# JoeyT1994/TensorNetworkQuantumSimulator.jl

Measured on AMD Instinct MI355X. Metric: two-site gates/sec at fixed chi (LxL TFIM Trotter layer), higher is better.
Workload: dtype c64 (ComplexF32; Gram/eigen steps in f64; the chi = 32 plane products as exact bf16 x 3 splits with f32 accumulation, TNQS_NO_BF16X3=1 for f32 matrix instructions)

## Files before the change

### include/tnqs_debug.h

```cpp
#ifndef TNQS_DEBUG_H
#define TNQS_DEBUG_H
#include <stdint.h>
#include "tnqs.h"
#ifdef __cplusplus
extern "C" {
#endif
int tnqs_dbg_jacobi(int dtype, int m, int n, void* A_inout, void* V_out, int* sweeps_out);
int tnqs_dbg_theta_svd_pre(int m, int n, int nq, void* A_inout, const void* Q, void* V_out, int* sweeps_out, int copies, int reps, double* ms_out, double* phase_us_out ,
                           int cap );
int tnqs_dbg_time_jacobi_f32(int m, int n, const void* A, int copies, int reps, double* ms_out, int* sweeps_out);
int tnqs_dbg_chol(int n, const void* G, void* L_out, void* W_out, int* fail_out, double tau);
int tnqs_dbg_fiber_gemm(int dtype, int D, int PA, int K, int PB, int Do, int No, const void* in, const void* X, void* out,
                        double* norm2_out, int use_mfma);
int tnqs_dbg_gram(int dtype, int D, int PA, int K, int PB, const void* X, const void* Y, void* out, int acc64, int use_mfma);
int tnqs_dbg_gram_fused(int PA, int K, int PB, const void* X, const void* Y, const void* M, void* out);
int tnqs_dbg_gauge_gram(int z, const int* chi, int bleg, const void* X, const void* M, void* out);
int tnqs_dbg_pair(int C0, int NMID, int NHI, const void* in, const void* Mx, const void* My, void* out);
int tnqs_dbg_pair_legs(int d, int z, const int* chi, int lx, int ly, const void* in, const void* Mx, const void* My, void* out);
int tnqs_dbg_pair_gram(int d, int z, const int* chi, int lx, int ly, const void* X, const void* Y, const void* M, void* out);
int tnqs_dbg_pair_gram2(int d, int z, const int* chi, int lx, int ly, const void* X, const void* Y, const void* Mx, const void* My, void* out_y, void* out_x);
int tnqs_dbg_bench_plane(int which, int nsites, int lx, int ly, int reps, double* ms);
#define TNQS_DBG_ROUTE_X3 1
#define TNQS_DBG_ROUTE_F32 2
#define TNQS_DBG_ROUTE_F64 3
#define TNQS_DBG_ROUTE_F64_SHARED 4
#define TNQS_DBG_ROUTE_HALF_LINES 5
#define TNQS_DBG_ROUTE_WHOLE_LINES 6
#define TNQS_DBG_ROUTE_SMALL_SCALAR 7
#define TNQS_DBG_ROUTE_SMALL_MFMA16 8
int tnqs_dbg_rowgemm(int D, int K, int nitems, const int* PA, const int* PB, const int* No, const void* in, const void* X, void* out, double* norm2_out,
                     int tpw, int* route_out);
int tnqs_dbg_gram_mfma(int nitems, const int* shape, const void* X, const void* Y, void* out, int nchunks, int* route_out);
int tnqs_dbg_pair16(int d, int nitems, const int* z, const int* chi, const int* lx, const int* ly, const void* in, const void* M, void* out, int spw, int* route_out);
int tnqs_dbg_pair_gram2x16(int d, int nitems, const int* z, const int* chi, const int* lx, const int* ly, const int* both, const void* X, const void* Y, const void* M,
                           void* out_y, void* out_x, int spw);
int tnqs_dbg_svd_tall(int nitems, const int* m, const int* n, void* A, int* chol_fail, int* polished, int* sweeps);
int tnqs_dbg_small_site(int nitems, const int* d, const int* z, const int* chi, const int* jo, const void* psi, const void* M, const int* present, int form,
                        const void* old_msg, const int* has_old, int normalize, void* out, void* new_msg, double* diff_out, int* route_out);
int tnqs_dbg_msg_finalize(int dtype, int nitems, const int* chi, const int* nchunks, const void* partials, const void* old_msg, const int* has_old, int normalize,
                          void* new_msg, double* diff_out);
int tnqs_dbg_default_sequence(tnqs_handle h, int* src, int* dst, int cap, int* n_out);
int tnqs_dbg_default_sequence_graph(int nv, int ne, const int32_t* esrc, const int32_t* edst, int* src, int* dst, int* level, int cap, int* n_out);
int tnqs_dbg_gate_schedule(int nv, int ne, const int32_t* esrc, const int32_t* edst, int ngates, const int32_t* nverts, const int32_t* verts, int update_cache,
                           int* step_of_gate, int* step_is_bp, int cap, int* nsteps_out);
int tnqs_dbg_fiber_plan(int use, int dtype, int use_mfma, int use_chi64, int nitems, const int* shape, int* launches_out, int cap, int* nlaunches_out, int* items_out);
int tnqs_dbg_loop_cgemm(int dtype, int opB, int nitems, const int* m, const int* n, const int* k, const void* A, const void* B, void* C, int guard);
int tnqs_dbg_loop_antiproject(int dtype, int nitems, const int* nr, const int* nc, void* T_inout, const void* f, const void* b);
int tnqs_dbg_loop_trace(int dtype, int nitems, const int* p, const int* q, const void* X, const void* Y, double* out_re_im);
int tnqs_dbg_msg_rescale(int dtype, int nitems, const int* chi, const void* me, const void* mer, const int* present, void* me_out, void* mer_out, int guard);
int tnqs_dbg_edge_scalar(int dtype, int nitems, const int* chi, const void* me, const void* mer, const int* present, double* out_re_im);
int tnqs_dbg_env_prepare(int dtype, int nitems, const int* n, const void* msg, const int* present, void* H_out, void* V_out, int guard);
int tnqs_dbg_env_finish(int dtype, int nitems, const int* n, const void* A, const void* V, const double* cutoff, void* msqrt_out, void* proj_out, int* flags_out, int guard);
int tnqs_dbg_symg_build(int dtype, int nitems, const int* n, const void* AX, const void* VX, const void* AY, const void* VY, double reg, void* rx, void* ry, void* irx, void* iry,
                        void* Ce, void* Ce0, int* flag_out, int guard);
int tnqs_dbg_symg_finish(int dtype, int nitems, const int* n, const void* USigma, const void* Vsvd, const void* irx, const void* iry, void* Xs, void* Xd, double* S, int guard);
int tnqs_dbg_diag(int dtype, int nitems, const int* chi, const double* S, void* out, int guard);
int tnqs_dbg_cscale(int dtype, int nitems, const int* len, const void* src, const double* re, const double* im, void* dst, int guard);
int tnqs_dbg_pending_scale(tnqs_handle h, int v, double* factor);
#ifdef __cplusplus
}
#endif
#endif
```

### tensornetworkquantumsimulator.jl_amd/csrc/api.cpp

```cpp
#include <cmath>
#include <cstring>
#include <string>
#include "engine.hpp"

using namespace tnqs;

struct tnqs_state_s { State* s; };

static thread_local std::string g_err;

template <class F> static int guard(F&& f) {
    try { f(); return TNQS_OK; }
    catch (const Err& e) { g_err = e.what(); return e.code; }
    catch (const std::bad_alloc&) { g_err = "out of host memory"; return TNQS_ERR_HIP; }
    catch (const std::exception& e) { g_err = e.what(); return TNQS_ERR_INVALID; }
    catch (...) { g_err = "unknown error"; return TNQS_ERR_INVALID; }
}
static State* S(tnqs_handle h) { if (!h || !h->s) throw Err(TNQS_ERR_INVALID, "null handle"); return h->s; }

extern "C" {

int tnqs_version(void) { return 102; }
const char* tnqs_last_error(void) { return g_err.c_str(); }
int tnqs_device_count(int* count) {
// ... 80 lines not shown
            double ore = op[2 * (sp + d * si)], oim = op[2 * (sp + d * si) + 1];
            double rre = r[2 * (si + d * sp)], rim = r[2 * (si + d * sp) + 1];
            nre += ore * rre - oim * rim; nim += ore * rim + oim * rre;
        }
        for (int si = 0; si < d; ++si) { tre += r[2 * (si + d * si)]; tim += r[2 * (si + d * si) + 1]; }
        double den = tre * tre + tim * tim;
        out[0] = (nre * tre + nim * tim) / den; out[1] = (nim * tre - nre * tim) / den;
    });
}
int tnqs_expect_region(tnqs_handle h, int nr, const int32_t* rv, const int32_t* parent, const double* ops, double* out4) {
    return guard([&] { expect_region(S(h), nr, rv, parent, ops, out4); });
}
int tnqs_vertex_scalars(tnqs_handle h, double* out) { return guard([&] { if (!out) throw Err(TNQS_ERR_INVALID, "vertex_scalars: null"); vertex_scalars(S(h), out); }); }
int tnqs_edge_scalars(tnqs_handle h, double* out) { return guard([&] { if (!out) throw Err(TNQS_ERR_INVALID, "edge_scalars: null"); edge_scalars(S(h), out); }); }
int tnqs_rescale(tnqs_handle h) { return guard([&] { rescale(S(h)); }); }
int tnqs_rescale_messages(tnqs_handle h, int n_edges, const int32_t* eu, const int32_t* ev) {
    return guard([&] { if (n_edges < 0) throw Err(TNQS_ERR_INVALID, "rescale_messages: negative count"); rescale_messages(S(h), n_edges, eu, ev); });
}
int tnqs_rescale_vertices(tnqs_handle h, int n_vertices, const int32_t* verts) {
    return guard([&] { if (n_vertices < 0) throw Err(TNQS_ERR_INVALID, "rescale_vertices: negative count"); rescale_vertices(S(h), n_vertices, verts); });
}
int tnqs_symmetric_gauge(tnqs_handle h, double regularization) { return guard([&] { symmetric_gauge(S(h), regularization); }); }
int tnqs_project_site(tnqs_handle h, int v, int config) { return guard([&] { project_site(S(h), v, config); }); }
int tnqs_site_dim(tnqs_handle h, int v, int* d) { return guard([&] { if (!d) throw Err(TNQS_ERR_INVALID, "site_dim: null output"); site_dim(S(h), v, d); }); }
int tnqs_site_probabilities(tnqs_handle h, int v, double* out_p) { return guard([&] { if (!out_p) throw Err(TNQS_ERR_INVALID, "site_probabilities: null output"); site_probabilities(S(h), v, out_p); }); }
int tnqs_sample_bp(tnqs_handle h, int nsamples, const tnqs_bp_opts* bp_opts, uint64_t seed, const double* uniforms, int32_t* out_config, double* out_prob, tnqs_apply_stats* stats) {
    return guard([&] { sample_bp(S(h), nsamples, bp_opts, seed, uniforms, out_config, out_prob, stats); });
}
int tnqs_loop_weights(tnqs_handle h, int ncycles, const int32_t* cycle_len, const int32_t* cycle_verts, double* out_re_im) {
    return guard([&] { loop_weights(S(h), ncycles, cycle_len, cycle_verts, out_re_im); });
}
int tnqs_expect_all(tnqs_handle h, const double* ops, double* out) {
    return guard([&] { if (!ops || !out) throw Err(TNQS_ERR_INVALID, "expect_all: null"); expect_all(S(h), ops, out); });
}

int tnqs_set_sharding(tnqs_handle h, int rank, int nranks, const int32_t* owner, tnqs_allgather_fn fn, void* ctx,
                      void* exch_dev, int64_t exch_bytes) {
    return guard([&] {
        State* s = S(h);
        if (nranks < 1 || rank < 0 || rank >= nranks) throw Err(TNQS_ERR_INVALID, "set_sharding: bad rank");
        if (nranks > 1) {
            if (!owner || !fn || !exch_dev || exch_bytes <= 0) throw Err(TNQS_ERR_INVALID, "set_sharding: owner, callback and exchange buffer are required for nranks > 1");
            for (int v = 0; v < s->g->nv; ++v) if (owner[v] < 0 || owner[v] >= nranks) throw Err(TNQS_ERR_INVALID, "set_sharding: owner out of range");
            s->owner.assign(owner, owner + s->g->nv);
        } else s->owner.clear();
        materialize_pending_all(s);
        s->comm.reset();
        s->rank = rank; s->nranks = nranks; s->ag_fn = fn; s->ag_ctx = ctx; s->exch = exch_dev; s->exch_bytes = (size_t)exch_bytes;
        if (nranks > 1) for (int v = 0; v < s->g->nv; ++v) if (!s->owns(v)) { s->site[v] = nullptr; s->sscale[v] = nullptr; }
    });
}

int tnqs_rccl_unique_id(void* out128) { return guard([&] { if (!out128) throw Err(TNQS_ERR_INVALID, "rccl_unique_id: null output"); rccl_unique_id(out128); }); }
int tnqs_set_sharding_rccl(tnqs_handle h, int rank, int nranks, const int32_t* owner, const void* unique_id128, int64_t exch_bytes) {
    return guard([&] { set_sharding_rccl(S(h), rank, nranks, owner, unique_id128, exch_bytes); });
}
int tnqs_sharding_stats(tnqs_handle h, int64_t* n_exchanges, int64_t* bytes_exchanged) {
    return guard([&] { State* s = S(h); if (n_exchanges) *n_exchanges = s->comm ? s->comm->n_exchanges : 0; if (bytes_exchanged) *bytes_exchanged = s->comm ? s->comm->bytes_exchanged : 0; });
}
int tnqs_rccl_selftest(int device, int64_t bytes) { return guard([&] { rccl_selftest(device, bytes); }); }
int tnqs_rccl_preflight(void) { return guard([&] { rccl_preflight(); }); }

int tnqs_profile_enable(tnqs_handle h, int on) { return guard([&] { S(h)->prof->on = on != 0; }); }
int tnqs_profile_get(tnqs_handle h, int cls, int64_t* launches, double* ms, double* bytes, double* flops) {
    return guard([&] {
        State* s = S(h);
        if (cls < 0 || cls >= TNQS_PROF_NCLASSES) throw Err(TNQS_ERR_INVALID, "profile_get: bad class");
        prof_collect(s);
        const ProfClass& pc = s->prof->cls[cls];
        if (launches) *launches = pc.launches;
        if (ms) *ms = pc.ms;
        if (bytes) *bytes = pc.bytes;
        if (flops) *flops = pc.flops;
    });
}
int tnqs_profile_reset(tnqs_handle h) {
    return guard([&] { State* s = S(h); prof_collect(s); for (auto& p : s->prof->cls) p = ProfClass{}; });
}

}

#include "../../include/tnqs_debug.h"
#include "kernels.hpp"
namespace tnqs { void dbg_default_sequence(const Graph& g, std::vector<int>& src, std::vector<int>& dst);
                 std::shared_ptr<Graph> dbg_make_graph(int nv, int ne, const int32_t* es, const int32_t* ed);
                 void dbg_default_sequence_graph(const Graph& g, std::vector<int>& src, std::vector<int>& dst, std::vector<int>& level);
                 void dbg_pair(int C0, int NMID, int NHI, const void* in, const void* Mx, const void* My, void* out);
                 void dbg_gram_fused(int PA, int K, int PB, const void* X, const void* Y, const void* M, void* out);
                 void dbg_gauge_gram(int z, const int* chi, int bleg, const void* X, const void* M, void* out);
                 void dbg_jacobi(int dtype, int m, int n, void* A, void* V, int* sweeps);
                 void dbg_chol(int n, const void* G, void* L, void* W, int* fail, double tau);
                 void dbg_theta_svd_pre(int m, int n, int nq, void* A, const void* Q, void* V, int* sweeps, int copies, int reps, double* ms, double* phase_us, int cap);
                 void dbg_time_jacobi_f32(int m, int n, const void* A, int copies, int reps, double* ms, int* sweeps);
                 void dbg_pair_legs(int d, int z, const int* chi, int lx, int ly, const void* in, const void* Mx, const void* My, void* out);
                 void dbg_pair_gram2(int d, int z, const int* chi, int lx, int ly, const void* X, const void* Y, const void* Mx, const void* My, void* out_y, void* out_x);
                 void dbg_bench_plane(int which, int nsites, int lx, int ly, int reps, double* ms);
                 void dbg_pair_gram(int d, int z, const int* chi, int lx, int ly, const void* X, const void* Y, const void* M, void* out);
                 void dbg_fiber_gemm(int dtype, int D, int PA, int K, int PB, int Do, int No, const void* in, const void* X, void* out, double* norm2, int use_mfma);
                 void dbg_gram(int dtype, int D, int PA, int K, int PB, const void* X, const void* Y, void* out, int acc64, int use_mfma);
                 void dbg_rowgemm(int D, int K, int nitems, const int* PA, const int* PB, const int* No, const void* in, const void* X, void* out, double* norm2, int tpw, int* route);
                 void dbg_gram_mfma(int nitems, const int* shape, const void* X, const void* Y, void* out, int nchunks, int* route);
                 void dbg_pair16(int d, int nitems, const int* z, const int* chi, const int* lx, const int* ly, const void* in, const void* M, void* out, int spw, int* route);
                 void dbg_pair_gram2x16(int d, int nitems, const int* z, const int* chi, const int* lx, const int* ly, const int* both, const void* X, const void* Y, const void* M,
                                        void* out_y, void* out_x, int spw);
                 void dbg_svd_tall(int nitems, const int* m, const int* n, void* A, int* chol_fail, int* polished, int* sweeps);
                 void dbg_small_site(int nitems, const int* d, const int* z, const int* chi, const int* jo, const void* psi, const void* M, const int* present, int form,
                                     const void* old_msg, const int* has_old, int normalize, void* out, void* new_msg, double* diff, int* route);
                 void dbg_msg_finalize(int dtype, int nitems, const int* chi, const int* nchunks, const void* partials, const void* old_msg, const int* has_old, int normalize,
                                       void* new_msg, double* diff);
                 void dbg_loop_cgemm(int dtype, int opB, int nitems, const int* m, const int* n, const int* k, const void* A, const void* B, void* C, int guard);
                 void dbg_loop_antiproject(int dtype, int nitems, const int* nr, const int* nc, void* T, const void* f, const void* b);
                 void dbg_loop_trace(int dtype, int nitems, const int* p, const int* q, const void* X, const void* Y, double* out);
                 void dbg_msg_rescale(int dtype, int nitems, const int* chi, const void* me, const void* mer, const int* present, void* me_out, void* mer_out, int guard);
                 void dbg_edge_scalar(int dtype, int nitems, const int* chi, const void* me, const void* mer, const int* present, double* out);
                 void dbg_env_prepare(int dtype, int nitems, const int* n, const void* msg, const int* present, void* H_out, void* V_out, int guard);
                 void dbg_env_finish(int dtype, int nitems, const int* n, const void* A, const void* V, const double* cutoff, void* msqrt_out, void* proj_out, int* flags_out, int guard);
                 void dbg_symg_build(int dtype, int nitems, const int* n, const void* AX, const void* VX, const void* AY, const void* VY, double reg, void* rx, void* ry, void* irx, void* iry,
                                     void* Ce, void* Ce0, int* flag_out, int guard);
                 void dbg_symg_finish(int dtype, int nitems, const int* n, const void* USigma, const void* Vsvd, const void* irx, const void* iry, void* Xs, void* Xd, double* S, int guard);
                 void dbg_diag(int dtype, int nitems, const int* chi, const double* S, void* out, int guard);
                 void dbg_cscale(int dtype, int nitems, const int* len, const void* src, const double* re, const double* im, void* dst, int guard);
                 double dbg_pending_scale(State* s, int v); }
extern "C" {
int tnqs_dbg_default_sequence(tnqs_handle h, int* src, int* dst, int cap, int* n_out) {
    return guard([&] { std::vector<int> a, b; dbg_default_sequence(*S(h)->g, a, b); *n_out = (int)a.size();
                       for (int i = 0; i < (int)a.size() && i < cap; ++i) { src[i] = a[i]; dst[i] = b[i]; } });
}
int tnqs_dbg_default_sequence_graph(int nv, int ne, const int32_t* esrc, const int32_t* edst, int* src, int* dst, int* level, int cap, int* n_out) {
    return guard([&] { if (nv < 0 || ne < 0 || (ne > 0 && (!esrc || !edst)) || !n_out) throw Err(TNQS_ERR_INVALID, "tnqs_dbg_default_sequence_graph: bad arguments");
                       auto g = dbg_make_graph(nv, ne, esrc, edst); std::vector<int> a, b, l; dbg_default_sequence_graph(*g, a, b, l); *n_out = (int)a.size();
                       for (int i = 0; i < (int)a.size() && i < cap; ++i) { if (src) src[i] = a[i]; if (dst) dst[i] = b[i]; if (level) level[i] = l[i]; } });
}
int tnqs_dbg_gate_schedule(int nv, int ne, const int32_t* esrc, const int32_t* edst, int ngates, const int32_t* nverts, const int32_t* verts, int update_cache,
                           int* step_of_gate, int* step_is_bp, int cap, int* nsteps_out) {
    return guard([&] { if (nv < 0 || ne < 0 || (ne > 0 && (!esrc || !edst)) || ngates < 0 || (ngates > 0 && (!nverts || !verts)) || !nsteps_out) throw Err(TNQS_ERR_INVALID, "tnqs_dbg_gate_schedule: bad arguments");
                       for (int i = 0, o = 0; i < ngates; o += nverts[i], ++i) { if (nverts[i] < 1 || nverts[i] > 2) throw Err(TNQS_ERR_INVALID, "tnqs_dbg_gate_schedule: only one- and two-site gates");
                                                                                 for (int k = 0; k < nverts[i]; ++k) if (verts[o + k] < 0 || verts[o + k] >= nv) throw Err(TNQS_ERR_INVALID, "tnqs_dbg_gate_schedule: vertex out of range"); }
                       auto g = dbg_make_graph(nv, ne, esrc, edst); const GateSchedule steps = build_gate_schedule(*g, ngates, nverts, verts, update_cache != 0); *nsteps_out = (int)steps.size();
                       for (int k = 0; k < (int)steps.size(); ++k) { if (step_is_bp && k < cap) step_is_bp[k] = steps[k].is_bp ? 1 : 0; if (step_of_gate) for (int i = steps[k].begin; i < steps[k].end; ++i) step_of_gate[i] = k; } });
}
int tnqs_dbg_fiber_plan(int use, int dtype, int use_mfma, int use_chi64, int nitems, const int* shape, int* launches, int cap, int* nlaunches_out, int* items_out) {
    return guard([&] { if (use < 0 || use > 2 || (dtype != TNQS_C64 && dtype != TNQS_C128) || nitems < 0 || (nitems > 0 && !shape) || !nlaunches_out) throw Err(TNQS_ERR_INVALID, "tnqs_dbg_fiber_plan: bad arguments");
                       std::vector<FiberItem> items(nitems);
                       for (int i = 0; i < nitems; ++i) { const int* q = shape + 6 * i; for (int k = 0; k < 6; ++k) if (q[k] < 1) throw Err(TNQS_ERR_INVALID, "tnqs_dbg_fiber_plan: bad shape");
                                                          FiberItem& it = items[i]; it.D = q[0]; it.PA = q[1]; it.K = q[2]; it.PB = q[3]; it.Do = q[4]; it.No = q[5]; }
                       const std::vector<FiberLaunch> plan = plan_fiber_pass(items.data(), nitems, fiber_rules(use == 0 ? FiberUse::Chain : use == 1 ? FiberUse::Epilogue : FiberUse::Plain, dtype == TNQS_C64, use_mfma != 0, use_chi64 != 0),
                                                                            dtype == TNQS_C64 ? 8 : 16);
                       *nlaunches_out = (int)plan.size();
                       for (int l = 0; l < (int)plan.size(); ++l) { const FiberLaunch& L = plan[l];
                           if (launches && l < cap) { const int v[10] = {(int)L.route, L.D, L.K, L.TR, L.tpw, L.KKmax, L.NNmax, L.wgs, (int)L.items.size(), L.general ? 1 : 0}; std::copy(v, v + 10, launches + 10 * l); }
                           if (items_out) for (size_t k = 0; k < L.items.size(); ++k) { const FiberItem& it = L.items[k]; const int v[7] = {l, it.tile_begin, L.nwg[k], it.TA, it.TB, it.nta, it.ntb}; std::copy(v, v + 7, items_out + 7 * L.index[k]); } } });
}
int tnqs_dbg_jacobi(int dtype, int m, int n, void* A, void* V, int* sweeps) { return guard([&] { dbg_jacobi(dtype, m, n, A, V, sweeps); }); }
int tnqs_dbg_theta_svd_pre(int m, int n, int nq, void* A, const void* Q, void* V, int* sweeps, int copies, int reps, double* ms, double* phase_us, int cap) { return guard([&] { dbg_theta_svd_pre(m, n, nq, A, Q, V, sweeps, copies, reps, ms, phase_us, cap); }); }
int tnqs_dbg_time_jacobi_f32(int m, int n, const void* A, int copies, int reps, double* ms, int* sweeps) { return guard([&] { dbg_time_jacobi_f32(m, n, A, copies, reps, ms, sweeps); }); }
int tnqs_dbg_chol(int n, const void* G, void* L, void* W, int* fail, double tau) { return guard([&] { dbg_chol(n, G, L, W, fail, tau); }); }
int tnqs_dbg_fiber_gemm(int dtype, int D, int PA, int K, int PB, int Do, int No, const void* in, const void* X, void* out, double* norm2, int use_mfma) {
    return guard([&] { dbg_fiber_gemm(dtype, D, PA, K, PB, Do, No, in, X, out, norm2, use_mfma); });
}
int tnqs_dbg_pair(int C0, int NMID, int NHI, const void* in, const void* Mx, const void* My, void* out) { return guard([&] { dbg_pair(C0, NMID, NHI, in, Mx, My, out); }); }
int tnqs_dbg_pair_legs(int d, int z, const int* chi, int lx, int ly, const void* in, const void* Mx, const void* My, void* out) { return guard([&] { dbg_pair_legs(d, z, chi, lx, ly, in, Mx, My, out); }); }
int tnqs_dbg_pair_gram2(int d, int z, const int* chi, int lx, int ly, const void* X, const void* Y, const void* Mx, const void* My, void* out_y, void* out_x) {
    return guard([&] { dbg_pair_gram2(d, z, chi, lx, ly, X, Y, Mx, My, out_y, out_x); });
}
int tnqs_dbg_bench_plane(int which, int nsites, int lx, int ly, int reps, double* ms) { return guard([&] { dbg_bench_plane(which, nsites, lx, ly, reps, ms); }); }
int tnqs_dbg_pair_gram(int d, int z, const int* chi, int lx, int ly, const void* X, const void* Y, const void* M, void* out) { return guard([&] { dbg_pair_gram(d, z, chi, lx, ly, X, Y, M, out); }); }
int tnqs_dbg_gram_fused(int PA, int K, int PB, const void* X, const void* Y, const void* M, void* out) { return guard([&] { dbg_gram_fused(PA, K, PB, X, Y, M, out); }); }
int tnqs_dbg_gauge_gram(int z, const int* chi, int bleg, const void* X, const void* M, void* out) { return guard([&] { dbg_gauge_gram(z, chi, bleg, X, M, out); }); }
int tnqs_dbg_gram(int dtype, int D, int PA, int K, int PB, const void* X, const void* Y, void* out, int acc64, int use_mfma) {
    return guard([&] { dbg_gram(dtype, D, PA, K, PB, X, Y, out, acc64, use_mfma); });
}
int tnqs_dbg_rowgemm(int D, int K, int nitems, const int* PA, const int* PB, const int* No, const void* in, const void* X, void* out, double* norm2_out, int tpw, int* route_out) {
    return guard([&] { dbg_rowgemm(D, K, nitems, PA, PB, No, in, X, out, norm2_out, tpw, route_out); });
}
int tnqs_dbg_gram_mfma(int nitems, const int* shape, const void* X, const void* Y, void* out, int nchunks, int* route_out) {
    return guard([&] { dbg_gram_mfma(nitems, shape, X, Y, out, nchunks, route_out); });
}
int tnqs_dbg_pair16(int d, int nitems, const int* z, const int* chi, const int* lx, const int* ly, const void* in, const void* M, void* out, int spw, int* route_out) {
    return guard([&] { dbg_pair16(d, nitems, z, chi, lx, ly, in, M, out, spw, route_out); });
}
int tnqs_dbg_pair_gram2x16(int d, int nitems, const int* z, const int* chi, const int* lx, const int* ly, const int* both, const void* X, const void* Y, const void* M,
                           void* out_y, void* out_x, int spw) {
    return guard([&] { dbg_pair_gram2x16(d, nitems, z, chi, lx, ly, both, X, Y, M, out_y, out_x, spw); });
}
int tnqs_dbg_svd_tall(int nitems, const int* m, const int* n, void* A, int* chol_fail, int* polished, int* sweeps) {
    return guard([&] { dbg_svd_tall(nitems, m, n, A, chol_fail, polished, sweeps); });
}
int tnqs_dbg_small_site(int nitems, const int* d, const int* z, const int* chi, const int* jo, const void* psi, const void* M, const int* present, int form,
                        const void* old_msg, const int* has_old, int normalize, void* out, void* new_msg, double* diff_out, int* route_out) {
    return guard([&] { dbg_small_site(nitems, d, z, chi, jo, psi, M, present, form, old_msg, has_old, normalize, out, new_msg, diff_out, route_out); });
}
int tnqs_dbg_msg_finalize(int dtype, int nitems, const int* chi, const int* nchunks, const void* partials, const void* old_msg, const int* has_old, int normalize,
                          void* new_msg, double* diff_out) {
    return guard([&] { dbg_msg_finalize(dtype, nitems, chi, nchunks, partials, old_msg, has_old, normalize, new_msg, diff_out); });
}
int tnqs_dbg_loop_cgemm(int dtype, int opB, int nitems, const int* m, const int* n, const int* k, const void* A, const void* B, void* C, int guard_elems) {
    return guard([&] { dbg_loop_cgemm(dtype, opB, nitems, m, n, k, A, B, C, guard_elems); });
}
int tnqs_dbg_loop_antiproject(int dtype, int nitems, const int* nr, const int* nc, void* T, const void* f, const void* b) { return guard([&] { dbg_loop_antiproject(dtype, nitems, nr, nc, T, f, b); }); }
int tnqs_dbg_loop_trace(int dtype, int nitems, const int* p, const int* q, const void* X, const void* Y, double* out) { return guard([&] { dbg_loop_trace(dtype, nitems, p, q, X, Y, out); }); }
int tnqs_dbg_msg_rescale(int dtype, int nitems, const int* chi, const void* me, const void* mer, const int* present, void* me_out, void* mer_out, int guard_elems) {
    return guard([&] { dbg_msg_rescale(dtype, nitems, chi, me, mer, present, me_out, mer_out, guard_elems); });
}
int tnqs_dbg_edge_scalar(int dtype, int nitems, const int* chi, const void* me, const void* mer, const int* present, double* out_re_im) {
    return guard([&] { dbg_edge_scalar(dtype, nitems, chi, me, mer, present, out_re_im); });
}
int tnqs_dbg_env_prepare(int dtype, int nitems, const int* n, const void* msg, const int* present, void* H_out, void* V_out, int guard_elems) {
    return guard([&] { dbg_env_prepare(dtype, nitems, n, msg, present, H_out, V_out, guard_elems); });
}
int tnqs_dbg_env_finish(int dtype, int nitems, const int* n, const void* A, const void* V, const double* cutoff, void* msqrt_out, void* proj_out, int* flags_out, int guard_elems) {
    return guard([&] { dbg_env_finish(dtype, nitems, n, A, V, cutoff, msqrt_out, proj_out, flags_out, guard_elems); });
}
int tnqs_dbg_symg_build(int dtype, int nitems, const int* n, const void* AX, const void* VX, const void* AY, const void* VY, double reg, void* rx, void* ry, void* irx, void* iry,
                        void* Ce, void* Ce0, int* flag_out, int guard_elems) {
    return guard([&] { dbg_symg_build(dtype, nitems, n, AX, VX, AY, VY, reg, rx, ry, irx, iry, Ce, Ce0, flag_out, guard_elems); });
}
int tnqs_dbg_symg_finish(int dtype, int nitems, const int* n, const void* USigma, const void* Vsvd, const void* irx, const void* iry, void* Xs, void* Xd, double* S, int guard_elems) {
    return guard([&] { dbg_symg_finish(dtype, nitems, n, USigma, Vsvd, irx, iry, Xs, Xd, S, guard_elems); });
}
int tnqs_dbg_diag(int dtype, int nitems, const int* chi, const double* S, void* out, int guard_elems) { return guard([&] { dbg_diag(dtype, nitems, chi, S, out, guard_elems); }); }
int tnqs_dbg_cscale(int dtype, int nitems, const int* len, const void* src, const double* re, const double* im, void* dst, int guard_elems) {
    return guard([&] { dbg_cscale(dtype, nitems, len, src, re, im, dst, guard_elems); });
}
int tnqs_dbg_pending_scale(tnqs_handle h, int v, double* factor) { return guard([&] { if (!factor) throw Err(TNQS_ERR_INVALID, "dbg_pending_scale: null output"); *factor = dbg_pending_scale(S(h), v); }); }
}
```

### tensornetworkquantumsimulator.jl_amd/csrc/debug.cpp

```cpp
#include <cstdio>
#include <cstring>
#include <cstdlib>
#include <vector>
#include <algorithm>
#include <memory>
#include <string>
#include "engine.hpp"
#include "kernels.hpp"
#include "launch_util.hpp"
#include "../../include/tnqs_debug.h"

namespace tnqs {
#define HIPCHK(x) hipchk((x), #x)
struct DBuf { void* p = nullptr; explicit DBuf(size_t n) { HIPCHK(hipMalloc(&p, n ? n : 1)); } ~DBuf() { (void)hipFree(p); }
              void up(const void* h, size_t n) { HIPCHK(hipMemcpy(p, h, n, hipMemcpyHostToDevice)); } void down(void* h, size_t n) { HIPCHK(hipMemcpy(h, p, n, hipMemcpyDeviceToHost)); } };
static void need_gpu() { int n = 0; if (hipGetDeviceCount(&n) != hipSuccess || n <= 0) throw Err(TNQS_ERR_HIP, "no HIP device available"); }

void dbg_jacobi(int dtype, int m, int n, void* A, void* V, int* sweeps) {
    need_gpu();
    if (m < 1 || n < 1 || m > 256 || n > 256) throw Err(TNQS_ERR_INVALID, "dbg_jacobi: 1 <= m, n <= 256");
    size_t esz = dtype == TNQS_C64 ? 8 : 16;
    DBuf dA((size_t)m * n * esz), dV((size_t)n * n * esz), dS(4), dI(sizeof(JacobiItem));
    dA.up(A, (size_t)m * n * esz);
    if (dtype == TNQS_C64) launch_identity<float>(nullptr, dV.p, n); else launch_identity<double>(nullptr, dV.p, n);
    const size_t lim = 160 * 1024 - 2048;
    size_t lds_av = jacobi_lds_bytes(m, n, true, esz), lds_a = jacobi_lds_bytes(m, n, false, esz);
    const char* fg = std::getenv("TNQS_DBG_NOV_GLOBAL");
    const bool force_global_nov = fg && fg[0] == '1';
    const char* ft = std::getenv("TNQS_DBG_THETA_SVD");
    const bool theta_route = ft && ft[0] == '1' && dtype == TNQS_C64 && lds_a <= lim;
    const bool nov = force_global_nov || theta_route || (lds_av > lim && lds_a <= lim);
    DBuf dA0((size_t)m * n * esz);
    if (nov) dA0.up(A, (size_t)m * n * esz);
    JacobiItem it{dA.p, nov ? nullptr : dV.p, m, n, (int*)dS.p};
    dI.up(&it, sizeof(it));
    size_t lds = force_global_nov ? 0 : (nov ? lds_a : (lds_av <= lim ? lds_av : 0));
    if (dtype == TNQS_C64) launch_jacobi<float>(nullptr, (const JacobiItem*)dI.p, 1, 60, lds, std::max(m, n)); else launch_jacobi<double>(nullptr, (const JacobiItem*)dI.p, 1, 60, lds, std::max(m, n));
    if (nov) {
        DBuf dRv(sizeof(RecoverItem)); RecoverItem rv{dA0.p, dA.p, dV.p, m, n, n}; dRv.up(&rv, sizeof(rv));
        if (dtype == TNQS_C64) launch_recover_v_mfma(nullptr, (const RecoverItem*)dRv.p, 1, n); else launch_recover_v<double>(nullptr, (const RecoverItem*)dRv.p, 1, n);
        HIPCHK(hipDeviceSynchronize());
    }
    HIPCHK(hipDeviceSynchronize());
    dA.down(A, (size_t)m * n * esz); dV.down(V, (size_t)n * n * esz);
    if (sweeps) dS.down(sweeps, 4);
}

void dbg_theta_svd_pre(int m, int n, int nq, void* A, const void* Q, void* V, int* sweeps, int copies, int reps, double* ms, double* phase_us, int cap) {
    need_gpu();
    if (!Q) nq = n;
    if (!theta_svd_pre_covers(m, n) || nq < n || nq > m) throw Err(TNQS_ERR_INVALID, "dbg_theta_svd_pre: 2 <= n <= 64, n <= nq <= m <= 128");
    if (copies < 1) copies = 1;
    const size_t ab = (size_t)m * n * 8, vb = (size_t)nq * n * 8;
    DBuf dA(ab * copies), dA0(ab), dQ((size_t)nq * n * 16), dV(vb * copies), dS(4 * (size_t)copies), dInfo(32), dI(sizeof(JacobiItem) * (size_t)copies), dT(64);
    dA0.up(A, ab); if (Q) dQ.up(Q, (size_t)nq * n * 16);
    const int info[8] = {m, nq, 0, 0, 0, 0, 0, Q ? n : 0};
    dInfo.up(info, 32);
    std::vector<JacobiItem> its(copies);
    for (int c = 0; c < copies; ++c) {
        JacobiItem it{}; it.A = (char*)dA.p + ab * c; it.V = (c == 0 && phase_us) ? dT.p : nullptr; it.m = m; it.n = nq; it.sweeps_out = (int*)dS.p + c; it.dyn = (const int*)dInfo.p; it.dm = 1; it.dn = 1; it.nhint = n;
        it.QB = Q ? dQ.p : nullptr; it.Vout = (char*)dV.p + vb * c; it.pre = 0 ; it.cap = cap; its[c] = it;
    }
    dI.up(its.data(), sizeof(JacobiItem) * (size_t)copies);
    auto reset = [&]() { for (int c = 0; c < copies; ++c) HIPCHK(hipMemcpyAsync((char*)dA.p + ab * c, dA0.p, ab, hipMemcpyDeviceToDevice, nullptr)); };
    reset();
    launch_theta_svd_pre(nullptr, (const JacobiItem*)dI.p, copies, 60, m, n);
    HIPCHK(hipDeviceSynchronize());
    dA.down(A, ab); dV.down(V, vb);
    if (sweeps) dS.down(sweeps, 4);
    if (phase_us) {
        unsigned long long t[8]; dT.down(t, 64);
        for (int k = 0; k < 6; ++k) phase_us[k] = (double)(t[k + 1] - t[k]) * 0.01;
    }
    if (reps > 0 && ms) {
        hipEvent_t e0, e1; HIPCHK(hipEventCreate(&e0)); HIPCHK(hipEventCreate(&e1));
        double tot = 0;
        for (int r = 0; r < reps; ++r) {
            reset();
            HIPCHK(hipEventRecord(e0, nullptr));
            launch_theta_svd_pre(nullptr, (const JacobiItem*)dI.p, copies, 60, m, n);
            HIPCHK(hipEventRecord(e1, nullptr)); HIPCHK(hipEventSynchronize(e1));
            float t = 0; HIPCHK(hipEventElapsedTime(&t, e0, e1)); tot += t;
        }
        *ms = tot / reps;
        (void)hipEventDestroy(e0); (void)hipEventDestroy(e1);
    }
}
void dbg_time_jacobi_f32(int m, int n, const void* A, int copies, int reps, double* ms, int* sweeps) {
    need_gpu();
    if (copies < 1) copies = 1;
    const size_t ab = (size_t)m * n * 8;
    DBuf dA(ab * copies), dA0(ab), dS(4 * (size_t)copies), dI(sizeof(JacobiItem) * (size_t)copies);
    dA0.up(A, ab);
    std::vector<JacobiItem> its(copies);
    for (int c = 0; c < copies; ++c) { JacobiItem it{}; it.A = (char*)dA.p + ab * c; it.m = m; it.n = n; it.sweeps_out = (int*)dS.p + c; its[c] = it; }
    dI.up(its.data(), sizeof(JacobiItem) * (size_t)copies);
    hipEvent_t e0, e1; HIPCHK(hipEventCreate(&e0)); HIPCHK(hipEventCreate(&e1));
    double tot = 0;
// ... 2 lines not shown
        HIPCHK(hipEventRecord(e0, nullptr));
        launch_jacobi<float>(nullptr, (const JacobiItem*)dI.p, copies, 60, jacobi_lds_bytes(m, n, false, 8), std::max(m, n), n);
        HIPCHK(hipEventRecord(e1, nullptr)); HIPCHK(hipEventSynchronize(e1));
        float t = 0; HIPCHK(hipEventElapsedTime(&t, e0, e1)); if (r > 0) tot += t;
    }
    if (ms) *ms = tot / std::max(1, reps);
    if (sweeps) dS.down(sweeps, 4);
    (void)hipEventDestroy(e0); (void)hipEventDestroy(e1);
}

void dbg_chol(int n, const void* G, void* Lout, void* Wout, int* fail, double tau) {
    need_gpu();
    if (n < 1 || n > 128) throw Err(TNQS_ERR_INVALID, "dbg_chol: 1 <= n <= 128");
    const size_t b = (size_t)n * n * 16;
    DBuf dG(b), dL(b), dW(b), dF(4), dI(sizeof(CholItem));
    dG.up(G, b); HIPCHK(hipMemset(dF.p, 0, 4)); HIPCHK(hipMemset(dW.p, 0, b));
    CholItem it{dG.p, dL.p, dW.p, n, (int*)dF.p, tau, 0.0};
    dI.up(&it, sizeof(it));
    if (n <= 96) launch_chol(nullptr, (const CholItem*)dI.p, 1, n); else launch_chol_packed(nullptr, (const CholItem*)dI.p, 1, n);
    HIPCHK(hipDeviceSynchronize());
    dL.down(Lout, b); dW.down(Wout, b); dF.down(fail, 4);
}

void dbg_fiber_gemm(int dtype, int D, int PA, int K, int PB, int Do, int No, const void* in, const void* X, void* out, double* norm2, int use_mfma) {
    need_gpu();
    size_t esz = dtype == TNQS_C64 ? 8 : 16;
    size_t nin = (size_t)D * PA * K * PB, nout = (size_t)Do * PA * No * PB, nx = (size_t)D * K * Do * No;
    DBuf dIn(nin * esz), dX(nx * esz), dOut(nout * esz), dI(sizeof(FiberItem));
    dIn.up(in, nin * esz); dX.up(X, nx * esz);
    HIPCHK(hipMemset(dOut.p, 0xff, nout * esz));
    FiberItem it{}; it.in = dIn.p; it.out = dOut.p; it.X = dX.p; it.D = D; it.PA = PA; it.K = K; it.PB = PB; it.Do = Do; it.No = No;
    it.want_norm = 1;
    FiberRules r = fiber_rules(FiberUse::Epilogue, dtype == TNQS_C64, use_mfma != 0, true); r.rg_D = 0; r.kk_min = 1; r.mfma_tpw = 5; r.f64_tpw = 12;
    const std::vector<FiberLaunch> plan = plan_fiber_pass(&it, 1, r, esz);
    const FiberLaunch& L = plan[0]; const int tiles = L.wgs;
    DBuf dN((size_t)tiles * 8);
    dI.up(L.items.data(), sizeof(FiberItem));
    if (dtype == TNQS_C64) launch_fiber_route<float>(nullptr, L, (const FiberItem*)dI.p, (double*)dN.p);
    else launch_fiber_route<double>(nullptr, L, (const FiberItem*)dI.p, (double*)dN.p);
    HIPCHK(hipDeviceSynchronize());
    dOut.down(out, nout * esz);
    if (norm2) { std::vector<double> np(tiles); dN.down(np.data(), (size_t)tiles * 8); double t = 0; for (double v : np) t += v; *norm2 = t; }
}

void dbg_gram(int dtype, int D, int PA, int K, int PB, const void* X, const void* Y, void* out, int acc64, int use_mfma) {
    need_gpu();
    size_t esz = dtype == TNQS_C64 ? 8 : 16;
    size_t nin = (size_t)D * PA * K * PB; int KK = D * K;
    bool same = (X == Y);
    DBuf dX(nin * esz), dY(same ? 1 : nin * esz), dI(sizeof(GramItem)), dR(sizeof(ReduceItem));
    dX.up(X, nin * esz); if (!same) dY.up(Y, nin * esz);
    GramItem it{}; it.X = dX.p; it.Y = same ? dX.p : dY.p; it.D = D; it.PA = PA; it.K = K; it.PB = PB;
    const bool mf = use_mfma && dtype == TNQS_C64 && !acc64 && KK <= 32;
    const bool mf64 = use_mfma && dtype == TNQS_C64 && acc64 && same && KK <= 64 && KK >= 16;
    const bool mfz = use_mfma && dtype == TNQS_C128 && gram_f64in_covers(D, K);
    const GramRoute r = mfz ? GramRoute::F64In : mf64 ? GramRoute::F64x64 : mf ? GramRoute::Mfma32 : GramRoute::Generic;
    const int TR = gram_tile_rows(r, KK, esz);
    tile_params(PA, PB, TR, it.TA, it.TB, it.nta, it.ntb);
    const char* e = std::getenv("TNQS_DBG_GRAM_CHUNKS");
    int npart = 0; plan_gram(&it, 1, r, false, e ? std::max(1, std::atoi(e)) : 7, &npart);
    bool a64 = acc64 || dtype == TNQS_C128;
    size_t asz = a64 ? 16 : 8;
    DBuf dP((size_t)npart * KK * KK * asz), dO((size_t)KK * KK * asz);
    it.partial = dP.p; dI.up(&it, sizeof(it));
    const GramItem* d = (const GramItem*)dI.p;
    if (dtype == TNQS_C128) launch_gram_route<double, double>(nullptr, r, d, 1, it.nchunks, TR, KK, KK == 64);
    else if (a64) launch_gram_route<float, double>(nullptr, r, d, 1, it.nchunks, TR, KK, KK == 64);
    else launch_gram_route<float, float>(nullptr, r, d, 1, it.nchunks, TR, KK);
    ReduceItem ri{dP.p, dO.p, KK * KK, npart, 0, 0}; dR.up(&ri, sizeof(ri));
    if (a64) launch_reduce<double, double>(nullptr, (const ReduceItem*)dR.p, 1, KK * KK); else launch_reduce<float, float>(nullptr, (const ReduceItem*)dR.p, 1, KK * KK);
    HIPCHK(hipDeviceSynchronize());
    dO.down(out, (size_t)KK * KK * asz);
}
void dbg_pair(int C0, int NMID, int NHI, const void* in, const void* Mx, const void* My, void* out) {
    need_gpu();
    if (C0 % 16) throw Err(TNQS_ERR_INVALID, "dbg_pair: C0 % 16 != 0");
    size_t n = (size_t)C0 * 32 * NMID * 32 * NHI;
    DBuf dIn(n * 8), dOut(n * 8), dX(32 * 32 * 8), dY(32 * 32 * 8), dI(sizeof(PairItem));
    dIn.up(in, n * 8); dX.up(Mx, 32 * 32 * 8); dY.up(My, 32 * 32 * 8);
    HIPCHK(hipMemset(dOut.p, 0xff, n * 8));
    PairItem it{}; it.in = dIn.p; it.out = dOut.p; it.Mx = dX.p; it.My = dY.p;
    it.g.cstr = 2; it.g.sx = C0; it.g.sy = (long long)C0 * 32 * NMID; it.g.n0 = C0 / 16; it.g.t0 = 16; it.g.n1 = NMID; it.g.t1 = (long long)C0 * 32;
    it.g.n2 = NHI; it.g.t2 = (long long)C0 * 32 * NMID * 32;
    const int wgs = plan_pair(&it, 1, 3);
    dI.up(&it, sizeof(it));
    launch_mfma_pair(nullptr, (const PairItem*)dI.p, 1, wgs);
    HIPCHK(hipDeviceSynchronize());
    dOut.down(out, n * 8);
}
void dbg_pair_legs(int d, int z, const int* chi, int lx, int ly, const void* in, const void* Mx, const void* My, void* out) {
    need_gpu();
    PairItem it{};
    if (!pair_geometry(d, z, chi, lx, ly, it.g)) throw Err(TNQS_ERR_UNSUPPORTED, "dbg_pair_legs: shape not covered by the pair kernel");
    size_t n = d; for (int i = 0; i < z; ++i) n *= chi[i];
    DBuf dIn(n * 8), dOut(n * 8), dX(32 * 32 * 8), dY(32 * 32 * 8), dI(sizeof(PairItem));
    dIn.up(in, n * 8); dX.up(Mx, 32 * 32 * 8); dY.up(My, 32 * 32 * 8);
    HIPCHK(hipMemset(dOut.p, 0xff, n * 8));
    it.in = dIn.p; it.out = dOut.p; it.Mx = dX.p; it.My = dY.p;
    if ((size_t)it.g.n0 * it.g.n1 * it.g.n2 * 16 * 1024 != n) throw Err(TNQS_ERR_INVALID, "dbg_pair_legs: slice count");
    const int wgs = plan_pair(&it, 1, 3);
    dI.up(&it, sizeof(it));
    launch_mfma_pair(nullptr, (const PairItem*)dI.p, 1, wgs);
    HIPCHK(hipDeviceSynchronize());
    dOut.down(out, n * 8);
}
void dbg_pair_gram(int d, int z, const int* chi, int lx, int ly, const void* X, const void* Y, const void* M, void* out) {
    need_gpu();
    PairGramItem it{};
    if (!pair_geometry(d, z, chi, lx, ly, it.g)) throw Err(TNQS_ERR_UNSUPPORTED, "dbg_pair_gram: shape not covered by the pair kernel");
    size_t n = d; for (int i = 0; i < z; ++i) n *= chi[i];
    const bool x3 = mfma_use_x3();
    PairGram2Item one{}; one.g = it.g;
    const int nwg = x3 ? plan_x3_pair_gram1(&one, 1, nullptr, 3) : plan_pair_gram(&it, 1, nullptr, 3), npart = nwg;
    DBuf dX(n * 8), dY(n * 8), dM(32 * 32 * 8), dI(sizeof(PairGram2Item)), dR(sizeof(ReduceItem)), dP((size_t)npart * 1024 * 8), dO(1024 * 8);
    dX.up(X, n * 8); dY.up(Y, n * 8); dM.up(M, 32 * 32 * 8);
    it.X = dX.p; it.Y = dY.p; it.M = dM.p; it.partial = dP.p;
    if (x3) {
        one.X = it.X; one.Y = it.Y; one.Mx = it.M; one.partial_y = it.partial;
        dI.up(&one, sizeof(one));
        launch_x3_pair_gram1(nullptr, (const PairGram2Item*)dI.p, 1, nwg);
    } else {
        dI.up(&it, sizeof(it));
        launch_mfma_pair_gram(nullptr, (const PairGramItem*)dI.p, 1, nwg);
    }
    ReduceItem ri{dP.p, dO.p, 1024, npart, 0, 0}; dR.up(&ri, sizeof(ri));
    launch_reduce<float, float>(nullptr, (const ReduceItem*)dR.p, 1, 1024);
    HIPCHK(hipDeviceSynchronize());
    dO.down(out, 1024 * 8);
}
void dbg_pair_gram2(int d, int z, const int* chi, int lx, int ly, const void* X, const void* Y, const void* Mx, const void* My, void* out_y, void* out_x) {
    need_gpu();
    PairGram2Item it{};
    if (!pair_geometry(d, z, chi, lx, ly, it.g)) throw Err(TNQS_ERR_UNSUPPORTED, "dbg_pair_gram2: shape not covered");
    size_t n = d; for (int i = 0; i < z; ++i) n *= chi[i];
    const int nwg = plan_pair_gram2(&it, 1, nullptr, 3), npart = nwg;
    DBuf dX(n * 8), dY(n * 8), dMx(1024 * 8), dMy(1024 * 8), dI(sizeof(PairGram2Item)), dR(2 * sizeof(ReduceItem)), dP1((size_t)npart * 1024 * 8), dP2((size_t)npart * 1024 * 8), dO(2 * 1024 * 8);
    dX.up(X, n * 8); dY.up(Y, n * 8); dMx.up(Mx, 1024 * 8); dMy.up(My, 1024 * 8);
    it.X = dX.p; it.Y = dY.p; it.Mx = dMx.p; it.My = dMy.p; it.partial_y = dP1.p; it.partial_x = dP2.p;
    dI.up(&it, sizeof(it));
    launch_mfma_pair_gram2(nullptr, (const PairGram2Item*)dI.p, 1, nwg);
    ReduceItem ri[2] = {{dP1.p, dO.p, 1024, npart, 0, 0}, {dP2.p, (char*)dO.p + 1024 * 8, 1024, npart, 0, 1024}};
    dR.up(ri, sizeof(ri));
    launch_reduce<float, float>(nullptr, (const ReduceItem*)dR.p, 2, 2048);
    HIPCHK(hipDeviceSynchronize());
    dO.down(out_y, 1024 * 8);
    HIPCHK(hipMemcpy(out_x, (char*)dO.p + 1024 * 8, 1024 * 8, hipMemcpyDeviceToHost));
}
static void fill_random(void* d, size_t nfloats, unsigned seed) {
    const size_t blk = (size_t)1 << 22;
    std::vector<float> h(blk + 4096);
    unsigned x = seed * 2654435761u + 12345u;
    for (auto& v : h) { x = x * 1664525u + 1013904223u; v = ((int)(x >> 8) - (1 << 23)) * (0.01f / (1 << 23)); }
    size_t off = 0; unsigned k = 0;
    while (off < nfloats) {
        const size_t m = std::min(blk, nfloats - off);
        HIPCHK(hipMemcpy((char*)d + off * 4, h.data() + (k * 257u) % 4096u, m * 4, hipMemcpyHostToDevice));
        off += m; ++k;
    }
}
static void dbg_bench_plane16(int which, int nsites, int lx, int ly, int reps, double* ms) {
    const int chi[6] = {16, 16, 16, 16, 16, 16};
    PlaneGeom g{};
    if (!plane_geometry(2, 6, chi, lx, ly, 16, g)) throw Err(TNQS_ERR_UNSUPPORTED, "dbg_bench_plane: legs not covered");
    const size_t n = (size_t)2 << 24;
    DBuf dA((size_t)nsites * n * 8), dB((size_t)nsites * n * 8), dM(2 * 256 * 8);
    fill_random(dA.p, (size_t)nsites * n * 2, 1); fill_random(dB.p, (size_t)nsites * n * 2, 2); fill_random(dM.p, 2 * 256 * 2, 3);
    hipEvent_t e0, e1; HIPCHK(hipEventCreate(&e0)); HIPCHK(hipEventCreate(&e1));
    float t = 0.f;
    if (which == 2) {
        std::vector<Pair16Item> items(nsites);
        for (int i = 0; i < nsites; ++i) {
            Pair16Item& it = items[i]; it.g = g; it.in = (char*)dA.p + (size_t)i * n * 8; it.out = (char*)dB.p + (size_t)i * n * 8;
            it.Mx = dM.p; it.My = (char*)dM.p + 256 * 8;
        }
        int w[2]; plan_pair16(items.data(), nsites, w);
        const int wgs = w[pair16_whole_lines(g) ? 1 : 0];
        DBuf dI(items.size() * sizeof(Pair16Item)); dI.up(items.data(), items.size() * sizeof(Pair16Item));
        launch_mfma_pair16(nullptr, (const Pair16Item*)dI.p, nsites, wgs, pair16_whole_lines(g));
        HIPCHK(hipEventRecord(e0, nullptr));
        for (int r = 0; r < reps; ++r) launch_mfma_pair16(nullptr, (const Pair16Item*)dI.p, nsites, wgs, pair16_whole_lines(g));
        HIPCHK(hipEventRecord(e1, nullptr)); HIPCHK(hipEventSynchronize(e1)); HIPCHK(hipEventElapsedTime(&t, e0, e1));
    } else {
        std::vector<PairGram2x16Item> items(nsites);
        for (auto& it : items) it.g = g;
        const int wgs = plan_pair_gram2x16(items.data(), nsites), nwg = wgs / nsites;
        DBuf dP((size_t)2 * nsites * nwg * 256 * 8);
        for (int i = 0; i < nsites; ++i) {
            PairGram2x16Item& it = items[i]; it.X = (char*)dA.p + (size_t)i * n * 8; it.Y = (char*)dB.p + (size_t)i * n * 8;
            it.Mx = dM.p; it.My = (char*)dM.p + 256 * 8;
            it.partial_y = (char*)dP.p + (size_t)(2 * i) * nwg * 256 * 8; it.partial_x = (char*)dP.p + (size_t)(2 * i + 1) * nwg * 256 * 8;
        }
        DBuf dI(items.size() * sizeof(PairGram2x16Item)); dI.up(items.data(), items.size() * sizeof(PairGram2x16Item));
        launch_mfma_pair_gram2x16(nullptr, (const PairGram2x16Item*)dI.p, nsites, wgs);
        HIPCHK(hipEventRecord(e0, nullptr));
        for (int r = 0; r < reps; ++r) launch_mfma_pair_gram2x16(nullptr, (const PairGram2x16Item*)dI.p, nsites, wgs);
        HIPCHK(hipEventRecord(e1, nullptr)); HIPCHK(hipEventSynchronize(e1)); HIPCHK(hipEventElapsedTime(&t, e0, e1));
    }
    HIPCHK(hipDeviceSynchronize());
    (void)hipEventDestroy(e0); (void)hipEventDestroy(e1);
    *ms = (double)t / reps;
}
void dbg_bench_plane(int which, int nsites, int lx, int ly, int reps, double* ms) {
    need_gpu();
    if (which == 2 || which == 3) { dbg_bench_plane16(which, nsites, lx, ly, reps, ms); return; }
    const int chi[4] = {32, 32, 32, 32};
    PairGeom g{};
    if (!pair_geometry(2, 4, chi, lx, ly, g)) throw Err(TNQS_ERR_UNSUPPORTED, "dbg_bench_plane: legs not covered");
    const size_t n = (size_t)2 * 32 * 32 * 32 * 32;
    DBuf dA((size_t)nsites * n * 8), dB((size_t)nsites * n * 8), dM(2 * 1024 * 8);
    fill_random(dA.p, (size_t)nsites * n * 2, 1); fill_random(dB.p, (size_t)nsites * n * 2, 2); fill_random(dM.p, 2 * 1024 * 2, 3);
    hipEvent_t e0, e1; HIPCHK(hipEventCreate(&e0)); HIPCHK(hipEventCreate(&e1));
    float t = 0.f;
    if (which == 4) {
        const char* e = std::getenv("TNQS_DBG_GROUP"); int G = e ? std::atoi(e) : 0; if (G <= 0 || G > nsites) G = nsites;
        int ox = -1, oy = -1; for (int q = 0; q < 4; ++q) if (q != lx && q != ly) { if (ox < 0) ox = q; else oy = q; }
        PairGeom g2{}; if (!pair_geometry(2, 4, chi, ox, oy, g2)) throw Err(TNQS_ERR_UNSUPPORTED, "dbg_bench_plane: other legs not covered");
        const int ngroups = (nsites + G - 1) / G;
        std::vector<PairItem> pit(nsites); std::vector<PairGram2Item> git(nsites);
        for (int i = 0; i < nsites; ++i) { pit[i].g = g; git[i].g = g2; }
        std::vector<int> pw(ngroups), gwg(ngroups), nwg(nsites);
        for (int gr = 0; gr < ngroups; ++gr) {
            const int cnt = std::min(G, nsites - gr * G);
            pw[gr] = plan_pair(&pit[(size_t)gr * G], cnt, gr ? pit[0].spw : 0);
            gwg[gr] = plan_pair_gram2(&git[(size_t)gr * G], cnt, &nwg[(size_t)gr * G], gr ? git[0].spw : 0);
        }
        const int spw_p = pit[0].spw, spw_g = git[0].spw, nwg_g = nwg[0];
        DBuf dT((size_t)G * n * 8), dP((size_t)2 * nsites * nwg_g * 1024 * 8);
        for (int i = 0; i < nsites; ++i) {
            const int k = i % G;
            PairItem& a = pit[i]; a.in = (char*)dA.p + (size_t)i * n * 8; a.out = (char*)dT.p + (size_t)k * n * 8; a.Mx = dM.p; a.My = (char*)dM.p + 1024 * 8;
            PairGram2Item& b = git[i]; b.X = a.out; b.Y = a.in; b.Mx = dM.p; b.My = (char*)dM.p + 1024 * 8;
            b.partial_y = (char*)dP.p + (size_t)(2 * i) * nwg_g * 1024 * 8; b.partial_x = (char*)dP.p + (size_t)(2 * i + 1) * nwg_g * 1024 * 8;
        }
        DBuf dPI(pit.size() * sizeof(PairItem)), dGI(git.size() * sizeof(PairGram2Item));
        dPI.up(pit.data(), pit.size() * sizeof(PairItem)); dGI.up(git.data(), git.size() * sizeof(PairGram2Item));
        auto level = [&]() {
            for (int gr = 0; gr < ngroups; ++gr) {
                const int cnt = std::min(G, nsites - gr * G);
                launch_mfma_pair(nullptr, (const PairItem*)dPI.p + (size_t)gr * G, cnt, pw[gr]);
                launch_mfma_pair_gram2(nullptr, (const PairGram2Item*)dGI.p + (size_t)gr * G, cnt, gwg[gr]);
            }
        };
        level();
        HIPCHK(hipEventRecord(e0, nullptr));
        for (int r = 0; r < reps; ++r) level();
        HIPCHK(hipEventRecord(e1, nullptr)); HIPCHK(hipEventSynchronize(e1)); HIPCHK(hipEventElapsedTime(&t, e0, e1));
        std::fprintf(stderr, "level bench: group %d, pair spw %d, gram spw %d\n", G, spw_p, spw_g);
    } else if (which == 0) {
        std::vector<PairItem> items(nsites);
        for (int i = 0; i < nsites; ++i) {
            PairItem& it = items[i]; it.g = g; it.in = (char*)dA.p + (size_t)i * n * 8; it.out = (char*)dB.p + (size_t)i * n * 8;
            it.Mx = dM.p; it.My = (char*)dM.p + 1024 * 8;
        }
        const int wgs = plan_pair(items.data(), nsites);
        DBuf dI(items.size() * sizeof(PairItem)); dI.up(items.data(), items.size() * sizeof(PairItem));
        launch_mfma_pair(nullptr, (const PairItem*)dI.p, nsites, wgs);
        HIPCHK(hipEventRecord(e0, nullptr));
        for (int r = 0; r < reps; ++r) launch_mfma_pair(nullptr, (const PairItem*)dI.p, nsites, wgs);
        HIPCHK(hipEventRecord(e1, nullptr)); HIPCHK(hipEventSynchronize(e1)); HIPCHK(hipEventElapsedTime(&t, e0, e1));
    } else {
        std::vector<PairGram2Item> items(nsites);
        for (auto& it : items) it.g = g;
        const int wgs = plan_pair_gram2(items.data(), nsites, nullptr, 16), nwg = wgs / nsites;
        DBuf dP((size_t)2 * nsites * nwg * 1024 * 8);
        for (int i = 0; i < nsites; ++i) {
            PairGram2Item& it = items[i]; it.X = (char*)dA.p + (size_t)i * n * 8; it.Y = (char*)dB.p + (size_t)i * n * 8;
            it.Mx = dM.p; it.My = (char*)dM.p + 1024 * 8;
            it.partial_y = (char*)dP.p + (size_t)(2 * i) * nwg * 1024 * 8; it.partial_x = (char*)dP.p + (size_t)(2 * i + 1) * nwg * 1024 * 8;
        }
        DBuf dI(items.size() * sizeof(PairGram2Item)); dI.up(items.data(), items.size() * sizeof(PairGram2Item));
        launch_mfma_pair_gram2(nullptr, (const PairGram2Item*)dI.p, nsites, wgs);
        HIPCHK(hipEventRecord(e0, nullptr));
        for (int r = 0; r < reps; ++r) launch_mfma_pair_gram2(nullptr, (const PairGram2Item*)dI.p, nsites, wgs);
        HIPCHK(hipEventRecord(e1, nullptr)); HIPCHK(hipEventSynchronize(e1)); HIPCHK(hipEventElapsedTime(&t, e0, e1));
    }
    HIPCHK(hipDeviceSynchronize());
    (void)hipEventDestroy(e0); (void)hipEventDestroy(e1);
    *ms = (double)t / reps;
}
void dbg_gram_fused(int PA, int K, int PB, const void* X, const void* Y, const void* M, void* out) {
    need_gpu();
    size_t nin = (size_t)PA * K * PB;
    DBuf dX(nin * 8), dY(nin * 8), dM(32 * 32 * 8), dI(sizeof(GramItem)), dR(sizeof(ReduceItem));
    dX.up(X, nin * 8); dY.up(Y, nin * 8); dM.up(M, 32 * 32 * 8);
    GramItem it{}; it.X = dX.p; it.Y = dY.p; it.M = dM.p; it.D = 1; it.PA = PA; it.K = K; it.PB = PB;
    tile_params(PA, PB, 64, it.TA, it.TB, it.nta, it.ntb);
    if (it.TA * it.TB != 64) throw Err(TNQS_ERR_INVALID, "dbg_gram_fused: tiles must hold 64 fibers");
    int npart = 0; plan_gram(&it, 1, GramRoute::Fused32, false, 3, &npart);
    DBuf dP((size_t)npart * K * K * 8), dO((size_t)K * K * 8);
    it.partial = dP.p; dI.up(&it, sizeof(it));
    launch_gram_route<float, float>(nullptr, GramRoute::Fused32, (const GramItem*)dI.p, 1, it.nchunks, 64, K);
    ReduceItem ri{dP.p, dO.p, K * K, npart, 0, 0}; dR.up(&ri, sizeof(ri));
    launch_reduce<float, float>(nullptr, (const ReduceItem*)dR.p, 1, K * K);
    HIPCHK(hipDeviceSynchronize());
    dO.down(out, (size_t)K * K * 8);
}
void dbg_gauge_gram(int z, const int* chi, int bleg, const void* X, const void* M, void* out) {
    need_gpu();
    if (z < 2 || z > 8 || bleg < 0 || bleg >= z) throw Err(TNQS_ERR_INVALID, "dbg_gauge_gram: bad shape");
    const int rleg = bleg == 0 ? 1 : 0, K = chi[bleg], KK = 2 * K;
    const bool k16 = gauge_gram32_covers(2, z, chi, bleg, rleg), k32 = gauge_gram64_covers(2, z, chi, bleg, rleg);
    if (!k16 && !k32) throw Err(TNQS_ERR_UNSUPPORTED, "dbg_gauge_gram: shape not covered by the fused kernels");
    size_t n = 2; for (int i = 0; i < z; ++i) n *= chi[i];
    long long PA = 1, PB = 1; for (int i = 0; i < bleg; ++i) PA *= chi[i]; for (int i = bleg + 1; i < z; ++i) PB *= chi[i];
    DBuf dX(n * 8), dM((size_t)chi[rleg] * chi[rleg] * 8), dI(sizeof(GramItem)), dR(sizeof(ReduceItem));
    dX.up(X, n * 8); dM.up(M, (size_t)chi[rleg] * chi[rleg] * 8);
    GramItem it{}; it.X = dX.p; it.Y = dX.p; it.M = dM.p; it.D = 2; it.PA = (int)PA; it.K = K; it.PB = (int)PB;
    tile_params(PA, PB, 64, it.TA, it.TB, it.nta, it.ntb);
    if (k16) { it.nta = gauge_gram32_units(z, chi, bleg); it.ntb = 1; }
    const GramRoute r = k16 ? GramRoute::Gauge32 : GramRoute::Gauge64;
    int npart = 0; plan_gram(&it, 1, r, true, 5, &npart);
    DBuf dP((size_t)npart * KK * KK * 16), dO((size_t)KK * KK * 16);
    HIPCHK(hipMemset(dP.p, 0, (size_t)npart * KK * KK * 16));
    it.partial = dP.p; dI.up(&it, sizeof(it));
    launch_gram_route<float, double>(nullptr, r, (const GramItem*)dI.p, 1, it.nchunks, 64, KK);
    ReduceItem ri{dP.p, dO.p, KK * KK, npart, 0, 0}; dR.up(&ri, sizeof(ri));
    launch_reduce<double, double>(nullptr, (const ReduceItem*)dR.p, 1, KK * KK);
    HIPCHK(hipDeviceSynchronize());
    dO.down(out, (size_t)KK * KK * 16);
}

namespace {
template <class F> void cat_offsets(int n, std::vector<size_t>& off, F&& size_of) { off.assign(n + 1, 0); for (int i = 0; i < n; ++i) off[i + 1] = off[i] + size_of(i); }
}
void svd_tall(State* s, const std::vector<JacobiItem>& tall, int* d_fail, int* d_polish_sweeps);

void dbg_rowgemm(int D, int K, int nitems, const int* PA, const int* PB, const int* No, const void* in, const void* X, void* out, double* norm2, int tpw, int* route) {
    need_gpu();
    if (nitems < 1 || !PA || !PB || !No) throw Err(TNQS_ERR_INVALID, "dbg_rowgemm: bad arguments");
    std::vector<FiberItem> items(nitems);
    for (int i = 0; i < nitems; ++i) {
        FiberItem& it = items[i]; it.D = D; it.PA = PA[i]; it.K = K; it.PB = PB[i]; it.Do = D; it.No = No[i];
        if (PA[i] < 1 || PB[i] < 1 || !rowgemm_covers(it)) throw Err(TNQS_ERR_UNSUPPORTED, "dbg_rowgemm: item not covered by the register-direct kernels");
        it.want_norm = 1;
    }
    std::vector<size_t> oi, ox, oo;
    cat_offsets(nitems, oi, [&](int i) { return (size_t)D * PA[i] * K * PB[i]; });
    cat_offsets(nitems, ox, [&](int i) { return (size_t)D * K * D * No[i]; });
    cat_offsets(nitems, oo, [&](int i) { return (size_t)D * PA[i] * No[i] * PB[i]; });
    DBuf dIn(oi[nitems] * 8), dX(ox[nitems] * 8), dOut(oo[nitems] * 8), dI(sizeof(FiberItem) * nitems);
    dIn.up(in, oi[nitems] * 8); dX.up(X, ox[nitems] * 8);
    HIPCHK(hipMemset(dOut.p, 0xff, oo[nitems] * 8));
    for (int i = 0; i < nitems; ++i) {
        FiberItem& it = items[i];
        it.in = (char*)dIn.p + oi[i] * 8; it.X = (char*)dX.p + ox[i] * 8; it.out = (char*)dOut.p + oo[i] * 8;
    }
// ... 49 lines not shown
        ri[i] = ReduceItem{items[i].partial, (char*)dO.p + oo[i] * asz, (int)(oo[i + 1] - oo[i]), npart[i], 0, (int)oo[i]};
    }
    dI.up(items.data(), sizeof(GramItem) * nitems); dR.up(ri.data(), sizeof(ReduceItem) * nitems);
    if (f64) {
        launch_gram_route<float, double>(nullptr, r, (const GramItem*)dI.p, nitems, chunks, 64, KKmax, all128);
        launch_reduce<double, double>(nullptr, (const ReduceItem*)dR.p, nitems, (int)oo[nitems]);
    } else {
        launch_gram_route<float, float>(nullptr, r, (const GramItem*)dI.p, nitems, chunks, 64, KKmax);
        launch_reduce<float, float>(nullptr, (const ReduceItem*)dR.p, nitems, (int)oo[nitems]);
    }
    HIPCHK(hipDeviceSynchronize());
    dO.down(out, oo[nitems] * asz);
    if (route) *route = f64 ? (all128 ? TNQS_DBG_ROUTE_F64_SHARED : TNQS_DBG_ROUTE_F64) : (mfma_use_x3() ? TNQS_DBG_ROUTE_X3 : TNQS_DBG_ROUTE_F32);
}

static void plane_items(int d, int nitems, const int* z, const int* chi, const int* lx, const int* ly, std::vector<PlaneGeom>& g, std::vector<size_t>& off) {
    if (nitems < 1 || !z || !chi || !lx || !ly || d < 1) throw Err(TNQS_ERR_INVALID, "dbg plane kernels: bad arguments");
    g.resize(nitems);
    int c = 0;
    cat_offsets(nitems, off, [&](int i) {
        if (z[i] < 2 || z[i] > 8) throw Err(TNQS_ERR_INVALID, "dbg plane kernels: 2 <= z <= 8");
        size_t n = d; for (int k = 0; k < z[i]; ++k) n *= chi[c + k];
        if (!plane_geometry(d, z[i], chi + c, lx[i], ly[i], 16, g[i]) || (size_t)g[i].nslices() * 16 * 256 != n)
            throw Err(TNQS_ERR_UNSUPPORTED, "dbg plane kernels: plane not covered by the chi = 16 kernels");
        c += z[i];
        return n;
    });
}
void dbg_pair16(int d, int nitems, const int* z, const int* chi, const int* lx, const int* ly, const void* in, const void* M, void* out, int spw, int* route) {
    need_gpu();
    std::vector<PlaneGeom> g; std::vector<size_t> off;
    plane_items(d, nitems, z, chi, lx, ly, g, off);
    const bool wl = pair16_whole_lines(g[0]);
    for (int i = 0; i < nitems; ++i) if (pair16_whole_lines(g[i]) != wl) throw Err(TNQS_ERR_UNSUPPORTED, "dbg_pair16: one launch holds items of one kind");
    if (spw > 0 && spw % 4) throw Err(TNQS_ERR_INVALID, "dbg_pair16: spw must be a multiple of 4");
    const size_t n = off[nitems];
    DBuf dIn(n * 8), dOut(n * 8), dM((size_t)nitems * 512 * 8), dI(sizeof(Pair16Item) * nitems);
    dIn.up(in, n * 8); dM.up(M, (size_t)nitems * 512 * 8);
    HIPCHK(hipMemset(dOut.p, 0xff, n * 8));
    std::vector<Pair16Item> items(nitems);
    for (int i = 0; i < nitems; ++i) {
        Pair16Item& it = items[i]; it.g = g[i]; it.in = (char*)dIn.p + off[i] * 8; it.out = (char*)dOut.p + off[i] * 8;
        it.Mx = (char*)dM.p + (size_t)i * 512 * 8; it.My = (char*)it.Mx + 256 * 8;
    }
    int wgs[2]; plan_pair16(items.data(), nitems, wgs, spw);
    dI.up(items.data(), sizeof(Pair16Item) * nitems);
    launch_mfma_pair16(nullptr, (const Pair16Item*)dI.p, nitems, wgs[wl ? 1 : 0], wl);
    HIPCHK(hipDeviceSynchronize());
    dOut.down(out, n * 8);
    if (route) *route = wl ? TNQS_DBG_ROUTE_WHOLE_LINES : TNQS_DBG_ROUTE_HALF_LINES;
}
void dbg_pair_gram2x16(int d, int nitems, const int* z, const int* chi, const int* lx, const int* ly, const int* both, const void* X, const void* Y, const void* M,
                       void* out_y, void* out_x, int spw) {
    need_gpu();
    std::vector<PlaneGeom> g; std::vector<size_t> off;
    plane_items(d, nitems, z, chi, lx, ly, g, off);
    if (!both) throw Err(TNQS_ERR_INVALID, "dbg_pair_gram2x16: bad arguments");
    if (spw > 0 && spw % pair_gram2x16_slices_at_a_time()) throw Err(TNQS_ERR_INVALID, "dbg_pair_gram2x16: spw must be a multiple of the slices a workgroup walks at a time");
    const size_t n = off[nitems];
    std::vector<PairGram2x16Item> items(nitems); std::vector<int> nwg(nitems); for (int i = 0; i < nitems; ++i) items[i].g = g[i];
    const int wgs = plan_pair_gram2x16(items.data(), nitems, nwg.data(), spw);
    DBuf dX(n * 8), dY(n * 8), dM((size_t)nitems * 512 * 8), dI(sizeof(PairGram2x16Item) * nitems), dP((size_t)2 * wgs * 256 * 8), dO((size_t)2 * nitems * 256 * 8),
         dR(sizeof(ReduceItem) * 2 * nitems);
    dX.up(X, n * 8); dY.up(Y, n * 8); dM.up(M, (size_t)nitems * 512 * 8);
    HIPCHK(hipMemset(dO.p, 0, (size_t)2 * nitems * 256 * 8));
    std::vector<ReduceItem> ri;
    for (int i = 0; i < nitems; ++i) {
        PairGram2x16Item& it = items[i];
        it.X = (char*)dX.p + off[i] * 8; it.Y = (char*)dY.p + off[i] * 8;
        it.Mx = (char*)dM.p + (size_t)i * 512 * 8; it.My = both[i] ? (const void*)((char*)it.Mx + 256 * 8) : nullptr;
        it.partial_y = (char*)dP.p + (size_t)it.wg_begin * 256 * 8;
        it.partial_x = both[i] ? (void*)((char*)dP.p + ((size_t)wgs + it.wg_begin) * 256 * 8) : nullptr;
        ri.push_back(ReduceItem{it.partial_y, (char*)dO.p + (size_t)i * 256 * 8, 256, nwg[i], 0, (int)ri.size() * 256});
        if (both[i]) ri.push_back(ReduceItem{it.partial_x, (char*)dO.p + ((size_t)nitems + i) * 256 * 8, 256, nwg[i], 0, (int)ri.size() * 256});
    }
    dI.up(items.data(), sizeof(PairGram2x16Item) * nitems); dR.up(ri.data(), sizeof(ReduceItem) * ri.size());
    launch_mfma_pair_gram2x16(nullptr, (const PairGram2x16Item*)dI.p, nitems, wgs);
    launch_reduce<float, float>(nullptr, (const ReduceItem*)dR.p, (int)ri.size(), (int)ri.size() * 256);
    HIPCHK(hipDeviceSynchronize());
    dO.down(out_y, (size_t)nitems * 256 * 8);
    if (out_x) for (int i = 0; i < nitems; ++i) if (both[i]) HIPCHK(hipMemcpy((char*)out_x + (size_t)i * 256 * 8, (char*)dO.p + ((size_t)nitems + i) * 256 * 8, 256 * 8, hipMemcpyDeviceToHost));
}

void dbg_svd_tall(int nitems, const int* m, const int* n, void* A, int* chol_fail, int* polished, int* sweeps) {
    need_gpu();
    if (nitems < 1 || !m || !n || !A) throw Err(TNQS_ERR_INVALID, "dbg_svd_tall: bad arguments");
    for (int i = 0; i < nitems; ++i)
        if (n[i] < 2 || n[i] > 128 || m[i] < n[i] || m[i] > 256) throw Err(TNQS_ERR_UNSUPPORTED, "dbg_svd_tall: 2 <= n <= 128, n <= m <= 256");
    std::vector<size_t> off; cat_offsets(nitems, off, [&](int i) { return (size_t)m[i] * n[i]; });
    int dev = 0; HIPCHK(hipGetDevice(&dev));
    std::unique_ptr<State> s(state_create(1, 0, nullptr, nullptr, nullptr, TNQS_C64, dev));
    {
        DBuf dA(off[nitems] * 8), dF(sizeof(int) * nitems), dS(sizeof(int) * nitems), dW(sizeof(int) * nitems);
        dA.up(A, off[nitems] * 8);
        HIPCHK(hipMemset(dS.p, 0, sizeof(int) * nitems)); HIPCHK(hipMemset(dW.p, 0xff, sizeof(int) * nitems));
        std::vector<JacobiItem> tall(nitems);
        for (int i = 0; i < nitems; ++i) { JacobiItem j{}; j.A = (char*)dA.p + off[i] * 8; j.m = m[i]; j.n = n[i]; j.sweeps_out = (int*)dS.p + i; tall[i] = j; }
        svd_tall(s.get(), tall, (int*)dF.p, (int*)dW.p);
        HIPCHK(hipStreamSynchronize(s->stream));
        dA.down(A, off[nitems] * 8);
        std::vector<int> f(nitems), w(nitems);
        dF.down(f.data(), sizeof(int) * nitems); dW.down(w.data(), sizeof(int) * nitems);
        if (sweeps) dS.down(sweeps, sizeof(int) * nitems);
        for (int i = 0; i < nitems; ++i) { if (chol_fail) chol_fail[i] = f[i]; if (polished) polished[i] = w[i] >= 0; }
    }
}

namespace {
inline size_t round256(size_t b) { return (b + 255) & ~(size_t)255; }
struct Slots {
    std::vector<size_t> off, len; std::vector<char> host; std::unique_ptr<DBuf> dev;
    void add(size_t bytes) { off.push_back(total); len.push_back(bytes); total += round256(bytes); }
    void alloc() { host.assign(total ? total : 1, (char)0xff); dev.reset(new DBuf(total)); }
    void put(size_t i, const void* src) { std::memcpy(host.data() + off[i], src, len[i]); }
    void get(size_t i, void* dst) const { std::memcpy(dst, host.data() + off[i], len[i]); }
    void up() { dev->up(host.data(), total); }
    void down(const char* what) {
        dev->down(host.data(), total);
        for (size_t i = 0; i < off.size(); ++i)
            for (size_t b = off[i] + len[i]; b < off[i] + round256(len[i]); ++b)
                if (host[b] != (char)0xff) throw Err(TNQS_ERR_INVALID, std::string("dbg: a kernel wrote past the end of a slot of ") + what);
    }
    char* at(size_t i) const { return (char*)dev->p + off[i]; }
    size_t total = 0;
};
}
void dbg_small_site(int nitems, const int* d, const int* z, const int* chi, const int* jo, const void* psi, const void* M, const int* present, int form,
                    const void* old_msg, const int* has_old, int normalize, void* out, void* new_msg, double* diff, int* route) {
    need_gpu();
    if (nitems < 1 || !d || !z || !chi || !jo || !psi || !M || !present || !out || form < -1 || form > 1 || (old_msg && !has_old))
        throw Err(TNQS_ERR_INVALID, "dbg_small_site: bad arguments");
    std::vector<SmallMsgItem> items(nitems); std::vector<int> leg0(nitems + 1, 0);
    Slots sPsi, sM, sOut, sNew, sOld, sRaw;
    int max_elems = 0;
    for (int i = 0; i < nitems; ++i) {
        if (z[i] < 1 || z[i] > 8) throw Err(TNQS_ERR_UNSUPPORTED, "dbg_small_site: 1 <= z <= 8");
        const int* c = chi + leg0[i]; leg0[i + 1] = leg0[i] + z[i];
        size_t n = (size_t)std::max(d[i], 0);
        for (int k = 0; k < z[i]; ++k) { if (c[k] < 1) throw Err(TNQS_ERR_INVALID, "dbg_small_site: leg dimension < 1"); n *= (size_t)c[k]; }
        if (!bp_small_site_covers(d[i], z[i], c, n)) throw Err(TNQS_ERR_UNSUPPORTED, "dbg_small_site: site not covered by bp_small_site_kernel (z <= 8, chi <= 32, <= 8192 elements)");
        if (jo[i] < 0 || jo[i] >= z[i]) throw Err(TNQS_ERR_INVALID, "dbg_small_site: outgoing leg out of range");
        bool all16 = (n % 256) == 0; for (int k = 0; k < z[i]; ++k) all16 = all16 && c[k] == 16;
        if (form == 1 && !all16) throw Err(TNQS_ERR_UNSUPPORTED, "dbg_small_site: the matrix-core form takes sites whose legs are all 16-dimensional");
        SmallMsgItem& it = items[i]; it = SmallMsgItem{};
        it.d = d[i]; it.z = z[i]; it.jo = jo[i]; it.mfma = (form != 0 && all16) ? 1 : 0; it.normalize = normalize;
        for (int k = 0; k < z[i]; ++k) { it.chi[k] = c[k]; sM.add((size_t)c[k] * c[k] * 8); }
        const size_t mb = (size_t)c[jo[i]] * c[jo[i]] * 8;
        sPsi.add(n * 8); sOut.add(mb); sNew.add(mb); sOld.add(mb); sRaw.add(mb);
        max_elems = std::max(max_elems, (int)n);
    }
    sPsi.alloc(); sM.alloc(); sOut.alloc(); sNew.alloc(); sOld.alloc(); sRaw.alloc();
    DBuf dDiff(sizeof(double) * nitems), dI(sizeof(SmallMsgItem) * nitems), dF(sizeof(MsgFinalItem) * nitems);
    std::vector<double> hdiff(nitems, 0.0); if (diff) std::copy(diff, diff + nitems, hdiff.begin());
    std::vector<MsgFinalItem> fin;
    const char *hpsi = (const char*)psi, *hM = (const char*)M, *hold = (const char*)old_msg; char *hout = (char*)out, *hnew = (char*)new_msg;
    size_t opsi = 0, oM = 0, omsg = 0;
    for (int i = 0; i < nitems; ++i) {
        SmallMsgItem& it = items[i];
        sPsi.put(i, hpsi + opsi); opsi += sPsi.len[i];
        for (int k = 0; k < it.z; ++k) {
            const size_t q = (size_t)leg0[i] + k;
            if (present[q]) { sM.put(q, hM + oM); it.M[k] = sM.at(q); }
            oM += sM.len[q];
        }
        sOut.put(i, hout + omsg); if (hnew) sNew.put(i, hnew + omsg);
        const bool old = hold && has_old[i]; if (old) sOld.put(i, hold + omsg);
// ... 311 lines not shown
```

### tensornetworkquantumsimulator.jl_amd/csrc/engine.hpp

```cpp
#pragma once
#include <hip/hip_runtime_api.h>
#include <climits>
#include <cstdint>
#include <deque>
#include <functional>
#include <map>
#include <memory>
#include <mutex>
#include <stdexcept>
#include <string>
#include <unordered_map>
#include <vector>
#include "../../include/tnqs.h"

namespace tnqs {

struct Err : std::runtime_error {
    int code;
    Err(int c, const std::string& m) : std::runtime_error(m), code(c) {}
};
void hipchk(hipError_t e, const char* what);

class Pool {
public:
// ... 16 lines not shown
    void* p = nullptr; size_t bytes = 0; size_t rounded = 0; std::shared_ptr<Pool> pool;
    std::shared_ptr<DevBuf> parent;
    ~DevBuf() { if (p && pool) pool->release(p, rounded); }
};
using Buf = std::shared_ptr<DevBuf>;
inline Buf sub_buffer(const Buf& parent, size_t off, size_t bytes) {
    Buf b = std::make_shared<DevBuf>(); b->p = reinterpret_cast<char*>(parent->p) + off; b->bytes = bytes; b->parent = parent; return b;
}

struct BPPlan {
    std::vector<int> seq;
    std::vector<std::vector<int>> levels;
    std::vector<int> pos_of;
    std::vector<int> level_of;
    bool in_place = false;
    int nlev = 0;
    std::vector<std::vector<int>> out_level, in_level;
    int levels_until(int L, int from) const { return L > from ? L - from : (L < from ? nlev - from + L : 0); }
    int levels_until_next(int L, int from) const { return L > from ? L - from : nlev - from + L; }
    int horizon(int src, int j, int t) const { const int L = in_level[src][j]; return L < 0 ? INT_MAX : levels_until(L, level_of[t]); }
};

struct Graph {
    int nv = 0, ne = 0;
    std::vector<int> esrc, edst;
    std::vector<std::vector<int>> nbr, nbr_e;
    std::unordered_map<uint64_t, int> emap;
    bool is_tree = false;
    std::vector<int> ecolor; int ncolors = 0;
    mutable std::vector<int> default_seq;
    mutable std::vector<int> default_set_starts;
    mutable std::shared_ptr<const BPPlan> default_plan;
    mutable std::shared_ptr<const BPPlan> forest_plan;
    mutable int spec_penalty = 0;
    int edge(int u, int v) const;
    int leg(int v, int w) const;
    int dedge(int src, int dst) const;
    int src_of(int de) const { return (de & 1) ? edst[de / 2] : esrc[de / 2]; }
    int dst_of(int de) const { return (de & 1) ? esrc[de / 2] : edst[de / 2]; }
};
std::shared_ptr<const BPPlan> plan_for(const Graph& g, const tnqs_bp_opts* o);

struct GateStep { bool is_bp; int begin, end; };
using GateSchedule = std::vector<GateStep>;
struct State;
void validate_gates(const State& s, int ngates, const int32_t* nverts, const int32_t* verts, std::vector<int>& voff, std::vector<size_t>& moff);
GateSchedule build_gate_schedule(const Graph& g, int ngates, const int32_t* nverts, const int32_t* verts, bool update_cache);

struct ProfClass { int64_t launches = 0; double ms = 0, bytes = 0, flops = 0; };
struct Prof {
    bool on = false; ProfClass cls[TNQS_PROF_NCLASSES];
    struct Pending { int cls; hipEvent_t a, b; bool own_a; };
    std::vector<Pending> pending; std::vector<hipEvent_t> ev_free;
    hipEvent_t last_b = nullptr; bool chain = false; hipStream_t last_stream = nullptr;
    ~Prof() { for (auto& p : pending) { if (p.own_a) (void)hipEventDestroy(p.a); (void)hipEventDestroy(p.b); } for (auto e : ev_free) (void)hipEventDestroy(e); }
};

struct RcclComm {
    void* comm = nullptr; int device = 0; void* exch_owned = nullptr;
    long long n_exchanges = 0, bytes_exchanged = 0;
    ~RcclComm();
};

constexpr int kCheckEvents = 16;
struct HostArena {
    char* base = nullptr; size_t cap = 0, off = 0;
    char* ring = nullptr; size_t ring_cap = 0, ring_off = 0;
    hipEvent_t cev[kCheckEvents] = {}; unsigned cevn = 0;
};

struct Check {
    int kind = 0;
    int step = 0;
    int iters_done = 0;
    hipEvent_t ev = nullptr;
    std::function<bool(State*)> eval;
};

struct State {
    std::shared_ptr<Graph> g;
    int dtype = TNQS_C64;
    bool real_io = false;
    int device = 0;
    std::vector<int> d;
    std::vector<char> projected;
    std::vector<int> chi;
    std::vector<Buf> site;
    std::vector<Buf> sscale;
    std::vector<std::vector<double>> pend1; std::vector<char> unit_norm;
    bool in_apply = false;
    std::vector<Buf> msg;
    std::shared_ptr<Pool> pool;
    hipStream_t stream = nullptr; bool own_stream = false;
    hipStream_t aux_stream = nullptr; hipEvent_t ev_fork = nullptr, ev_join = nullptr;
    int rank = 0, nranks = 1; std::vector<int> owner; tnqs_allgather_fn ag_fn = nullptr; void* ag_ctx = nullptr;
    void* exch = nullptr; size_t exch_bytes = 0;
    std::shared_ptr<RcclComm> comm;
    std::shared_ptr<Prof> prof;
    std::vector<Buf> keepalive;
    size_t keep_mark = 0;
    HostArena arena;
    tnqs_apply_stats stats{};
    std::deque<Check> checks;
    int cur_step = -1;

    size_t esz() const { return dtype == TNQS_C64 ? 8 : 16; }
    int scalartype() const { return real_io ? (dtype == TNQS_C64 ? TNQS_F32 : TNQS_F64) : dtype; }
    size_t io_esz() const { return real_io ? esz() / 2 : esz(); }
    bool owns(int v) const { return nranks == 1 || owner[v] == rank; }
    bool force_exchange = false;
    bool msg_hermitian = true;
    bool sharded() const { return nranks > 1 || force_exchange; }
    ~State();
};

State* state_create(int nv, int ne, const int32_t* es, const int32_t* ed, const int32_t* sd, int dtype, int device);
State* state_copy(const State* s);
void state_set_site(State* s, int v, const void* host, int ndim, const int64_t* dims, const int32_t* role);
void state_get_site(State* s, int v, void* host, int ndim, const int32_t* role);
void state_set_site_random(State* s, int v, int nn, const int64_t* bond_dims, uint64_t seed, double scale);
int64_t state_site_size(const State* s, int v);
void state_set_message(State* s, int src, int dst, const void* host, int chi);
void state_get_message(State* s, int src, int dst, void* host, int chi);
void bp_update(State* s, const tnqs_bp_opts* opts, int* niter, double* diff);
void apply_gates(State* s, int ngates, const int32_t* nverts, const int32_t* verts, const double* mats,
                 const tnqs_apply_opts* opts, const tnqs_bp_opts* bp, double* errs);
void truncate_bp(State* s, int maxdim, double cutoff, int normalize, int ngroups, const int32_t* offs,
                 const int32_t* eu, const int32_t* ev, const tnqs_bp_opts* bp);
void rdm_1site(State* s, int v, double* out);
void expect_all(State* s, const double* ops, double* out);
void expect_region(State* s, int nr, const int32_t* rv, const int32_t* parent, const double* ops, double* out4);
void vertex_scalars(State* s, double* out);
void edge_scalars(State* s, double* out);
void rescale(State* s);
void rescale_messages(State* s, int n, const int32_t* eu, const int32_t* ev);
void rescale_vertices(State* s, int n, const int32_t* verts);
void symmetric_gauge(State* s, double regularization);
void site_dim(const State* s, int v, int* d);
void project_site(State* s, int v, int config);
void site_probabilities(State* s, int v, double* out_p);
void sample_bp(State* s, int nsamples, const tnqs_bp_opts* bp, uint64_t seed, const double* uniforms, int32_t* out_config, double* out_prob, tnqs_apply_stats* stats);
void loop_weights(State* s, int ncycles, const int32_t* cycle_len, const int32_t* cycle_verts, double* out_re_im);
void prof_collect(State* s);
void materialize_pending_all(State* s);
void rccl_unique_id(void* out128);
void set_sharding_rccl(State* s, int rank, int nranks, const int32_t* owner, const void* unique_id128, int64_t exch_bytes);
void rccl_allgather(State* s, size_t bytes_per_rank);
void rccl_selftest(int device, int64_t bytes);
void rccl_preflight();

}
```

### tensornetworkquantumsimulator.jl_amd/csrc/engine_batch.cpp

```cpp
#include "engine_internal.hpp"

namespace tnqs {

void FiberPass::prepare(State* s, size_t k, bool norms) {
    if (norms) np[k] = dalloc(s, (size_t)std::max(1, plan[k].wgs) * sizeof(double));
    d_items[k] = upload(s, plan[k].items);
}
template <class T> void FiberPass::launch(State* s, size_t k, int cls, bool book) const {
    const FiberLaunch& L = plan[k];
    if (L.items.empty()) return;
    double* const partials = np[k] ? reinterpret_cast<double*>(np[k]->p) : nullptr;
    if (cls < 0) { launch_fiber_route<T>(s->stream, L, d_items[k], partials); return; }
    double bytes = 0, flops = 0;
    const bool rg = L.route == FiberRoute::RowGemm;
    if (book && !(rg && k > 0))
        for (size_t q = k; q < plan.size() && (q == k || (rg && plan[q].route == FiberRoute::RowGemm)); ++q)
            for (const FiberItem& it : plan[q].items) {
                const double fibers = (double)it.PA * it.PB, nin = fibers * it.D * it.K;
                bytes += (nin + fibers * it.Do * it.No) * s->esz(); flops += 8.0 * nin * it.Do * it.No;
            }
    ProfScope ps(s, cls, bytes, flops);
    launch_fiber_route<T>(s->stream, L, d_items[k], partials);
}
template void FiberPass::launch<float>(State*, size_t, int, bool) const;
template void FiberPass::launch<double>(State*, size_t, int, bool) const;

template <class T> void run_chains(State* s, std::vector<Chain>& chains, int cls, int cls_pair) {
    if (cls_pair < 0) cls_pair = cls;
    const size_t esz = s->esz();
    std::vector<int> nt(chains.size(), 0);
    for (auto& c : chains) c.result = c.src;
    if (std::is_same<T, float>::value && use_mfma() && use_pair()) {
        std::vector<PairItem> items; double bytes = 0, flops = 0;
        std::vector<std::pair<size_t, std::pair<int, int>>> sel;
        for (size_t ci = 0; ci < chains.size(); ++ci) {
            Chain& c = chains[ci];
            if (c.steps.size() < 2) continue;
            int py = -1, px = -1;
            for (int q = (int)c.steps.size() - 1; q >= 0 && px < 0; --q) {
                int leg = c.steps[q].first;
                bool ok = c.sd.chi[leg] == 32 && leg >= 1 && (c.sd.pre(leg) % 16 == 0);
                if (!ok) continue;
                if (py < 0) py = q; else px = q;
            }
            if (px < 0) continue;
            sel.push_back({ci, {px, py}});
        }
        if (!sel.empty()) {
            for (auto& se : sel) {
                Chain& c = chains[se.first];
                int x = c.steps[se.second.first].first, y = c.steps[se.second.second].first;
                PairItem it{};
                Buf& dst = c.tmp[nt[se.first] & 1];
                if (!dst) dst = dalloc(s, c.sd.n * esz);
                it.in = c.result; it.out = dst->p; it.Mx = c.steps[se.second.first].second; it.My = c.steps[se.second.second].second;
                if (!pair_geometry(c.sd.d, c.sd.z, c.sd.chi.data(), x, y, it.g)) throw Err(TNQS_ERR_HIP, "internal: pair geometry");
                items.push_back(it);
                c.result = dst->p; nt[se.first]++; c.trail.push_back({x, y});
                c.steps.erase(c.steps.begin() + se.second.second); c.steps.erase(c.steps.begin() + se.second.first);
                bytes += 2.0 * c.sd.n * esz; flops += 2 * 8.0 * c.sd.n * 32;
            }
            const int wgs = plan_pair(items.data(), (int)items.size());
            const PairItem* d = upload(s, items);
            ProfScope ps(s, cls_pair, bytes, flops);
            launch_mfma_pair(s->stream, d, (int)items.size(), wgs);
        }
        for (;;) {
            std::vector<Pair16Item> it16; std::vector<std::pair<size_t, std::pair<int, int>>> sel16; double by16 = 0, fl16 = 0;
            for (size_t ci = 0; ci < chains.size(); ++ci) {
                Chain& c = chains[ci];
                if (c.steps.size() < 2 || c.sd.n < (size_t)(1u << 14)) continue;
                bool found = false;
                if (c.ordered) {
                    Pair16Item it{};
                    if (plane_geometry(c.sd.d, c.sd.z, c.sd.chi.data(), c.steps[0].first, c.steps[1].first, 16, it.g)) {
                        it.Mx = c.steps[0].second; it.My = c.steps[1].second;
                        it16.push_back(it); sel16.push_back({ci, {0, 1}}); found = true;
                    }
                }
                for (int qx = 0; qx + 1 < (int)c.steps.size() && !found; ++qx)
                    for (int qy = (int)c.steps.size() - 1; qy > qx && !found; --qy) {
                        Pair16Item it{};
                        if (!plane_geometry(c.sd.d, c.sd.z, c.sd.chi.data(), c.steps[qx].first, c.steps[qy].first, 16, it.g)) continue;
                        it.Mx = c.steps[qx].second; it.My = c.steps[qy].second;
                        it16.push_back(it); sel16.push_back({ci, {qx, qy}}); found = true;
                    }
            }
            if (it16.empty()) break;
            std::vector<Pair16Item> kind[2]; int wgs16[2];
            plan_pair16(it16.data(), (int)it16.size(), wgs16);
            for (size_t q = 0; q < it16.size(); ++q) {
                Chain& c = chains[sel16[q].first]; Pair16Item& it = it16[q];
                Buf& dst = c.tmp[nt[sel16[q].first] & 1];
                if (!dst) dst = dalloc(s, c.sd.n * esz);
                it.in = c.result; it.out = dst->p;
                kind[pair16_whole_lines(it.g) ? 1 : 0].push_back(it);
                c.result = dst->p; nt[sel16[q].first]++;
                c.trail.push_back({c.steps[sel16[q].second.first].first, c.steps[sel16[q].second.second].first});
                c.steps.erase(c.steps.begin() + sel16[q].second.second); c.steps.erase(c.steps.begin() + sel16[q].second.first);
                by16 += 2.0 * c.sd.n * esz; fl16 += 2 * 8.0 * c.sd.n * 16;
            }
            ProfScope ps(s, cls_pair, by16, fl16);
            for (int wl = 0; wl < 2; ++wl) {
                if (kind[wl].empty()) continue;
                const Pair16Item* d = upload(s, kind[wl]);
                launch_mfma_pair16(s->stream, d, (int)kind[wl].size(), wgs16[wl], wl == 1);
            }
        }
    }
    size_t maxsteps = 0;
    for (auto& c : chains) maxsteps = std::max(maxsteps, c.steps.size());
    const FiberRules rules = fiber_rules_of(s, FiberUse::Chain);
    std::vector<FiberItem> items;
    for (size_t o = 0; o < maxsteps; ++o) {
        items.clear();
        for (size_t ci = 0; ci < chains.size(); ++ci) {
            Chain& c = chains[ci];
            if (c.steps.size() <= o) continue;
            const int j = c.steps[o].first;
            c.trail.push_back({j});
            Buf& dst = c.tmp[nt[ci] & 1];
            if (!dst) dst = dalloc(s, c.sd.n * esz);
            FiberItem it = site_fiber_item(c.sd, j, false, c.sd.chi[j], false);
            it.in = c.result; it.out = dst->p; it.X = c.steps[o].second;
            items.push_back(it);
            c.result = dst->p; nt[ci]++;
        }
        FiberPass(items, rules, esz).run<T>(s, cls, false);
    }
}

void svd_tall(State* s, const std::vector<JacobiItem>& tall, int* d_fail_out, int* d_polish_sweeps) {
    const size_t esz = sizeof(float) * 2;
    const size_t nt = tall.size();
    size_t off = 0; std::vector<size_t> oG(nt), oL(nt), oW(nt), oR0(nt), oRr(nt), oJ(nt), oT(nt);
    for (size_t i = 0; i < nt; ++i) {
        const size_t nn = (size_t)tall[i].n * tall[i].n, mn = (size_t)tall[i].m * tall[i].n;
        oG[i] = off; off += round256(nn * 16); oL[i] = off; off += round256(nn * 16); oW[i] = off; off += round256(nn * 16);
        oR0[i] = off; off += round256(nn * 8); oRr[i] = off; off += round256(nn * 8); oJ[i] = off; off += round256(nn * 16); oT[i] = off; off += round256(mn * 8);
    }
    Buf arena = dalloc(s, off); s->keepalive.push_back(arena);
    Buf fail_buf; if (!d_fail_out) { fail_buf = dalloc(s, nt * sizeof(int)); s->keepalive.push_back(fail_buf); }
    int* const d_fail = d_fail_out ? d_fail_out : reinterpret_cast<int*>(fail_buf->p);
    HIPCHK(hipMemsetAsync(d_fail, 0, nt * sizeof(int), s->stream));
    char* ap = reinterpret_cast<char*>(arena->p);
    std::vector<TallSvdItem> ti, wi; std::vector<CholItem> ci; std::vector<JacobiItem> rj; std::vector<SmallGemmItem> gi; std::vector<CopyItem> cp;
    int nmax = 1, mmax = 1;
    for (size_t i = 0; i < nt; ++i) {
// ... 110 lines not shown
```

### tensornetworkquantumsimulator.jl_amd/csrc/engine_bp.cpp

```cpp
#include "engine_internal.hpp"
#include "launch_util.hpp"

namespace tnqs {

static int fused_leg(const State* s, const SD& sd, int jo) {
    if (s->dtype != TNQS_C64 || !use_mfma() || sd.d != 2 || sd.z < 2) return -1;
    int r = (jo == 0) ? 1 : 0;
    if (sd.chi[r] != 32 || sd.chi[jo] > 32 || sd.chi[jo] < 8) return -1;
    return r;
}

static double default_tol(const State* s) { return s->dtype == TNQS_C64 ? 1e-5 : 1e-8; }
static bool small_site_on() { static const bool v = !envflag("TNQS_NO_SMALL_SITE_BP"); return v; }

struct SharedT { Buf site, ma, mb, T; int la = -1, lb = -1; };

typedef std::vector<std::pair<int, Buf>> LegBufs;
struct ProdEntry { Buf site; LegBufs legs; Buf prod; long long next_use = 0; };
static void drop_legs(LegBufs& want, const LegBufs& have) {
    LegBufs rest; for (auto& w : want) { bool in = false; for (auto& b : have) in = in || b.first == w.first; if (!in) rest.push_back(w); }
    want.swap(rest);
}
struct SweepClock { int level = 0, iter = 1, maxiter = 1; };
struct ProdCache {
// ... 334 lines not shown
        const int fr = fused_leg(s, c.sd, jo);
        std::vector<char> done(c.sd.z, 0);
        {
            auto pf = prefix.find(src);
            if (pf != prefix.end() && pf->second.prod && (!pf->second.has_bra || pf->second.bra) && pf->second.site == s->site[src]) {
                bool same = true;
                for (auto& lm : pf->second.legs) { if (lm.first == jo) { same = false; break; } const Buf& mb = u.incoming(src, lm.first, t); if (!mb || mb->p != lm.second) { same = false; break; } }
                if (same) { c.y = pf->second.has_bra ? pf->second.bra->p : c.src; c.src = pf->second.prod->p; for (auto& lm : pf->second.legs) done[lm.first] = 1; }
            }
        }
        LegBufs want, base;
        for (int j = 0; j < c.sd.z; ++j) {
            if (j == jo || done[j]) continue;
            const Buf& mb = u.incoming(src, j, t);
            if (!mb) continue;
            want.push_back({j, mb});
        }
        const bool from_prefix = c.y != nullptr;
        if (u.cache_on && !from_prefix) {
            u.by_stability(want, src, t); c.ordered = true;
            const void* psi = c.src;
            if (continue_from_remembered(c, want, base)) c.y = psi;
        }
        for (auto& w : want) {
            if (w.first == fr) m.fused = w.second->p;
            else c.steps.push_back({w.first, w.second->p});
        }
        if (u.cache_on && !from_prefix) continued[msgs.size()] = Continued{std::move(base), std::move(want)};
        m.route = m.fused ? Route::GenericFused : Route::GenericPlain;
    }

    void pair_up_planes16() {
        if (!(std::is_same<T, float>::value && use_mfma() && use_pair())) return;
        std::unordered_map<int, std::vector<int>> by_src;
        for (size_t ci = 0; ci < chains.size(); ++ci)
            if (chains[ci].y && chains[ci].steps.size() == 1 && !msgs[ci].fused && chains[ci].sd.n >= (size_t)(1u << 14)) by_src[chains[ci].v].push_back((int)ci);
        for (auto& kv : by_src) {
            if (kv.second.size() != 2) continue;
            const int ci = kv.second[0], cj = kv.second[1];
            Chain& a = chains[ci]; Chain& b = chains[cj];
            const int ly = msgs[ci].jo, lx = msgs[cj].jo;
            if (a.src != b.src || a.y != b.y || a.steps[0].first != lx || b.steps[0].first != ly) continue;
            PairGram2x16Item it{};
            if (!plane_geometry(a.sd.d, a.sd.z, a.sd.chi.data(), lx, ly, 16, it.g)) continue;
            it.X = a.src; it.Y = a.y; it.Mx = a.steps[0].second; it.My = b.steps[0].second;
            g16.push_back(it); g16_msg.push_back({ci, cj});
            a.steps.clear(); b.steps.clear();
            msgs[ci].route = msgs[cj].route = Route::Plane16Double;
        }
        for (size_t ci = 0; ci < chains.size(); ++ci) {
            Chain& c = chains[ci];
            if (!generic(msgs[ci].route)) continue;
            auto ct = continued.find(ci);
            if ((c.y && (ct == continued.end() || ct->second.base.empty())) || msgs[ci].fused || c.steps.empty() || (c.steps.size() & 1) == 0 || c.sd.n < (size_t)(1u << 14)) continue;
            const int ly = msgs[ci].jo, lx = c.steps.back().first;
            PairGram2x16Item it{};
            if (!plane_geometry(c.sd.d, c.sd.z, c.sd.chi.data(), lx, ly, 16, it.g)) continue;
            bool all16 = true; for (auto& st : c.steps) all16 = all16 && c.sd.chi[st.first] == 16;
            if (!all16) continue;
            it.Y = c.y ? c.y : c.src; it.Mx = c.steps.back().second; it.My = nullptr; it.X = nullptr;
            c.steps.pop_back();
            g16_single.push_back((int)g16.size());
            g16.push_back(it); g16_msg.push_back({(int)ci, -1});
            msgs[ci].route = Route::Plane16Single;
        }
    }

    struct SplitGuard { State* s; hipStream_t m; bool on; ~SplitGuard() { s->stream = m; if (on) s->pool->set_defer(false); } };
    void on_side(bool side) { if (split_level) { s->stream = side ? side_stream : main_stream; s->prof->chain = false; } }
    void fork() {
        main_stream = s->stream;
        bool has_other = false;
        for (const Msg& m : msgs) has_other = has_other || m.route == Route::Small || generic(m.route);
        split_level = (!sh_pair.empty() || !sh_dbl.empty()) && has_other && g16.empty();
        if (!split_level) return;
        side_stream = aux_stream_of(s);
        HIPCHK(hipEventRecord(s->ev_fork, main_stream)); HIPCHK(hipStreamWaitEvent(side_stream, s->ev_fork, 0));
        s->pool->set_defer(true);
    }
    void join() { if (split_level) { HIPCHK(hipEventRecord(s->ev_join, side_stream)); HIPCHK(hipStreamWaitEvent(main_stream, s->ev_join, 0)); } }

    void launch_products() {
        if (!sh_pair.empty()) {
            const int wgs = plan_pair(sh_pair.data(), (int)sh_pair.size());
            const PairItem* d = upload(s, sh_pair);
            ProfScope ps(s, TNQS_PROF_BP_PAIR, 2.0 * sh_pair_slices * 16384.0 * esz, 2 * 8.0 * sh_pair_slices * 16384.0 * 32);
            launch_mfma_pair(s->stream, d, (int)sh_pair.size(), wgs);
        }
        on_side(true);
        run_chains<T>(s, chains, TNQS_PROF_BP_MODEPROD, TNQS_PROF_BP_PAIR);
        on_side(false);
        if (u.cache_on) for (auto& kv : continued) if (!chains[kv.first].trail.empty()) u.remember(chains[kv.first], s->site[chains[kv.first].v], kv.second.base, kv.second.absorbed);
        for (size_t i = 0; i < chains.size(); ++i) {
            GramJob j{}; j.X = chains[i].result; j.Y = chains[i].y ? chains[i].y : chains[i].src; j.sd = chains[i].sd; j.leg = msgs[i].jo; j.keep_site = false;
            j.M = msgs[i].fused;
            jobs.push_back(j);
        }
    }
    void launch_small_sites() {
        if (small_items.empty()) return;
        size_t slab_bytes = 0;
        for (size_t q = 0; q < small_items.size(); ++q) { const int co = small_items[q].chi[small_items[q].jo]; slab_bytes += round256((size_t)co * co * esz); }
        Buf slab = dalloc(s, slab_bytes); size_t off = 0;
        for (size_t q = 0; q < small_items.size(); ++q) {
            GramJob& j = jobs[small_msg[q]];
            const int co = small_items[q].chi[small_items[q].jo];
            j.nchunks = 1; j.KK = co; j.partial = sub_buffer(slab, off, (size_t)co * co * esz); off += round256((size_t)co * co * esz);
            small_items[q].out = j.partial->p;
        }
        if (!s->sharded() && !plan.in_place) {
            size_t nb_bytes = 0;
            for (size_t q = 0; q < small_items.size(); ++q) if (small_items[q].mfma) nb_bytes += round256((size_t)256 * esz);
            if (nb_bytes) {
                Buf nslab = dalloc(s, nb_bytes); size_t noff = 0;
                for (size_t q = 0; q < small_items.size(); ++q) {
                    SmallMsgItem& si = small_items[q]; if (!si.mfma) continue;
                    GramJob& j = jobs[small_msg[q]];
                    const int t = msgs[small_msg[q]].t; const int de = plan.seq[t];
                    j.final_msg = sub_buffer(nslab, noff, (size_t)256 * esz); noff += round256((size_t)256 * esz);
                    si.new_msg = j.final_msg->p; si.old_msg = u.cur[de] ? u.cur[de]->p : nullptr;
                    si.diff_out = reinterpret_cast<double*>(u.d_diffs->p) + t; si.normalize = u.normalize;
                }
            }
        }
        on_side(true);
        const SmallMsgItem* d = upload_small(s, small_items);
        { ProfScope ps(s, TNQS_PROF_BP_FUSED, 0, 0); launch_bp_small_site(s->stream, d, (int)small_items.size(), small_max); }
        on_side(false);
    }
    template <class Item, class PlanFn, class LaunchFn>
    void launch_pair32_singles(std::vector<Item>& items, void* Item::*partial, const std::vector<int>& of_msg, double slices, PlanFn plan_fn, LaunchFn launch_fn) {
        std::vector<int> nwg(items.size()); const int wgs = plan_fn(items.data(), (int)items.size(), nwg.data(), 0);
        for (size_t q = 0; q < items.size(); ++q) {
            GramJob& j = jobs[of_msg[q]];
            j.nchunks = nwg[q]; j.KK = 32; j.partial = dalloc(s, (size_t)j.nchunks * 1024 * esz);
            items[q].*partial = j.partial->p;
        }
        const Item* d = upload(s, items);
        ProfScope ps(s, TNQS_PROF_BP_PAIRGRAM, 2.0 * slices * 16384.0 * esz, 2 * 8.0 * slices * 16384.0 * 32);
        launch_fn(s->stream, d, (int)items.size(), wgs);
    }
    void launch_plane_grams() {
        if (!sh_dbl.empty()) {
            std::vector<int> nwg(sh_dbl.size()); const int wgs = plan_pair_gram2(sh_dbl.data(), (int)sh_dbl.size(), nwg.data());
            for (size_t q = 0; q < sh_dbl.size(); ++q) {
                PairGram2Item& it = sh_dbl[q]; GramJob& jy = jobs[sh_dbl_msg[q].first]; GramJob& jx = jobs[sh_dbl_msg[q].second];
                jy.nchunks = jx.nchunks = nwg[q]; jy.KK = jx.KK = 32;
                jy.partial = dalloc(s, (size_t)jy.nchunks * 1024 * esz); jx.partial = dalloc(s, (size_t)jx.nchunks * 1024 * esz);
                it.partial_y = jy.partial->p; it.partial_x = jx.partial->p;
            }
            const PairGram2Item* d = upload(s, sh_dbl);
            ProfScope ps(s, TNQS_PROF_BP_PAIRGRAM, 2.0 * sh_dbl_slices * 8192.0 * esz, 4 * 8.0 * sh_dbl_slices * 8192.0 * 32);
            launch_mfma_pair_gram2(s->stream, d, (int)sh_dbl.size(), wgs);
        }
        for (int q : g16_single) g16[q].X = chains[g16_msg[q].first].result;
        if (!g16.empty()) {
            std::vector<int> nwgs(g16.size()); const int wgs = plan_pair_gram2x16(g16.data(), (int)g16.size(), nwgs.data()); double by = 0, fl = 0;
            for (size_t q = 0; q < g16.size(); ++q) {
                PairGram2x16Item& it = g16[q]; GramJob& jy = jobs[g16_msg[q].first]; const int nwg = nwgs[q];
                jy.nchunks = nwg; jy.KK = 16; jy.partial = dalloc(s, (size_t)nwg * 256 * esz); it.partial_y = jy.partial->p;
                if (g16_msg[q].second >= 0) {
                    GramJob& jx = jobs[g16_msg[q].second];
                    jx.nchunks = nwg; jx.KK = 16; jx.partial = dalloc(s, (size_t)nwg * 256 * esz); it.partial_x = jx.partial->p;
                } else it.partial_x = nullptr;
                by += 2.0 * jy.sd.n * esz; fl += (g16_msg[q].second >= 0 ? 4 : 2) * 8.0 * jy.sd.n * 16;
            }
            const PairGram2x16Item* d = upload(s, g16);
            ProfScope ps(s, TNQS_PROF_BP_PAIRGRAM, by, fl);
            launch_mfma_pair_gram2x16(s->stream, d, (int)g16.size(), wgs);
        }
// ... 138 lines not shown
```

### tensornetworkquantumsimulator.jl_amd/csrc/engine_core.cpp

```cpp
#include "engine_internal.hpp"

namespace tnqs {

double HostTimer::acc[16] = {0}; long HostTimer::cnt[16] = {0};
static struct HostTimerReport { ~HostTimerReport() { if (envflag("TNQS_HOST_TIMING")) for (int k = 0; k < 16; ++k) if (HostTimer::cnt[k])
    std::fprintf(stderr, "[tnqs host timing] phase %d: %.2f ms total, %ld calls, %.1f us each\n", k, HostTimer::acc[k], HostTimer::cnt[k], 1e3 * HostTimer::acc[k] / HostTimer::cnt[k]); } } g_host_timer_report;

void hipchk(hipError_t e, const char* what) {
    if (e != hipSuccess) throw Err(TNQS_ERR_HIP, std::string(what) + ": " + hipGetErrorString(e));
}
void throw_unsupported(const char* what) { throw Err(TNQS_ERR_UNSUPPORTED, what); }

static size_t round_size(size_t b) {
    if (b < 256) return 256;
    if (b <= (1u << 20)) return (b + 255) & ~size_t(255);
    size_t p = size_t(1) << (63 - __builtin_clzll(b));
    size_t step = p >> 3;
    return (b + step - 1) / step * step;
}
Pool::~Pool() { set_defer(false); trim(); }
void Pool::trim() {
    std::lock_guard<std::mutex> lk(mu_);
    for (auto& kv : free_) for (void* p : kv.second) (void)hipFree(p);
    free_.clear(); cached_ = 0;
// ... 93 lines not shown
    if (ar.base) { (void)hipHostFree(ar.base); ar.base = nullptr; }
}
void recycle_arena(HostArena ar) {
    if (!ar.base) return;
    { std::lock_guard<std::mutex> lk(g_recycle_mu); if (g_spare_arenas.size() < kMaxSpares) { ar.off = 0; ar.ring_off = 0; g_spare_arenas.push_back(ar); ar.base = nullptr; } }
    if (ar.base) arena_free(ar);
}
static hipStream_t acquire_stream(int device, int hi = 0) {
    {
        std::lock_guard<std::mutex> lk(g_recycle_mu);
        for (size_t i = 0; i < g_spare_streams.size(); ++i)
            if (g_spare_streams[i].device == device && g_spare_streams[i].hi == hi) { hipStream_t st = g_spare_streams[i].st; g_spare_streams.erase(g_spare_streams.begin() + (std::ptrdiff_t)i); return st; }
    }
    hipStream_t st = nullptr;
    if (hi) { int least = 0, greatest = 0; HIPCHK(hipDeviceGetStreamPriorityRange(&least, &greatest)); HIPCHK(hipStreamCreateWithPriority(&st, hipStreamNonBlocking, greatest)); }
    else HIPCHK(hipStreamCreateWithFlags(&st, hipStreamNonBlocking));
    return st;
}

State::~State() {
    if (own_stream && stream) (void)hipStreamSynchronize(stream);
    if (aux_stream) (void)hipStreamSynchronize(aux_stream);
    keepalive.clear(); site.clear(); msg.clear();
    HostArena ar = arena; arena = HostArena{};
    SpareStream st[2] = {{device, 0, (own_stream && stream) ? stream : nullptr}, {device, 0, aux_stream}};
    {
        std::lock_guard<std::mutex> lk(g_recycle_mu);
        if (ar.base && g_spare_arenas.size() < kMaxSpares) { ar.off = 0; g_spare_arenas.push_back(ar); ar.base = nullptr; }
        for (auto& q : st) if (q.st && g_spare_streams.size() < kMaxSpares) { g_spare_streams.push_back(q); q.st = nullptr; }
    }
    if (ar.base) arena_free(ar);
    for (auto& q : st) if (q.st) (void)hipStreamDestroy(q.st);
    for (hipEvent_t e : {ev_fork, ev_join}) if (e) (void)hipEventDestroy(e);
}
hipStream_t aux_stream_of(State* s) {
    if (!s->aux_stream) {
        s->aux_stream = acquire_stream(s->device);
        HIPCHK(hipEventCreateWithFlags(&s->ev_fork, hipEventDisableTiming));
        HIPCHK(hipEventCreateWithFlags(&s->ev_join, hipEventDisableTiming));
    }
    return s->aux_stream;
}
void sync(State* s) {
    HIPCHK(hipStreamSynchronize(s->stream));
    s->keepalive.clear(); s->keep_mark = 0;
    s->arena.off = 0;
    if (s->prof) s->prof->chain = false;
}

void prof_collect(State* s) {
    Prof& P = *s->prof;
    if (P.pending.empty()) return;
    HIPCHK(hipStreamSynchronize(s->stream));
    for (auto& p : P.pending) {
        float ms = 0; (void)hipEventElapsedTime(&ms, p.a, p.b);
        P.cls[p.cls].ms += ms;
    }
    for (auto& p : P.pending) { if (p.own_a) P.ev_free.push_back(p.a); P.ev_free.push_back(p.b); }
    P.pending.clear(); P.last_b = nullptr; P.chain = false;
}

int64_t state_site_size(const State* s, int v) { return (int64_t)site_dims(s, v).n; }

template <class T> static void fill_product_up(State* s, int v) {
    std::vector<T> h(2 * s->d[v], T(0)); h[0] = T(1);
    Buf b = dalloc(s, s->d[v] * s->esz());
    HIPCHK(hipMemcpyAsync(b->p, h.data(), s->d[v] * s->esz(), hipMemcpyHostToDevice, s->stream));
    HIPCHK(hipStreamSynchronize(s->stream));
    s->site[v] = b;
}

State* state_create(int nv, int ne, const int32_t* es, const int32_t* ed, const int32_t* sd, int dtype, int device) {
    if (nv <= 0 || ne < 0) throw Err(TNQS_ERR_INVALID, "tnqs_create: nv must be > 0 and ne >= 0");
    if (dtype != TNQS_C64 && dtype != TNQS_C128 && dtype != TNQS_F32 && dtype != TNQS_F64) throw Err(TNQS_ERR_INVALID, "tnqs_create: unknown dtype");
    const bool real_io = (dtype == TNQS_F32 || dtype == TNQS_F64);
    if (dtype == TNQS_F32) dtype = TNQS_C64; else if (dtype == TNQS_F64) dtype = TNQS_C128;
    int ndev = 0;
    if (hipGetDeviceCount(&ndev) != hipSuccess || ndev <= 0) throw Err(TNQS_ERR_HIP, "tnqs_create: no HIP device available (the HIP path has no CPU fallback)");
    if (device < 0 || device >= ndev) throw Err(TNQS_ERR_INVALID, "tnqs_create: bad device index");
    HIPCHK(hipSetDevice(device));
    auto s = std::make_unique<State>();
    s->g = make_graph(nv, ne, es, ed);
    s->dtype = dtype; s->real_io = real_io; s->device = device;
    s->d.assign(nv, 2);
    if (sd) for (int v = 0; v < nv; ++v) { if (sd[v] < 1 || sd[v] > 16) throw Err(TNQS_ERR_INVALID, "tnqs_create: site dimension out of range"); s->d[v] = sd[v]; }
    s->chi.assign(ne, 1);
    s->site.resize(nv); s->sscale.assign(nv, nullptr); s->msg.assign(2 * (size_t)ne, nullptr);
    s->pend1.assign(nv, {}); s->unit_norm.assign(nv, 0); s->projected.assign(nv, 0);
    s->pool = std::make_shared<Pool>(device);
    s->prof = std::make_shared<Prof>();
    s->stream = acquire_stream(device); s->own_stream = true;
    for (int v = 0; v < nv; ++v) { if (dtype == TNQS_C64) fill_product_up<float>(s.get(), v); else fill_product_up<double>(s.get(), v); }
    return s.release();
}

State* state_copy(const State* o) {
    auto s = std::make_unique<State>();
    s->g = o->g; s->dtype = o->dtype; s->real_io = o->real_io; s->device = o->device; s->d = o->d; s->chi = o->chi;
    s->site = o->site; s->sscale = o->sscale; s->msg = o->msg; s->pool = o->pool; s->prof = o->prof;
    s->pend1 = o->pend1; s->unit_norm = o->unit_norm; s->projected = o->projected;
    s->rank = o->rank; s->nranks = o->nranks; s->owner = o->owner; s->ag_fn = o->ag_fn; s->ag_ctx = o->ag_ctx;
    s->exch = o->exch; s->exch_bytes = o->exch_bytes; s->comm = o->comm; s->force_exchange = o->force_exchange; s->msg_hermitian = o->msg_hermitian;
    HIPCHK(hipSetDevice(o->device));
    if (o->own_stream) { HIPCHK(hipStreamSynchronize(o->stream)); s->stream = acquire_stream(o->device); s->own_stream = true; }
    else { s->stream = o->stream; s->own_stream = false; }
    return s.release();
}

template <class T> static void permute_dispatch(State* s, const PermItem& it) { launch_permute<T>(s->stream, it); }

static std::vector<char> widen_real(const State* s, const void* host, size_t n) {
    std::vector<char> out(n * s->esz());
    if (s->dtype == TNQS_C64) { const float* p = static_cast<const float*>(host); float* q = reinterpret_cast<float*>(out.data()); for (size_t i = 0; i < n; ++i) { q[2 * i] = p[i]; q[2 * i + 1] = 0.f; } }
    else { const double* p = static_cast<const double*>(host); double* q = reinterpret_cast<double*>(out.data()); for (size_t i = 0; i < n; ++i) { q[2 * i] = p[i]; q[2 * i + 1] = 0.0; } }
    return out;
}
static void narrow_real(const State* s, const std::vector<char>& cplx, void* host, size_t n) {
    bool bad = false;
    if (s->dtype == TNQS_C64) { const float* q = reinterpret_cast<const float*>(cplx.data()); float* p = static_cast<float*>(host); for (size_t i = 0; i < n; ++i) { p[i] = q[2 * i]; bad = bad || q[2 * i + 1] != 0.f; } }
    else { const double* q = reinterpret_cast<const double*>(cplx.data()); double* p = static_cast<double*>(host); for (size_t i = 0; i < n; ++i) { p[i] = q[2 * i]; bad = bad || q[2 * i + 1] != 0.0; } }
    if (bad) throw Err(TNQS_ERR_NUMERIC, "internal: a real-typed handle holds a non-zero imaginary part");
}

void state_set_site(State* s, int v, const void* host, int ndim, const int64_t* dims, const int32_t* role) {
    const Graph& g = *s->g;
    if (v < 0 || v >= g.nv) throw Err(TNQS_ERR_INVALID, "set_site_tensor: bad vertex");
    const int z = (int)g.nbr[v].size();
    if (ndim != z + 1 || ndim > 8) throw Err(TNQS_ERR_INVALID, "set_site_tensor: tensor must have one site leg and one leg per neighbour (<= 7 neighbours)");
    std::vector<int> canon_of(ndim, -1); std::vector<int> src_of(ndim, -1);
    for (int k = 0; k < ndim; ++k) {
        int c;
        if (role[k] < 0) c = 0;
        else { int j = g.leg(v, role[k]); if (j < 0) throw Err(TNQS_ERR_INVALID, "set_site_tensor: leg_role names a non-neighbour"); c = 1 + j; }
        if (src_of[c] >= 0) throw Err(TNQS_ERR_INVALID, "set_site_tensor: duplicate leg role");
        canon_of[k] = c; src_of[c] = k;
    }
    if (dims[src_of[0]] != s->d[v]) throw Err(TNQS_ERR_INVALID, "set_site_tensor: site dimension mismatch");
    size_t n = 1; std::vector<long long> stride_caller(ndim);
    for (int k = 0; k < ndim; ++k) { stride_caller[k] = (long long)n; if (dims[k] < 1) throw Err(TNQS_ERR_INVALID, "set_site_tensor: bad dim"); n *= (size_t)dims[k]; }
    HIPCHK(hipSetDevice(s->device));
    s->pend1[v].clear(); s->unit_norm[v] = 0;
    if (!s->owns(v)) {
        s->site[v] = nullptr; s->sscale[v] = nullptr;
        for (int j = 0; j < z; ++j) {
            int e = g.nbr_e[v][j]; int c = (int)dims[src_of[1 + j]];
            if (s->chi[e] != c) { s->chi[e] = c; s->msg[2 * e] = nullptr; s->msg[2 * e + 1] = nullptr; }
        }
        return;
    }
    if (!host) throw Err(TNQS_ERR_INVALID, "set_site_tensor: null data for an owned vertex");
    Buf raw = dalloc(s, n * s->esz());
    std::vector<char> widened; if (s->real_io) { widened = widen_real(s, host, n); host = widened.data(); }
    HIPCHK(hipMemcpyAsync(raw->p, host, n * s->esz(), hipMemcpyHostToDevice, s->stream));
    Buf out = dalloc(s, n * s->esz());
    PermItem it{}; it.in = raw->p; it.out = out->p; it.ndim = ndim; it.n = n;
    for (int c = 0; c < ndim; ++c) { it.dims_out[c] = (int)dims[src_of[c]]; it.stride_in[c] = stride_caller[src_of[c]]; }
    if (s->dtype == TNQS_C64) permute_dispatch<float>(s, it); else permute_dispatch<double>(s, it);
    HIPCHK(hipStreamSynchronize(s->stream));
    s->site[v] = out; s->sscale[v] = nullptr;
    for (int j = 0; j < z; ++j) {
        int e = g.nbr_e[v][j]; int c = it.dims_out[1 + j];
        if (s->chi[e] != c) { s->chi[e] = c; s->msg[2 * e] = nullptr; s->msg[2 * e + 1] = nullptr; }
    }
}

void state_set_site_random(State* s, int v, int nn, const int64_t* bond_dims, uint64_t seed, double scale) {
    const Graph& g = *s->g;
    if (v < 0 || v >= g.nv) throw Err(TNQS_ERR_INVALID, "set_site_random: bad vertex");
    const int z = (int)g.nbr[v].size();
    if (nn != z) throw Err(TNQS_ERR_INVALID, "set_site_random: one bond dimension per neighbour expected");
    size_t n = (size_t)s->d[v];
    for (int j = 0; j < z; ++j) { if (bond_dims[j] < 1 || bond_dims[j] > 4096) throw Err(TNQS_ERR_INVALID, "set_site_random: bad bond dimension"); n *= (size_t)bond_dims[j]; }
    HIPCHK(hipSetDevice(s->device));
    s->pend1[v].clear(); s->unit_norm[v] = 0;
    if (s->owns(v)) {
        Buf out = dalloc(s, n * s->esz());
        const unsigned long long sd = seed * 0x9E3779B97F4A7C15ull + (unsigned long long)v * 0xC2B2AE3D27D4EB4Full;
        if (s->dtype == TNQS_C64) launch_random_fill<float>(s->stream, out->p, n, sd, scale, s->real_io); else launch_random_fill<double>(s->stream, out->p, n, sd, scale, s->real_io);
        HIPCHK(hipStreamSynchronize(s->stream));
        s->site[v] = out; s->sscale[v] = nullptr;
    } else { s->site[v] = nullptr; s->sscale[v] = nullptr; }
// ... 81 lines not shown
```

### tensornetworkquantumsimulator.jl_amd/csrc/engine_internal.hpp

```cpp
#pragma once
#include "engine.hpp"
#include "kernels.hpp"
#include <algorithm>
#include <array>
#include <chrono>
#include <climits>
#include <cmath>
#include <complex>
#include <cstdio>
#include <cstdlib>
#include <cstring>
#include <functional>
#include <limits>
#include <memory>
#include <mutex>
#include <numeric>
#include <set>
#include <type_traits>
#include <unordered_map>

namespace tnqs {

#define HIPCHK(x) hipchk((x), #x)

// ... 2 lines not shown
TNQS_SWITCH(use_mfma, !envflag("TNQS_NO_MFMA"))
TNQS_SWITCH(use_pair, !envflag("TNQS_NO_PAIR"))
TNQS_SWITCH(use_bra_products, !envflag("TNQS_NO_BRA_PRODUCTS"))
TNQS_SWITCH(use_prodcache, !envflag("TNQS_NO_PRODCACHE"))
TNQS_SWITCH(use_chol, !envflag("TNQS_NO_CHOL"))
TNQS_SWITCH(use_qr2, !envflag("TNQS_NO_QR2"))
TNQS_SWITCH(use_lowrank, !envflag("TNQS_NO_LOWRANK"))
TNQS_SWITCH(use_precond_svd, !envflag("TNQS_NO_PRECOND_SVD"))
TNQS_SWITCH(use_small_svd, !envflag("TNQS_NO_SMALLSVD"))
TNQS_SWITCH(defer_site1, !envflag("TNQS_NO_DEFER_1SITE"))
TNQS_SWITCH(use_chi64, !envflag("TNQS_NO_CHI64"))
TNQS_SWITCH(speculation_on, !envflag("TNQS_NO_SPECULATION"))
#undef TNQS_SWITCH
inline size_t bp_cache_budget() { static const size_t v = [] { const char* e = std::getenv("TNQS_BP_CACHE_MB"); return (e ? (size_t)std::atoll(e) : (size_t)49152) << 20; }(); return v; }
inline size_t bp_ws_budget() { static const size_t v = [] { const char* e = std::getenv("TNQS_BP_WS_MB"); return (e ? (size_t)std::atoll(e) : (size_t)24576) << 20; }(); return v; }
inline size_t jacobi_lds(size_t bytes) { static const bool g = envflag("TNQS_JACOBI_GLOBAL"); return (g || bytes > 160 * 1024 - 2048) ? 0 : bytes; }
inline int mmax_of(const std::vector<JacobiItem>& ji) { int m = 1; for (auto& j : ji) m = std::max(m, std::max(j.m, j.n)); return m; }

struct HostTimer {
    static double acc[16]; static long cnt[16];
    int k; std::chrono::steady_clock::time_point t0; bool on;
    explicit HostTimer(int kk) : k(kk), t0(std::chrono::steady_clock::now()), on(true) {}
    void stop() { if (on) { static std::mutex mu; std::lock_guard<std::mutex> lk(mu); acc[k] += std::chrono::duration<double, std::milli>(std::chrono::steady_clock::now() - t0).count(); cnt[k]++; on = false; } }
    ~HostTimer() { stop(); }
};

void sync(State* s);
hipStream_t aux_stream_of(State* s);
void recycle_arena(HostArena ar);
HostArena acquire_arena();
inline void drain_for_arena_reuse(State* s) {
    HIPCHK(hipStreamSynchronize(s->stream));
    if (s->aux_stream && s->aux_stream != s->stream) HIPCHK(hipStreamSynchronize(s->aux_stream));
}
template <class X> const X* readback(State* s, const void* dsrc, size_t count) {
    const size_t bytes = count * sizeof(X);
    HostArena& ar = s->arena;
    if (!ar.base) ar = acquire_arena();
    const size_t aligned = (std::max<size_t>(bytes, 1) + 255) & ~size_t(255);
    if (aligned > ar.cap) throw Err(TNQS_ERR_UNSUPPORTED, "read-back too large for the staging arena");
    if (ar.off + aligned > ar.cap) { drain_for_arena_reuse(s); ar.off = 0; }
    char* h = ar.base + ar.off; ar.off += aligned;
    if (bytes) HIPCHK(hipMemcpyAsync(h, dsrc, bytes, hipMemcpyDeviceToHost, s->stream));
    return reinterpret_cast<const X*>(h);
}
inline void reserve_readback(State* s, size_t bytes) {
    HostArena& ar = s->arena;
    if (!ar.base) ar = acquire_arena();
    if (bytes > ar.cap) throw Err(TNQS_ERR_UNSUPPORTED, "read-backs of one batch too large for the staging arena");
    if (ar.off + bytes > ar.cap) { drain_for_arena_reuse(s); ar.off = 0; }
}
inline void soft_sync(State* s) { s->keep_mark = s->keepalive.size(); }
inline void drained(State* s) {
    s->prof->chain = false;
    s->arena.off = 0;
    if (s->keep_mark) { s->keepalive.erase(s->keepalive.begin(), s->keepalive.begin() + (std::ptrdiff_t)std::min(s->keep_mark, s->keepalive.size())); s->keep_mark = 0; }
}
void materialize_scale(State* s, const std::vector<int>& verts);
void materialize_scale_all(State* s);
void materialize_pending(State* s, const std::vector<int>& verts);
void materialize_pending_all(State* s);
inline Buf dalloc(State* s, size_t bytes) {
    auto b = std::make_shared<DevBuf>();
    b->pool = s->pool; b->bytes = bytes;
    b->p = s->pool->alloc(bytes ? bytes : 1, &b->rounded);
    return b;
}
template <class Item> const Item* upload(State* s, const std::vector<Item>& v) {
    if (v.empty()) return nullptr;
    size_t bytes = v.size() * sizeof(Item);
    HostArena& ar = s->arena;
    if (!ar.base) ar = acquire_arena();
    size_t aligned = (bytes + 255) & ~size_t(255);
    if (aligned > ar.cap) throw Err(TNQS_ERR_UNSUPPORTED, "descriptor batch too large");
    if (ar.off + aligned > ar.cap) { drain_for_arena_reuse(s); ar.off = 0; s->prof->chain = false; }
    char* h = ar.base + ar.off; ar.off += aligned;
    std::memcpy(h, v.data(), bytes);
    Buf b = dalloc(s, bytes);
    HIPCHK(hipMemcpyAsync(b->p, h, bytes, hipMemcpyHostToDevice, s->stream));
    s->keepalive.push_back(b);
    return reinterpret_cast<const Item*>(b->p);
}

template <class Item> const Item* upload_small(State* s, const std::vector<Item>& v) {
    if (v.empty()) return nullptr;
    const size_t bytes = v.size() * sizeof(Item);
    HostArena& ar = s->arena;
    if (!ar.base) ar = acquire_arena();
    const size_t aligned = (bytes + 255) & ~size_t(255);
    if (aligned > ar.cap) throw Err(TNQS_ERR_UNSUPPORTED, "descriptor batch too large");
    if (ar.off + aligned > ar.cap) { drain_for_arena_reuse(s); ar.off = 0; s->prof->chain = false; }
    char* h = ar.base + ar.off; ar.off += aligned;
    std::memcpy(h, v.data(), bytes);
    return reinterpret_cast<const Item*>(h);
}

struct ProfScope {
    State* s; int cls; hipEvent_t a = nullptr, b = nullptr; bool own_a = true;
    ProfScope(State* st, int c, double bytes, double flops) : s(st), cls(c) {
        Prof& P = *s->prof;
        if (!P.on) return;
        P.cls[c].bytes += bytes; P.cls[c].flops += flops; P.cls[c].launches += 1;
        auto get = [&]() { hipEvent_t e; if (!P.ev_free.empty()) { e = P.ev_free.back(); P.ev_free.pop_back(); } else HIPCHK(hipEventCreate(&e)); return e; };
        if (P.chain && P.last_b && P.last_stream == s->stream) { a = P.last_b; own_a = false; }
        else { a = get(); own_a = true; HIPCHK(hipEventRecord(a, s->stream)); }
        b = get();
    }
    ~ProfScope() {
        if (!a) return;
        Prof& P = *s->prof;
        (void)hipEventRecord(b, s->stream);
        P.pending.push_back({cls, a, b, own_a});
        P.last_b = b; P.chain = true; P.last_stream = s->stream;
    }
};

struct PhaseScope {
    State* s; int cls; hipEvent_t a = nullptr, b = nullptr; long count = 1;
    PhaseScope(State* st, int c) : s(st), cls(c) {
        Prof& P = *s->prof;
        if (!P.on) return;
        auto get = [&]() { hipEvent_t e; if (!P.ev_free.empty()) { e = P.ev_free.back(); P.ev_free.pop_back(); } else HIPCHK(hipEventCreate(&e)); return e; };
        a = get(); b = get();
        HIPCHK(hipEventRecord(a, s->stream));
    }
    ~PhaseScope() {
        if (!a) return;
        Prof& P = *s->prof;
        (void)hipEventRecord(b, s->stream);
        P.cls[cls].launches += count;
        P.pending.push_back({cls, a, b, true});
    }
};

struct ChiVec {
    int inl[8]; int n = 0; std::vector<int> big;
    void push_back(int c) { if (n < 8 && big.empty()) inl[n++] = c; else { if (big.empty()) big.assign(inl, inl + n); big.push_back(c); ++n; } }
    int* data() { return big.empty() ? inl : big.data(); }
    const int* data() const { return big.empty() ? inl : big.data(); }
    int& operator[](size_t i) { return data()[i]; }
    const int& operator[](size_t i) const { return data()[i]; }
    size_t size() const { return (size_t)n; }
    bool empty() const { return n == 0; }
    const int* begin() const { return data(); }
    const int* end() const { return data() + n; }
};
struct SD {
    int z = 0, d = 1; ChiVec chi; size_t n = 1;
    size_t pre(int j) const { size_t p = d; for (int i = 0; i < j; ++i) p *= chi[i]; return p; }
    size_t post(int j) const { size_t p = 1; for (int i = j + 1; i < z; ++i) p *= chi[i]; return p; }
};
inline SD site_dims(const State* s, int v) {
    SD r; const Graph& g = *s->g;
    r.z = (int)g.nbr[v].size(); r.d = s->d[v]; r.n = r.d;
    for (int j = 0; j < r.z; ++j) { int c = s->chi[g.nbr_e[v][j]]; r.chi.push_back(c); r.n *= c; }
    return r;
}

inline size_t site_nelem(const State* s, int v) { size_t n = (size_t)s->d[v]; for (int e : s->g->nbr_e[v]) n *= (size_t)s->chi[e]; return n; }
inline size_t round256(size_t b) { return (b + 255) & ~size_t(255); }
void exchange(State* s, size_t bytes_per_rank);
void check_exchange(const State* s, size_t bytes_per_rank);



struct Chain {
// ... 93 lines not shown
```

### tensornetworkquantumsimulator.jl_amd/csrc/kernels.hpp

```cpp
#pragma once
#include <algorithm>
#include <cstdlib>
#include <hip/hip_runtime_api.h>
#include <cstddef>
#include <cstdint>
#include <vector>

namespace tnqs {

struct FiberItem {
    const void* in; void* out; const void* X;
    int D, PA, K, PB;
    int Do, No;
    int TA, TB, nta, ntb;
    int tile_begin;
    int tpw;
    int want_norm;
};

struct GramItem {
    const void* X; const void* Y; void* partial;
    int D, PA, K, PB;
    int TA, TB, nta, ntb;
    int chunk_begin, nchunks, tiles_per_chunk;
// ... 208 lines not shown
int plan_loop_trace(LoopTraceItem* it, int n);
template <class T> void launch_loop_trace(hipStream_t s, const LoopTraceItem* d_items, int nitems, int total_wgs);
void launch_site1_c64(hipStream_t s, const Site1Item* d_items, int nitems, int nbx, double* d_norm_partials);

struct PairGeom { long long cstr, sx, sy, t0, t1, t2; int n0, n1, n2; };
struct PairItem {
    const void* in; void* out; const void* Mx; const void* My;
    PairGeom g;
    int slice_begin;
    int spw;
};
struct PairGramItem {
    const void* X; const void* Y; const void* M; void* partial;
    PairGeom g;
    int wg_begin;
    int spw;
};

struct PlaneGeom { long long cstr, sx, sy, t0, t1, t2, t3; int n0, n1, n2, n3; int nslices() const { return n0 * n1 * n2 * n3; } };
inline bool plane_geometry(int d, int z, const int* chi, int lx, int ly, int DIM, PlaneGeom& g) {
    if (lx == ly || lx < 0 || ly < 0 || lx >= z || ly >= z || chi[lx] != DIM || chi[ly] != DIM) return false;
    auto pre = [&](int j) { long long p = d; for (int i = 0; i < j; ++i) p *= chi[i]; return p; };
    const int p = lx < ly ? lx : ly, q = lx < ly ? ly : lx;
    g.sx = pre(lx); g.sy = pre(ly);
    g.n1 = g.n2 = g.n3 = 1; g.t1 = g.t2 = g.t3 = 0;
    if (pre(p) % 16 == 0) {
        g.cstr = 2; g.n0 = (int)(pre(p) / 16); g.t0 = 16;
        g.n1 = (int)(pre(q) / (pre(p) * DIM)); g.t1 = pre(p) * DIM;
        long long post = 1; for (int i = q + 1; i < z; ++i) post *= chi[i];
        g.n2 = (int)post; g.t2 = pre(q) * DIM;
        return true;
    }
    if (pre(p) != 2) return false;
    int a = -1;
    for (int i = 0; i < z; ++i) if (i != p && i != q && chi[i] % 8 == 0) { a = i; break; }
    if (a < 0) return false;
    g.cstr = pre(a); g.n0 = chi[a] / 8; g.t0 = 8 * pre(a);
    int k = 0;
    for (int i = 0; i < z; ++i) {
        if (i == p || i == q || i == a) continue;
        if (k == 0) { g.n1 = chi[i]; g.t1 = pre(i); } else if (k == 1) { g.n2 = chi[i]; g.t2 = pre(i); } else if (k == 2) { g.n3 = chi[i]; g.t3 = pre(i); } else return false;
        ++k;
    }
    return true;
}
inline bool pair_geometry(int d, int z, const int* chi, int lx, int ly, PairGeom& g) {
    PlaneGeom p;
    if (!plane_geometry(d, z, chi, lx, ly, 32, p) || p.t3 != 0) return false;
    g = PairGeom{p.cstr, p.sx, p.sy, p.t0, p.t1, p.t2, p.n0, p.n1, p.n2};
    return true;
}
struct Pair16Item {
    const void* in; void* out; const void* Mx; const void* My;
    PlaneGeom g;
    int wg_begin;
    int spw;
};
struct PairGram2x16Item { const void* X; const void* Y; const void* Mx; const void* My; void* partial_y; void* partial_x; PlaneGeom g; int wg_begin; int spw; };
bool pair16_whole_lines(const PlaneGeom& g);
void plan_pair16(Pair16Item* it, int n, int wgs[2], int spw = 0);
void launch_mfma_pair16(hipStream_t s, const Pair16Item* d_items, int nitems, int total_wgs, bool whole_lines);
int pair_gram2x16_slices_at_a_time();
int plan_pair_gram2x16(PairGram2x16Item* it, int n, int* nwg = nullptr, int spw = 0);
void launch_mfma_pair_gram2x16(hipStream_t s, const PairGram2x16Item* d_items, int nitems, int total_wgs);

int mfma_fiber_tile_rows(int KK, int NN);
void launch_mfma_fiber_gemm(hipStream_t s, const FiberItem* d_items, int nitems, int total_tiles, int KKmax, int NNmax,
                            double* d_norm_partials);
bool launch_mfma_gram32(hipStream_t s, const GramItem* d_items, int nitems, int total_chunks, int KKmax);
bool launch_mfma_gram64(hipStream_t s, const GramItem* d_items, int nitems, int total_chunks, int KKmax);
void launch_mfma_gram32_fused(hipStream_t s, const GramItem* d_items, int nitems, int total_chunks);
bool launch_mfma_gram64_f64(hipStream_t s, const GramItem* d_items, int nitems, int total_chunks, int KKmax, bool all_kk64 = false);
bool fiber_gemm_f64_covers(const FiberItem& it);
int plan_fiber_gemm_f64(FiberItem* it, int n, int* nwg = nullptr, int tpw = 0);
void launch_mfma_fiber_gemm_f64(hipStream_t s, const FiberItem* d_items, int nitems, int total_wgs, int Kmax, int Nmax, double* d_norm_partials, bool general);
bool gram_f64in_covers(int D, int K);
void launch_mfma_gram_f64in(hipStream_t s, const GramItem* d_items, int nitems, int total_chunks);
bool gauge_gram64_covers(int d, int z, const int* chi, int bleg, int rleg);
bool gauge_gram32_covers(int d, int z, const int* chi, int bleg, int rleg);
int gauge_gram32_units(int z, const int* chi, int bleg);
void launch_mfma_gauge_gram32(hipStream_t s, const GramItem* d_items, int nitems, int total_chunks);
void launch_mfma_gauge_gram64(hipStream_t s, const GramItem* d_items, int nitems, int total_chunks);
bool launch_mfma_gram128_f64(hipStream_t s, const GramItem* d_items, int nitems, int total_chunks, int KKmax, bool all_kk128 = false);
int plan_pair(PairItem* it, int n, int spw = 0);
void launch_mfma_pair(hipStream_t s, const PairItem* d_items, int nitems, int total_wgs);
void launch_x3_pair(hipStream_t s, const PairItem* d_items, int nitems, int total_wgs);
struct PairGram2Item { const void* X; const void* Y; const void* Mx; const void* My; void* partial_y; void* partial_x; PairGeom g; int wg_begin; int spw; };
int plan_pair_gram2(PairGram2Item* it, int n, int* nwg = nullptr, int spw = 0);
void launch_mfma_pair_gram2(hipStream_t s, const PairGram2Item* d_items, int nitems, int total_wgs);
void launch_x3_pair_gram2(hipStream_t s, const PairGram2Item* d_items, int nitems, int total_wgs);
int plan_x3_pair_gram1(PairGram2Item* it, int n, int* nwg = nullptr, int spw = 0);
void launch_x3_pair_gram1(hipStream_t s, const PairGram2Item* d_items, int nitems, int total_wgs);
int plan_pair_gram(PairGramItem* it, int n, int* nwg = nullptr, int spw = 0);
void launch_mfma_pair_gram(hipStream_t s, const PairGramItem* d_items, int nitems, int total_wgs);

}
```

### tensornetworkquantumsimulator.jl_amd/csrc/kernels_mfma.hip

```cpp
#include "kernels.hpp"
#include "mfma_common.hpp"
#include <stdexcept>
#include <type_traits>
#include "launch_util.hpp"

namespace tnqs {

template <int KB, int NB, int NU>
__global__ __launch_bounds__(256) void mfma_fiber_gemm_w_kernel(const FiberItem* __restrict__ items, int nitems,
                                                                double* __restrict__ norm_partials) {
    constexpr int KKP = 32 * KB, NNP = 32 * NB;
    constexpr int CP = (KKP > NNP ? KKP : NNP);
    constexpr int PT = CP + 1, PX = KKP + 1;
    extern __shared__ __attribute__((aligned(16))) char smem[];
    float* Xt_re = reinterpret_cast<float*>(smem);
    float* Xt_im = Xt_re + NNP * PX;
    const int tid = threadIdx.x, lane = tid & 63, w = tid >> 6, ln = lane & 31, h = lane >> 5;
    float* At_re = Xt_im + NNP * PX + w * (2 * 32 * PT);
    float* At_im = At_re + 32 * PT;
    __shared__ double sh_red[4];
    const int gw = blockIdx.x;
    const int lo = find_item(items, nitems, &FiberItem::tile_begin, gw);
    const FiberItem it = items[lo];
    const int D = it.D, K = it.K, TA = it.TA, TB = it.TB, KK = D * K;
// ... 403 lines not shown
#pragma unroll
        for (int q = 0; q < 16; q += 4) {
            const v4f u = ldg4(My + 2 * q + 4 * h), v = ldg4(My + 2 * q + 4 * h + 2);
            myr[q] = u[0]; myi[q] = u[1]; myr[q + 1] = u[2]; myi[q + 1] = u[3]; myr[q + 2] = v[0]; myi[q + 2] = v[1]; myr[q + 3] = v[2]; myi[q + 3] = v[3];
        }
    }
    const int f4 = tid & 3, sg0 = tid >> 2;
    const int ix0 = sg0 & 31, iy0 = sg0 >> 5;
    const long long toff = (long long)(4 * half + f4) * g.cstr + g.sx * ix0 + g.sy * iy0, tstr = 4 * g.sy;
    v2f* const lbase = L + (2 * f4) * PS + iy0 * 33 + ix0;
    v4f pre[8];
    auto commit = [&](int buf) {
#pragma unroll
        for (int j = 0; j < 8; ++j) {
            v2f* p0 = lbase + buf * BUF + 132 * j;
            v2f a; a[0] = pre[j][0]; a[1] = pre[j][1]; v2f b; b[0] = pre[j][2]; b[1] = pre[j][3];
            p0[0] = a; p0[PS] = b;
        }
    };
    auto store1 = [&](int buf, long long ob, int j) {
        const v2f* p0 = lbase + buf * BUF + 132 * j;
        const v2f a = p0[0], c = p0[PS];
        v4f v; v[0] = a[0]; v[1] = a[1]; v[2] = c[0]; v[3] = c[1];
        stg4(out + ob + tstr * j, v);
    };
    if (s_begin < s_end) {
        const long long b = pair_slice_base(g, s_begin) + toff;
#pragma unroll
        for (int j = 0; j < 8; ++j) pre[j] = ldg4(in + b + tstr * j);
        commit(0);
    }
    lds_barrier();
    for (int sl = s_begin; sl < s_end; ++sl) {
        const int buf = (sl - s_begin) & 1;
        const bool more = sl + 1 < s_end, prev = sl > s_begin;
        const long long nb = pair_slice_base(g, more ? sl + 1 : sl) + toff;
        const long long ob = pair_slice_base(g, prev ? sl - 1 : sl) + toff;
        v2f* P = L + buf * BUF + w * PS;
        v2f xc[4], xn[4];
#pragma unroll
        for (int i = 0; i < 4; ++i) xc[i] = P[ln * 33 + i + 16 * h];
        CAcc32<true> Y;
#pragma unroll
        for (int c4 = 0; c4 < 4; ++c4) {
            if (c4 < 3) {
#pragma unroll
                for (int i = 0; i < 4; ++i) xn[i] = P[ln * 33 + 4 * (c4 + 1) + i + 16 * h];
            }
            TNQS_PIN();
#pragma unroll
            for (int i = 0; i < 4; ++i) {
                const int q = 4 * c4 + i;
                const float br = mxr[q], bi = mxi[q];
                if (q == 0) Y.template mac_bpre<true>(xc[i][0], xc[i][1], br, bi - br, br + bi);
                else Y.template mac_bpre<false>(xc[i][0], xc[i][1], br, bi - br, br + bi);
                if ((q & 1) == 0) { pre[q >> 1] = ldg4(in + nb + tstr * (q >> 1)); TNQS_PIN(); }
            }
#pragma unroll
            for (int i = 0; i < 4; ++i) xc[i] = xn[i];
        }
        CAcc32<true> S;
#pragma unroll
        for (int r = 0; r < 16; ++r) {
            const float br = myr[r], bi = myi[r];
            if (r == 0) S.template mac_bpre<true>(Y.re(r), Y.im(r), br, bi - br, br + bi);
            else S.template mac_bpre<false>(Y.re(r), Y.im(r), br, bi - br, br + bi);
            if ((r & 1) == 0) { if (prev) store1(buf ^ 1, ob, r >> 1); TNQS_PIN(); }
        }
        S.finish();
#pragma unroll
        for (int r = 0; r < 16; ++r) { const int jx = (r & 3) + 8 * (r >> 2) + 4 * h; v2f v; v[0] = S.a[r]; v[1] = S.b[r]; P[ln * 33 + jx] = v; }
        if (more) commit(buf ^ 1);
        lds_barrier();
    }
    if (s_begin < s_end) {
        const int buf = (s_end - 1 - s_begin) & 1;
        const long long ob = pair_slice_base(g, s_end - 1) + toff;
#pragma unroll
        for (int j = 0; j < 8; ++j) store1(buf, ob, j);
    }
    #undef TNQS_PIN
}
static int pair_slices(const PairGeom& g) { return g.n0 * g.n1 * g.n2; }
int plan_pair(PairItem* it, int n, int spw) {
    if (spw <= 0) {
        double tot = 0; for (int i = 0; i < n; ++i) tot += pair_slices(it[i].g); spw = 16; while (spw > 1 && 2.0 * tot / spw < 1024.0) spw >>= 1;
    }
    return lay_out(it, n, &PairItem::slice_begin, nullptr, [&](PairItem& p) { p.spw = spw; const int np = (pair_slices(p.g) + spw - 1) / spw; return 16 * ((np + 7) / 8); });
}
void launch_mfma_pair(hipStream_t s, const PairItem* d_items, int nitems, int total_wgs) {
    if (total_wgs <= 0) return;
    if (mfma_use_x3()) { launch_x3_pair(s, d_items, nitems, total_wgs); return; }
    const size_t lds = (size_t)16 * (32 * 33 + 4) * 2 * sizeof(float);
    set_max_dynamic_lds((const void*)mfma_pair_kernel, lds); hipLaunchKernelGGL(mfma_pair_kernel, dim3(total_wgs), dim3(512), lds, s, d_items, nitems);
    TNQS_CHECK_LAUNCH();
}

__global__ __launch_bounds__(512) void mfma_pair_gram_kernel(const PairGramItem* __restrict__ items, int nitems) {
    constexpr int PS = 32 * 33 + 1;
    extern __shared__ __attribute__((aligned(16))) char smem[];
    v2f* L = reinterpret_cast<v2f*>(smem);
    const int tid = threadIdx.x, lane = tid & 63, w = tid >> 6, ln = lane & 31, h = lane >> 5;
    const int gw = blockIdx.x;
    const int lo = find_item(items, nitems, &PairGramItem::wg_begin, gw);
    const PairGramItem it = items[lo];
    const PairGeom g = it.g;
    const int nslices = g.n0 * g.n1 * g.n2;
    const int lw = gw - it.wg_begin;
    const int s_begin = lw * it.spw, s_end = min(nslices, s_begin + it.spw);
    const cf* __restrict__ Xg = reinterpret_cast<const cf*>(it.X);
    const cf* __restrict__ Yg = reinterpret_cast<const cf*>(it.Y);
    const cf* __restrict__ Mg = reinterpret_cast<const cf*>(it.M);
    float mr[16], mi[16];
#pragma unroll
    for (int q = 0; q < 16; ++q) { cf v = Mg[(q + 16 * h) + 32 * ln]; mr[q] = v.re; mi[q] = v.im; }
    v16f Or, Oi;
#pragma unroll
    for (int r = 0; r < 16; ++r) { Or[r] = 0.f; Oi[r] = 0.f; }
    const int f = tid & 7, sg0 = tid >> 3;
    const long long sx = g.sx, sy = g.sy, fo = (long long)f * g.cstr;
    v4f pre[16];
    const int ix0 = sg0 & 31, iy0 = sg0 >> 5;
    const long long toff = fo + sx * ix0 + sy * iy0, tstr = 2 * sy;
    v2f* const lbase = L + (2 * f) * PS + iy0 * 33 + ix0;
    auto issue = [&](const cf* __restrict__ G, int sl) {
        const cf* p = G + pair_slice_base(g, sl) + toff;
#pragma unroll
        for (int j = 0; j < 16; ++j) pre[j] = ldg4(p + tstr * j);
    };
    auto commit = [&]() {
#pragma unroll
        for (int j = 0; j < 16; ++j) {
            v2f* p0 = lbase + 66 * j;
            v2f a; a[0] = pre[j][0]; a[1] = pre[j][1]; v2f b; b[0] = pre[j][2]; b[1] = pre[j][3];
            p0[0] = a; p0[PS] = b;
        }
    };

    if (s_begin < s_end) issue(Xg, s_begin);
    for (int sl = s_begin; sl < s_end; ++sl) {
        lds_barrier();
        commit();
        lds_barrier();
        issue(Yg, sl);
        v16f C1r[2], C1i[2];
#pragma unroll
        for (int pp = 0; pp < 2; ++pp) {
            const v2f* P = L + (w + 8 * pp) * PS;
            float xr[16], xi[16];
#pragma unroll
            for (int q = 0; q < 16; ++q) { v2f v = P[ln * 33 + q + 16 * h]; xr[q] = v[0]; xi[q] = v[1]; }
#pragma unroll
            for (int r = 0; r < 16; ++r) { C1r[pp][r] = 0.f; C1i[pp][r] = 0.f; }
#pragma unroll
            for (int q = 0; q < 16; ++q) {
                C1r[pp] = __builtin_amdgcn_mfma_f32_32x32x2f32(mr[q], xr[q], C1r[pp], 0, 0, 0);
                C1r[pp] = __builtin_amdgcn_mfma_f32_32x32x2f32(-mi[q], xi[q], C1r[pp], 0, 0, 0);
                C1i[pp] = __builtin_amdgcn_mfma_f32_32x32x2f32(mr[q], xi[q], C1i[pp], 0, 0, 0);
                C1i[pp] = __builtin_amdgcn_mfma_f32_32x32x2f32(mi[q], xr[q], C1i[pp], 0, 0, 0);
            }
        }
        lds_barrier();
        commit();
        lds_barrier();
        if (sl + 1 < s_end) issue(Xg, sl + 1);
#pragma unroll
        for (int pp = 0; pp < 2; ++pp) {
            const v2f* P = L + (w + 8 * pp) * PS;
            float yr[16], yi[16];
#pragma unroll
            for (int r = 0; r < 16; ++r) { int jx = (r & 3) + 8 * (r >> 2) + 4 * h; v2f v = P[ln * 33 + jx]; yr[r] = v[0]; yi[r] = v[1]; }
#pragma unroll
            for (int r = 0; r < 16; ++r) {
                Or = __builtin_amdgcn_mfma_f32_32x32x2f32(C1r[pp][r], yr[r], Or, 0, 0, 0);
                Or = __builtin_amdgcn_mfma_f32_32x32x2f32(C1i[pp][r], yi[r], Or, 0, 0, 0);
// ... 416 lines not shown
```

### tensornetworkquantumsimulator.jl_amd/csrc/kernels_x3.hip

```cpp
#include <type_traits>
#include "kernels.hpp"
#include "mfma_common.hpp"
#include "launch_util.hpp"
#include "x3_common.hpp"

namespace tnqs {

__device__ __forceinline__ long long x3_slice_base(const PairGeom& g, int sl) {
    int a0 = sl % g.n0; int r1 = sl / g.n0; int a1 = r1 % g.n1; int a2 = r1 / g.n1;
    return (long long)a0 * g.t0 + (long long)a1 * g.t1 + (long long)a2 * g.t2;
}

template <bool SINGLE>
__global__ __launch_bounds__(512) __attribute__((amdgpu_waves_per_eu(2, 2))) void x3_pair_gram2_kernel(const PairGram2Item* __restrict__ items, int nitems) {
    constexpr int P = 34;
    constexpr int PS = 32 * P + 2;
    #define TNQS_PIN() __builtin_amdgcn_sched_barrier(0x2 | 0x4)
    extern __shared__ __attribute__((aligned(16))) char smem[];
    v2f* L = reinterpret_cast<v2f*>(smem);
    const int tid = threadIdx.x, lane = tid & 63, w = tid >> 6, ln = lane & 31, h = lane >> 5;
    const int gw = blockIdx.x;
    const int lo = find_item(items, nitems, &PairGram2Item::wg_begin, gw);
    const PairGram2Item it = items[lo];
    const PairGeom g = it.g;
// ... 90 lines not shown
                for (int j = 4; j < 6; ++j) { px[j] = ldg4(Xg + nb + tstr * j); py[j] = ldg4(Yg + nb + tstr * j); }
            }
            TNQS_PIN();
            {
                float cr[8], ci[8];
#pragma unroll
                for (int e = 0; e < 8; ++e) { cr[e] = Cr[e]; ci[e] = Ci[e]; }
                const P3 pcr = split8(cr), pci = split8(ci), yr = split8(ar), yi = split8(ai);
                mac6x2<false>(Or, pcr, yr, Oi, pci, yr);
                mac6x2<false>(Or, pci, yi, Oi, neg(pcr), yi);
            }
            if (t == 0) {
#pragma unroll
                for (int j = 6; j < 8; ++j) { px[j] = ldg4(Xg + nb + tstr * j); py[j] = ldg4(Yg + nb + tstr * j); }
            }
            if (t == 0 && !SINGLE) read8(L + (comp + 4) * PS, 8 * h, 8 * h + 4, ar, ai);
            TNQS_PIN();
            {
                float cr[8], ci[8];
#pragma unroll
                for (int e = 0; e < 8; ++e) { cr[e] = Cr[8 + e]; ci[e] = Ci[8 + e]; }
                const P3 pcr = split8(cr), pci = split8(ci), yr = split8(br), yi = split8(bi);
                mac6x2<false>(Or, pcr, yr, Oi, pci, yr);
                mac6x2<false>(Or, pci, yi, Oi, neg(pcr), yi);
            }
        }
        TNQS_PIN();
        lds_barrier();
        if (more) commit();
        lds_barrier();
    }
    };
    if (SINGLE || msg == 0) run(std::integral_constant<int, 0>{}); else run(std::integral_constant<int, 1>{});
    cf* __restrict__ p1 = reinterpret_cast<cf*>(it.partial_y) + (size_t)lw * 1024;
    cf* __restrict__ p2 = reinterpret_cast<cf*>(it.partial_x) + (size_t)lw * 1024;
    v2f* const R = L;
#pragma unroll
    for (int r = 0; r < 16; ++r) {
        const int i = (r & 3) + 8 * (r >> 2) + 4 * h;
        v2f v; v[0] = Or[r]; v[1] = Oi[r];
        R[w * (32 * 33) + ln * 33 + i] = v;
    }
    lds_barrier();
    if (SINGLE) {
        for (int e = tid; e < 1024; e += 512) {
            const int i = e & 31, j = e >> 5;
            float sr = 0.f, si = 0.f;
#pragma unroll
            for (int ww = 0; ww < 8; ++ww) { const v2f v = R[ww * (32 * 33) + j * 33 + i]; sr += v[0]; si += v[1]; }
            cf o; o.re = sr; o.im = si; stgc(p1 + e, o);
        }
        return;
    }
    for (int e = tid; e < 2048; e += 512) {
        const int mm = e >> 10, ee = e & 1023, i = ee & 31, j = ee >> 5;
        float sr = 0.f, si = 0.f;
#pragma unroll
        for (int ww = 0; ww < 4; ++ww) { const v2f v = R[(4 * mm + ww) * (32 * 33) + j * 33 + i]; sr += v[0]; si += v[1]; }
        cf o; o.re = sr; o.im = si; stgc((mm ? p2 : p1) + ee, o);
    }
}
#undef TNQS_PIN
int x3_pair_gram2_group() { return 16; }
int plan_x3_pair_gram1(PairGram2Item* it, int n, int* nwg, int spw) {
    auto slices = [](const PairGram2Item& p) { return p.g.n0 * p.g.n1 * p.g.n2; };
    if (spw <= 0) { double tot = 0; for (int i = 0; i < n; ++i) tot += (double)slices(it[i]); spw = 16; while (spw > 1 && 2.0 * tot / spw < 1024.0) spw >>= 1; }
    return lay_out(it, n, &PairGram2Item::wg_begin, nwg, [&](PairGram2Item& p) { p.spw = spw; const int np = (slices(p) + spw - 1) / spw; return 16 * ((np + 7) / 8); });
}
void launch_x3_pair_gram1(hipStream_t s, const PairGram2Item* d_items, int nitems, int total_wgs) {
    if (total_wgs <= 0) return;
    const size_t lds = (size_t)16 * (32 * 34 + 2) * 2 * sizeof(float);
    set_max_dynamic_lds((const void*)x3_pair_gram2_kernel<true>, lds);
    hipLaunchKernelGGL((x3_pair_gram2_kernel<true>), dim3(total_wgs), dim3(512), lds, s, d_items, nitems);
    TNQS_CHECK_LAUNCH();
}
void launch_x3_pair_gram2(hipStream_t s, const PairGram2Item* d_items, int nitems, int total_wgs) {
    if (total_wgs <= 0) return;
    const size_t lds = (size_t)16 * (32 * 34 + 2) * 2 * sizeof(float);
    set_max_dynamic_lds((const void*)x3_pair_gram2_kernel<false>, lds);
    hipLaunchKernelGGL(x3_pair_gram2_kernel<false>, dim3(total_wgs), dim3(512), lds, s, d_items, nitems);
    TNQS_CHECK_LAUNCH();
}

__global__ __launch_bounds__(512) __attribute__((amdgpu_waves_per_eu(2, 2))) void x3_pair_kernel(const PairItem* __restrict__ items, int nitems) {
    constexpr int P = 34;
    constexpr int PS = 32 * P + 2;
    constexpr int BUF = 8 * PS;
    extern __shared__ __attribute__((aligned(16))) char smem[];
    v2f* L = reinterpret_cast<v2f*>(smem);
    const int tid = threadIdx.x, lane = tid & 63, w = tid >> 6, ln = lane & 31, h = lane >> 5;
    const int gw = blockIdx.x;
    const int lo = find_item(items, nitems, &PairItem::slice_begin, gw);
    const PairItem it = items[lo];
    const PairGeom g = it.g;
    const int nslices = g.n0 * g.n1 * g.n2;
    const int lw = gw - it.slice_begin;
    const int half = (lw >> 3) & 1, pw = ((lw >> 4) << 3) | (lw & 7);
    const int s_begin = pw * it.spw, s_end = min(nslices, s_begin + it.spw);
    const cf* __restrict__ in = reinterpret_cast<const cf*>(it.in);
    cf* __restrict__ out = reinterpret_cast<cf*>(it.out);
    P3 Mxr[2], Mxi[2];
    u4* const MyL = reinterpret_cast<u4*>(L + 16 * PS) + lane;
    {
        const cf* __restrict__ Mx = reinterpret_cast<const cf*>(it.Mx) + 32 * ln; const cf* __restrict__ My = reinterpret_cast<const cf*>(it.My) + 32 * ln;
#pragma unroll
        for (int n = 0; n < 2; ++n) {
            float xr[8], xi[8];
#pragma unroll
            for (int e = 0; e < 8; e += 2) { const v4f v = ldg4(Mx + 16 * n + 8 * h + e); xr[e] = v[0]; xi[e] = v[1]; xr[e + 1] = v[2]; xi[e + 1] = v[3]; }
            Mxr[n] = split8(xr); Mxi[n] = split8(xi);
#pragma unroll
            for (int e = 0; e < 8; e += 2) { const v4f v = ldg4(My + 4 * h + 16 * n + 8 * (e >> 2) + (e & 3)); xr[e] = v[0]; xi[e] = v[1]; xr[e + 1] = v[2]; xi[e + 1] = v[3]; }
            const P3 yr_ = split8(xr), yi_ = split8(xi);
            if (w == 0) { MyL[(6 * n + 0) * 64] = yr_.h; MyL[(6 * n + 1) * 64] = yr_.m; MyL[(6 * n + 2) * 64] = yr_.l; MyL[(6 * n + 3) * 64] = yi_.h; MyL[(6 * n + 4) * 64] = yi_.m; MyL[(6 * n + 5) * 64] = yi_.l; }
        }
    }
    const int f4 = tid & 3, sg0 = tid >> 2;
    const int ix0 = sg0 & 31, iy0 = sg0 >> 5;
    const long long toff = (long long)(4 * half + f4) * g.cstr + g.sx * ix0 + g.sy * iy0, tstr = 4 * g.sy;
    v2f* const lbase = L + (2 * f4) * PS + iy0 * P + ix0;
    v4f preA[8], preB[8];
    #define TNQS_PIN() __builtin_amdgcn_sched_barrier(0x2 | 0x4)
    auto commit = [&](int buf, const v4f (&pre)[8]) {
#pragma unroll
        for (int j = 0; j < 8; ++j) {
            v2f* p0 = lbase + buf * BUF + 4 * P * j;
            v2f a; a[0] = pre[j][0]; a[1] = pre[j][1]; v2f b; b[0] = pre[j][2]; b[1] = pre[j][3];
            p0[0] = a; p0[PS] = b;
        }
    };
    auto store1 = [&](int buf, long long ob, int j) {
        const v2f* p0 = lbase + buf * BUF + 4 * P * j;
        const v2f a = p0[0], c = p0[PS];
        v4f v; v[0] = a[0]; v[1] = a[1]; v[2] = c[0]; v[3] = c[1];
        stg4(out + ob + tstr * j, v);
    };
    if (s_begin < s_end) {
        const long long b = x3_slice_base(g, s_begin) + toff;
#pragma unroll
        for (int j = 0; j < 8; ++j) preB[j] = ldg4(in + b + tstr * j);
        const long long b1 = x3_slice_base(g, s_begin + 1 < s_end ? s_begin + 1 : s_begin) + toff;
#pragma unroll
        for (int j = 0; j < 8; ++j) preA[j] = ldg4(in + b1 + tstr * j);
        commit(0, preB);
    }
    lds_barrier();
    auto phase = [&](int sl, int buf, const v4f (&cur)[8], v4f (&nxt)[8]) {
        const bool more = sl + 1 < s_end, prev = sl > s_begin;
        const long long nb = x3_slice_base(g, sl + 2 < s_end ? sl + 2 : sl) + toff;
        const long long ob = x3_slice_base(g, prev ? sl - 1 : sl) + toff;
        v2f* Pw = L + buf * BUF + w * PS;
        v16f Yr, Yi;
#pragma unroll
        for (int n = 0; n < 2; ++n) {
            float ar[8], ai[8];
            const v4f* a = reinterpret_cast<const v4f*>(Pw + ln * P + 16 * n + 8 * h);
#pragma unroll
            for (int q = 0; q < 4; ++q) { const v4f v = a[q]; ar[2 * q] = v[0]; ai[2 * q] = v[1]; ar[2 * q + 1] = v[2]; ai[2 * q + 1] = v[3]; }
#pragma unroll
            for (int j = 0; j < 4; ++j) nxt[4 * n + j] = ldg4(in + nb + tstr * (4 * n + j));
            TNQS_PIN();
            const P3 sr = split8(ar), si = split8(ai), nsi = neg(si);
            if (n == 0) mac6x2<true>(Yr, sr, Mxr[n], Yi, sr, Mxi[n]); else mac6x2<false>(Yr, sr, Mxr[n], Yi, sr, Mxi[n]);
            mac6x2<false>(Yr, nsi, Mxi[n], Yi, si, Mxr[n]);
        }
        v16f Sr, Si;
#pragma unroll
        for (int n = 0; n < 2; ++n) {
            float yr[8], yi[8];
#pragma unroll
            for (int e = 0; e < 8; ++e) { yr[e] = Yr[8 * n + e]; yi[e] = Yi[8 * n + e]; }
            const P3 pr = split8(yr), pi = split8(yi), npi = neg(pi);
            if (prev) {
#pragma unroll
                for (int j = 0; j < 4; ++j) store1(buf ^ 1, ob, 4 * n + j);
            }
            P3 myr, myi;
            myr.h = MyL[(6 * n + 0) * 64]; myr.m = MyL[(6 * n + 1) * 64]; myr.l = MyL[(6 * n + 2) * 64]; myi.h = MyL[(6 * n + 3) * 64]; myi.m = MyL[(6 * n + 4) * 64]; myi.l = MyL[(6 * n + 5) * 64];
            TNQS_PIN();
            if (n == 0) mac6x2<true>(Sr, pr, myr, Si, pr, myi); else mac6x2<false>(Sr, pr, myr, Si, pr, myi);
            mac6x2<false>(Sr, npi, myi, Si, pi, myr);
        }
        TNQS_PIN();
#pragma unroll
        for (int r = 0; r < 16; r += 2) { const int jx = (r & 3) + 8 * (r >> 2) + 4 * h; v4f v; v[0] = Sr[r]; v[1] = Si[r]; v[2] = Sr[r + 1]; v[3] = Si[r + 1]; *reinterpret_cast<v4f*>(Pw + ln * P + jx) = v; }
        if (more) commit(buf ^ 1, cur);
        lds_barrier();
    };
    for (int sl = s_begin; sl < s_end; sl += 2) {
        phase(sl, 0, preA, preB);
        if (sl + 1 < s_end) phase(sl + 1, 1, preB, preA);
    }
    if (s_begin < s_end) {
        const int buf = (s_end - 1 - s_begin) & 1;
        const long long ob = x3_slice_base(g, s_end - 1) + toff;
#pragma unroll
        for (int j = 0; j < 8; ++j) store1(buf, ob, j);
    }
    #undef TNQS_PIN
}
void launch_x3_pair(hipStream_t s, const PairItem* d_items, int nitems, int total_wgs) {
    if (total_wgs <= 0) return;
    const size_t lds = (size_t)16 * (32 * 34 + 2) * 2 * sizeof(float) + 12 * 64 * 16;
    set_max_dynamic_lds((const void*)x3_pair_kernel, lds);
    hipLaunchKernelGGL(x3_pair_kernel, dim3(total_wgs), dim3(512), lds, s, d_items, nitems);
    TNQS_CHECK_LAUNCH();
}

template <int D>
__global__ __launch_bounds__(256, 2) void x3_rowgemm64_kernel(const FiberItem* __restrict__ items, int nitems, double* __restrict__ norm_partials) {
    constexpr int KK = 64;
    extern __shared__ __attribute__((aligned(16))) char smem[];
    u4* const Xl = reinterpret_cast<u4*>(smem);
    __shared__ double sh_red[4];
    const int tid = threadIdx.x, lane = tid & 63, w = tid >> 6, ln = lane & 31, h = lane >> 5;
    const int gw = blockIdx.x;
    const int lo = find_item(items, nitems, &FiberItem::tile_begin, gw);
    const FiberItem it = items[lo];
    const int K = it.K, No = it.No, NN = it.Do * No;
    const long long PA = it.PA;
    const int ntiles = it.nta * it.ntb;
    const int t_begin = (gw - it.tile_begin) * it.tpw, t_end = min(ntiles, t_begin + it.tpw);
    const cf* __restrict__ in = reinterpret_cast<const cf*>(it.in);
    const cf* __restrict__ X = reinterpret_cast<const cf*>(it.X);
    cf* __restrict__ out = reinterpret_cast<cf*>(it.out);
    for (int e = tid; e < 4 * 2 * 64; e += 256) {
        const int l = e & 63, nb = (e >> 6) & 1, n = e >> 7;
        const int nn = 32 * nb + (l & 31), kk0 = 16 * n + 8 * (l >> 5);
        float xr[8], xi[8];
#pragma unroll
        for (int q = 0; q < 8; q += 2) {
            v4f v = {0.f, 0.f, 0.f, 0.f};
            if (nn < NN) v = ldg4(X + kk0 + q + (size_t)KK * nn);
            xr[q] = v[0]; xi[q] = v[1]; xr[q + 1] = v[2]; xi[q + 1] = v[3];
        }
        const P3 pr = split8(xr), pi = split8(xi);
        u4* d = Xl + (size_t)((2 * n + nb) * 6) * 64 + l;
        d[0] = pr.h; d[64] = pr.m; d[128] = pr.l; d[192] = pi.h; d[256] = pi.m; d[320] = pi.l;
    }
    __syncthreads();
    float hb[2][32];
    const bool rows_b = PA < 32;
    const int RB = rows_b ? 32 / (int)PA : 1;
    const long long kst = (long long)D * PA;
    const long long lane_in = rows_b ? (long long)D * (ln % (int)PA) + kst * K * (ln / (int)PA) : (long long)D * ln;
    const long long lane_out = rows_b ? (long long)D * (ln % (int)PA) + kst * No * (ln / (int)PA) : (long long)D * ln;
    auto base_in = [&](int t) { return rows_b ? kst * K * RB * t : (long long)D * 32 * (t % it.nta) + kst * K * (t / it.nta); };
    auto base_out = [&](int t) { return rows_b ? kst * No * RB * t : (long long)D * 32 * (t % it.nta) + kst * No * (t / it.nta); };
    const unsigned voff = (unsigned)((lane_in + kst * (D == 1 ? 8 : 4) * h) * (long long)sizeof(cf));
    auto issue_half = [&](int t, int hf) {
        const cf* pu = in + base_in(t);
#pragma unroll
        for (int nn2 = 0; nn2 < 2; ++nn2) {
            const int n = 2 * hf + nn2;
            if (D == 1) {
#pragma unroll
                for (int e = 0; e < 8; ++e) { const v2f v = ldg2(reinterpret_cast<const char*>(pu + kst * (16 * n + e)) + voff); hb[hf][16 * nn2 + e] = v[0]; hb[hf][16 * nn2 + 8 + e] = v[1]; }
            } else {
#pragma unroll
                for (int j = 0; j < 4; ++j) { const v4f v = ldg4(reinterpret_cast<const char*>(pu + kst * (8 * n + j)) + voff);
                                              hb[hf][16 * nn2 + 2 * j] = v[0]; hb[hf][16 * nn2 + 8 + 2 * j] = v[1]; hb[hf][16 * nn2 + 2 * j + 1] = v[2]; hb[hf][16 * nn2 + 8 + 2 * j + 1] = v[3]; }
            }
        }
    };
    double nrm = 0;
    int t = t_begin + w;
    if (t < t_end) { issue_half(t, 0); issue_half(t, 1); }
    for (; t < t_end; t += 4) {
        v16f Cr[2], Ci[2];
#pragma unroll
        for (int hf = 0; hf < 2; ++hf) {
#pragma unroll
            for (int nn2 = 0; nn2 < 2; ++nn2) {
                const int n = 2 * hf + nn2;
                float br[8], bi[8];
#pragma unroll
                for (int e = 0; e < 8; ++e) { br[e] = hb[hf][16 * nn2 + e]; bi[e] = hb[hf][16 * nn2 + 8 + e]; }
                const P3 pbr = split8(br), pbi = split8(bi), nbi = neg(pbi);
#pragma unroll
                for (int nb = 0; nb < 2; ++nb) {
                    const u4* a = Xl + (size_t)((2 * n + nb) * 6) * 64 + lane;
                    P3 xr, xi; xr.h = a[0]; xr.m = a[64]; xr.l = a[128]; xi.h = a[192]; xi.m = a[256]; xi.l = a[320];
                    if (n == 0) mac6x2<true>(Cr[nb], xr, pbr, Ci[nb], xr, pbi); else mac6x2<false>(Cr[nb], xr, pbr, Ci[nb], xr, pbi);
                    mac6x2<false>(Cr[nb], xi, nbi, Ci[nb], xi, pbr);
                }
            }
            __builtin_amdgcn_sched_barrier(0);
            if (t + 4 < t_end) issue_half(t + 4, hf);
// ... 199 lines not shown
```

### tensornetworkquantumsimulator.jl_amd/csrc/launch_util.hpp

```cpp
#pragma once
#include <hip/hip_runtime_api.h>
#include <cstdlib>
#include <map>
#include <mutex>
#include <utility>

namespace tnqs {

inline void set_max_dynamic_lds(const void* func, size_t bytes) {
    static std::mutex mu;
    static std::map<std::pair<int, const void*>, size_t> done;
    int dev = 0; (void)hipGetDevice(&dev);
    std::lock_guard<std::mutex> lk(mu);
    auto key = std::make_pair(dev, func);
    auto it = done.find(key);
    if (it != done.end() && it->second >= bytes) return;
    (void)hipFuncSetAttribute(func, hipFuncAttributeMaxDynamicSharedMemorySize, (int)bytes);
    done[key] = bytes;
}


inline bool mfma_use_x3() { static const bool v = [] { const char* e = std::getenv("TNQS_NO_BF16X3"); return !(e && e[0] == '1'); }(); return v; }

}
```

Measured before the change: 6770.

## Replace per-item slice partitioning of x3 pair kernel with a persistent CU-sized plane walk

The bf16x3 pair-product kernel no longer launches a fixed number of workgroups per item with a slices-per-workgroup split. The grid is now sized to k times the CU count, and a host-planned list of shares spreads the total slices evenly across workgroup pairs, so one workgroup can walk across item boundaries. This aims to remove tail imbalance and small-grid underuse when there are many or uneven items. It costs an extra share-array upload per launch, a per-item LDS barrier, and longer serial loops per workgroup that may hide latency less well.

```diff
diff --git a/include/tnqs_debug.h b/include/tnqs_debug.h
--- a/include/tnqs_debug.h
+++ b/include/tnqs_debug.h
@@ -34,6 +34,8 @@
 int tnqs_dbg_pair16(int d, int nitems, const int* z, const int* chi, const int* lx, const int* ly, const void* in, const void* M, void* out, int spw, int* route_out);
 int tnqs_dbg_pair_gram2x16(int d, int nitems, const int* z, const int* chi, const int* lx, const int* ly, const int* both, const void* X, const void* Y, const void* M,
                            void* out_y, void* out_x, int spw);
+int tnqs_dbg_plane_walk(int nitems, const int* slices, int cus, int k, int grid, int* grid_out, int* wgs_out, int cap);
+int tnqs_dbg_pair_walk(int nitems, const int* lx, const int* ly, const void* in, const void* M, void* out, int grid, int k);
 int tnqs_dbg_svd_tall(int nitems, const int* m, const int* n, void* A, int* chol_fail, int* polished, int* sweeps);
 int tnqs_dbg_small_site(int nitems, const int* d, const int* z, const int* chi, const int* jo, const void* psi, const void* M, const int* present, int form,
                         const void* old_msg, const int* has_old, int normalize, void* out, void* new_msg, double* diff_out, int* route_out);
diff --git a/profiles/walk_bench.py b/profiles/walk_bench.py
--- /dev/null
+++ b/profiles/walk_bench.py
@@ -0,0 +1,34 @@
+import ctypes as C
+import os
+import sys
+
+here = os.path.dirname(os.path.abspath(__file__))
+mode = sys.argv[1] if len(sys.argv) > 1 else "walk"
+lib = C.CDLL(sys.argv[2] if len(sys.argv) > 2 else os.path.join(here, "..", "tensornetworkquantumsimulator.jl_amd", "libtnqs_hip.so"))
+lib.tnqs_dbg_bench_plane.argtypes = [C.c_int, C.c_int, C.c_int, C.c_int, C.c_int, C.POINTER(C.c_double)]
+SITES = (16, 17, 32, 33, 100, 324)
+
+
+def run(which, nsites, key, val):
+    os.environ[key] = str(val)
+    vals = []
+    for _ in range(3):
+        ms = C.c_double(0)
+        rc = lib.tnqs_dbg_bench_plane(which, nsites, 1, 2, 10 if nsites < 200 else 4, C.byref(ms))
+        if rc != 0:
+            sys.exit(f"tnqs_dbg_bench_plane: rc {rc}")
+        vals.append(ms.value)
+    print(f"{mode} which {which} nsites {nsites:4d} {key} {val:3d} ms " + " ".join(f"{v:8.4f}" for v in vals), flush=True)
+
+
+if mode == "spw":
+    for which in ((1,) if os.environ.get("TNQS_NO_BF16X3") != "1" else (0, 1)):
+        for ns in SITES:
+            run(which, ns, "TNQS_DBG_SPW", 16)
+        for ns in (32, 96):
+            for spw in (2, 4, 8, 16):
+                run(which, ns, "TNQS_DBG_SPW", spw)
+else:
+    for k in (1, 2, 4):
+        for ns in SITES:
+            run(0, ns, "TNQS_DBG_WALK_K", k)
diff --git a/tensornetworkquantumsimulator.jl_amd/csrc/api.cpp b/tensornetworkquantumsimulator.jl_amd/csrc/api.cpp
--- a/tensornetworkquantumsimulator.jl_amd/csrc/api.cpp
+++ b/tensornetworkquantumsimulator.jl_amd/csrc/api.cpp
@@ -186,6 +186,7 @@
 
 #include "../../include/tnqs_debug.h"
 #include "kernels.hpp"
+#include "launch_util.hpp"
 namespace tnqs { void dbg_default_sequence(const Graph& g, std::vector<int>& src, std::vector<int>& dst);
                  std::shared_ptr<Graph> dbg_make_graph(int nv, int ne, const int32_t* es, const int32_t* ed);
                  void dbg_default_sequence_graph(const Graph& g, std::vector<int>& src, std::vector<int>& dst, std::vector<int>& level);
@@ -207,6 +208,7 @@
                  void dbg_pair16(int d, int nitems, const int* z, const int* chi, const int* lx, const int* ly, const void* in, const void* M, void* out, int spw, int* route);
                  void dbg_pair_gram2x16(int d, int nitems, const int* z, const int* chi, const int* lx, const int* ly, const int* both, const void* X, const void* Y, const void* M,
                                         void* out_y, void* out_x, int spw);
+                 void dbg_pair_walk(int nitems, const int* lx, const int* ly, const void* in, const void* M, void* out, int grid, int k);
                  void dbg_svd_tall(int nitems, const int* m, const int* n, void* A, int* chol_fail, int* polished, int* sweeps);
                  void dbg_small_site(int nitems, const int* d, const int* z, const int* chi, const int* jo, const void* psi, const void* M, const int* present, int form,
                                      const void* old_msg, const int* has_old, int normalize, void* out, void* new_msg, double* diff, int* route);
@@ -280,6 +282,19 @@
 int tnqs_dbg_gram_mfma(int nitems, const int* shape, const void* X, const void* Y, void* out, int nchunks, int* route_out) {
     return guard([&] { dbg_gram_mfma(nitems, shape, X, Y, out, nchunks, route_out); });
 }
+int tnqs_dbg_plane_walk(int nitems, const int* slices, int cus, int k, int grid, int* grid_out, int* wgs_out, int cap) {
+    return guard([&] { if (nitems < 1 || !slices || !grid_out || cap < 0 || (cap > 0 && !wgs_out)) throw Err(TNQS_ERR_INVALID, "tnqs_dbg_plane_walk: bad arguments");
+                       if (!mfma_use_x3()) throw Err(TNQS_ERR_UNSUPPORTED, "tnqs_dbg_plane_walk: the f32 route (TNQS_NO_BF16X3=1) has no walk");
+                       for (int i = 0; i < nitems; ++i) if (slices[i] < 1) throw Err(TNQS_ERR_INVALID, "tnqs_dbg_plane_walk: an item has at least one slice");
+                       PlaneWalk w; w.cus = cus; w.k = k; w.grid = grid;
+                       std::vector<PairItem> it((size_t)nitems); for (int i = 0; i < nitems; ++i) { it[(size_t)i].g.n0 = slices[i]; it[(size_t)i].g.n1 = it[(size_t)i].g.n2 = 1; }
+                       *grid_out = plan_pair(it.data(), nitems, w);
+                       for (int gw = 0; gw < *grid_out && gw < cap; ++gw) {
+                           const WalkShare& a = w.shares[(size_t)walk_pair_of(gw)]; int* q = wgs_out + 4 * gw; q[0] = a.item; q[1] = a.s_begin; q[2] = a.count; q[3] = walk_half_of(gw); } });
+}
+int tnqs_dbg_pair_walk(int nitems, const int* lx, const int* ly, const void* in, const void* M, void* out, int grid, int k) {
+    return guard([&] { dbg_pair_walk(nitems, lx, ly, in, M, out, grid, k); });
+}
 int tnqs_dbg_pair16(int d, int nitems, const int* z, const int* chi, const int* lx, const int* ly, const void* in, const void* M, void* out, int spw, int* route_out) {
     return guard([&] { dbg_pair16(d, nitems, z, chi, lx, ly, in, M, out, spw, route_out); });
 }
diff --git a/tensornetworkquantumsimulator.jl_amd/csrc/debug.cpp b/tensornetworkquantumsimulator.jl_amd/csrc/debug.cpp
--- a/tensornetworkquantumsimulator.jl_amd/csrc/debug.cpp
+++ b/tensornetworkquantumsimulator.jl_amd/csrc/debug.cpp
@@ -14,6 +14,9 @@
 #define HIPCHK(x) hipchk((x), #x)
 struct DBuf { void* p = nullptr; explicit DBuf(size_t n) { HIPCHK(hipMalloc(&p, n ? n : 1)); } ~DBuf() { (void)hipFree(p); }
               void up(const void* h, size_t n) { HIPCHK(hipMemcpy(p, h, n, hipMemcpyHostToDevice)); } void down(void* h, size_t n) { HIPCHK(hipMemcpy(h, p, n, hipMemcpyDeviceToHost)); } };
+static PlaneWalk dbg_walk(int grid = 0, int k = 0) { PlaneWalk w; int dev = 0; (void)hipGetDevice(&dev); if (hipDeviceGetAttribute(&w.cus, hipDeviceAttributeMultiprocessorCount, dev) != hipSuccess) w.cus = 0; w.grid = grid; w.k = k; return w; }
+struct DWalk { std::unique_ptr<DBuf> b; const WalkShare* p = nullptr;
+               explicit DWalk(const PlaneWalk& w) { if (w.shares.empty()) return; const size_t n = w.shares.size() * sizeof(WalkShare); b.reset(new DBuf(n)); b->up(w.shares.data(), n); p = (const WalkShare*)b->p; } };
 static void need_gpu() { int n = 0; if (hipGetDeviceCount(&n) != hipSuccess || n <= 0) throw Err(TNQS_ERR_HIP, "no HIP device available"); }
 
 void dbg_jacobi(int dtype, int m, int n, void* A, void* V, int* sweeps) {
@@ -182,9 +185,9 @@
     PairItem it{}; it.in = dIn.p; it.out = dOut.p; it.Mx = dX.p; it.My = dY.p;
     it.g.cstr = 2; it.g.sx = C0; it.g.sy = (long long)C0 * 32 * NMID; it.g.n0 = C0 / 16; it.g.t0 = 16; it.g.n1 = NMID; it.g.t1 = (long long)C0 * 32;
     it.g.n2 = NHI; it.g.t2 = (long long)C0 * 32 * NMID * 32;
-    const int wgs = plan_pair(&it, 1, 3);
+    PlaneWalk walk = dbg_walk(); const int wgs = plan_pair(&it, 1, walk, 3); DWalk dW(walk);
     dI.up(&it, sizeof(it));
-    launch_mfma_pair(nullptr, (const PairItem*)dI.p, 1, wgs);
+    launch_mfma_pair(nullptr, (const PairItem*)dI.p, 1, wgs, dW.p);
     HIPCHK(hipDeviceSynchronize());
     dOut.down(out, n * 8);
 }
@@ -198,9 +201,9 @@
     HIPCHK(hipMemset(dOut.p, 0xff, n * 8));
     it.in = dIn.p; it.out = dOut.p; it.Mx = dX.p; it.My = dY.p;
     if ((size_t)it.g.n0 * it.g.n1 * it.g.n2 * 16 * 1024 != n) throw Err(TNQS_ERR_INVALID, "dbg_pair_legs: slice count");
-    const int wgs = plan_pair(&it, 1, 3);
+    PlaneWalk walk = dbg_walk(); const int wgs = plan_pair(&it, 1, walk, 3); DWalk dW(walk);
     dI.up(&it, sizeof(it));
-    launch_mfma_pair(nullptr, (const PairItem*)dI.p, 1, wgs);
+    launch_mfma_pair(nullptr, (const PairItem*)dI.p, 1, wgs, dW.p);
     HIPCHK(hipDeviceSynchronize());
     dOut.down(out, n * 8);
 }
@@ -300,6 +303,7 @@
     (void)hipEventDestroy(e0); (void)hipEventDestroy(e1);
     *ms = (double)t / reps;
 }
+static int dbg_env(const char* name, int dflt) { const char* e = std::getenv(name); const int v = e ? std::atoi(e) : 0; return v > 0 ? v : dflt; }
 void dbg_bench_plane(int which, int nsites, int lx, int ly, int reps, double* ms) {
     need_gpu();
     if (which == 2 || which == 3) { dbg_bench_plane16(which, nsites, lx, ly, reps, ms); return; }
@@ -319,9 +323,11 @@
         std::vector<PairItem> pit(nsites); std::vector<PairGram2Item> git(nsites);
         for (int i = 0; i < nsites; ++i) { pit[i].g = g; git[i].g = g2; }
         std::vector<int> pw(ngroups), gwg(ngroups), nwg(nsites);
+        std::vector<std::unique_ptr<DWalk>> dpw(ngroups);
         for (int gr = 0; gr < ngroups; ++gr) {
             const int cnt = std::min(G, nsites - gr * G);
-            pw[gr] = plan_pair(&pit[(size_t)gr * G], cnt, gr ? pit[0].spw : 0);
+            PlaneWalk wp = dbg_walk();
+            pw[gr] = plan_pair(&pit[(size_t)gr * G], cnt, wp, gr ? pit[0].spw : 0); dpw[gr].reset(new DWalk(wp));
             gwg[gr] = plan_pair_gram2(&git[(size_t)gr * G], cnt, &nwg[(size_t)gr * G], gr ? git[0].spw : 0);
         }
         const int spw_p = pit[0].spw, spw_g = git[0].spw, nwg_g = nwg[0];
@@ -337,7 +343,7 @@
         auto level = [&]() {
             for (int gr = 0; gr < ngroups; ++gr) {
                 const int cnt = std::min(G, nsites - gr * G);
-                launch_mfma_pair(nullptr, (const PairItem*)dPI.p + (size_t)gr * G, cnt, pw[gr]);
+                launch_mfma_pair(nullptr, (const PairItem*)dPI.p + (size_t)gr * G, cnt, pw[gr], dpw[gr]->p);
                 launch_mfma_pair_gram2(nullptr, (const PairGram2Item*)dGI.p + (size_t)gr * G, cnt, gwg[gr]);
             }
         };
@@ -352,16 +358,16 @@
             PairItem& it = items[i]; it.g = g; it.in = (char*)dA.p + (size_t)i * n * 8; it.out = (char*)dB.p + (size_t)i * n * 8;
             it.Mx = dM.p; it.My = (char*)dM.p + 1024 * 8;
         }
-        const int wgs = plan_pair(items.data(), nsites);
+        PlaneWalk walk = dbg_walk(0, dbg_env("TNQS_DBG_WALK_K", 0)); const int wgs = plan_pair(items.data(), nsites, walk, dbg_env("TNQS_DBG_SPW", 0)); DWalk dW(walk);
         DBuf dI(items.size() * sizeof(PairItem)); dI.up(items.data(), items.size() * sizeof(PairItem));
-        launch_mfma_pair(nullptr, (const PairItem*)dI.p, nsites, wgs);
+        launch_mfma_pair(nullptr, (const PairItem*)dI.p, nsites, wgs, dW.p);
         HIPCHK(hipEventRecord(e0, nullptr));
-        for (int r = 0; r < reps; ++r) launch_mfma_pair(nullptr, (const PairItem*)dI.p, nsites, wgs);
+        for (int r = 0; r < reps; ++r) launch_mfma_pair(nullptr, (const PairItem*)dI.p, nsites, wgs, dW.p);
         HIPCHK(hipEventRecord(e1, nullptr)); HIPCHK(hipEventSynchronize(e1)); HIPCHK(hipEventElapsedTime(&t, e0, e1));
     } else {
         std::vector<PairGram2Item> items(nsites);
         for (auto& it : items) it.g = g;
-        const int wgs = plan_pair_gram2(items.data(), nsites, nullptr, 16), nwg = wgs / nsites;
+        const int wgs = plan_pair_gram2(items.data(), nsites, nullptr, dbg_env("TNQS_DBG_SPW", 16)), nwg = wgs / nsites;
         DBuf dP((size_t)2 * nsites * nwg * 1024 * 8);
         for (int i = 0; i < nsites; ++i) {
             PairGram2Item& it = items[i]; it.X = (char*)dA.p + (size_t)i * n * 8; it.Y = (char*)dB.p + (size_t)i * n * 8;
@@ -577,6 +583,31 @@
     if (out_x) for (int i = 0; i < nitems; ++i) if (both[i]) HIPCHK(hipMemcpy((char*)out_x + (size_t)i * 256 * 8, (char*)dO.p + ((size_t)nitems + i) * 256 * 8, 256 * 8, hipMemcpyDeviceToHost));
 }
 
+static void bulk_items(int nitems, const int* lx, const int* ly, std::vector<PairGeom>& g) {
+    if (nitems < 1 || !lx || !ly) throw Err(TNQS_ERR_INVALID, "dbg plane walk: bad arguments");
+    const int chi[4] = {32, 32, 32, 32};
+    g.resize((size_t)nitems);
+    for (int i = 0; i < nitems; ++i) if (!pair_geometry(2, 4, chi, lx[i], ly[i], g[(size_t)i])) throw Err(TNQS_ERR_UNSUPPORTED, "dbg plane walk: legs not covered by the pair kernels");
+}
+void dbg_pair_walk(int nitems, const int* lx, const int* ly, const void* in, const void* M, void* out, int grid, int k) {
+    need_gpu();
+    std::vector<PairGeom> g; bulk_items(nitems, lx, ly, g);
+    const size_t n1 = (size_t)2 << 20, n = n1 * nitems;
+    DBuf dIn(n * 8), dOut(n * 8), dM((size_t)nitems * 2048 * 8), dI(sizeof(PairItem) * nitems);
+    dIn.up(in, n * 8); dM.up(M, (size_t)nitems * 2048 * 8);
+    HIPCHK(hipMemset(dOut.p, 0xff, n * 8));
+    std::vector<PairItem> items((size_t)nitems);
+    for (int i = 0; i < nitems; ++i) {
+        PairItem& it = items[(size_t)i]; it.g = g[(size_t)i]; it.in = (char*)dIn.p + i * n1 * 8; it.out = (char*)dOut.p + i * n1 * 8;
+        it.Mx = (char*)dM.p + (size_t)i * 2048 * 8; it.My = (char*)it.Mx + 1024 * 8;
+    }
+    PlaneWalk walk = dbg_walk(grid, k); const int wgs = plan_pair(items.data(), nitems, walk); DWalk dW(walk);
+    dI.up(items.data(), sizeof(PairItem) * nitems);
+    launch_mfma_pair(nullptr, (const PairItem*)dI.p, nitems, wgs, dW.p);
+    HIPCHK(hipDeviceSynchronize());
+    dOut.down(out, n * 8);
+}
+
 void dbg_svd_tall(int nitems, const int* m, const int* n, void* A, int* chol_fail, int* polished, int* sweeps) {
     need_gpu();
     if (nitems < 1 || !m || !n || !A) throw Err(TNQS_ERR_INVALID, "dbg_svd_tall: bad arguments");
diff --git a/tensornetworkquantumsimulator.jl_amd/csrc/engine.hpp b/tensornetworkquantumsimulator.jl_amd/csrc/engine.hpp
--- a/tensornetworkquantumsimulator.jl_amd/csrc/engine.hpp
+++ b/tensornetworkquantumsimulator.jl_amd/csrc/engine.hpp
@@ -122,6 +122,7 @@
     int dtype = TNQS_C64;
     bool real_io = false;
     int device = 0;
+    int cus = 0;
     std::vector<int> d;
     std::vector<char> projected;
     std::vector<int> chi;
diff --git a/tensornetworkquantumsimulator.jl_amd/csrc/engine_batch.cpp b/tensornetworkquantumsimulator.jl_amd/csrc/engine_batch.cpp
--- a/tensornetworkquantumsimulator.jl_amd/csrc/engine_batch.cpp
+++ b/tensornetworkquantumsimulator.jl_amd/csrc/engine_batch.cpp
@@ -60,10 +60,11 @@
                 c.steps.erase(c.steps.begin() + se.second.second); c.steps.erase(c.steps.begin() + se.second.first);
                 bytes += 2.0 * c.sd.n * esz; flops += 2 * 8.0 * c.sd.n * 32;
             }
-            const int wgs = plan_pair(items.data(), (int)items.size());
-            const PairItem* d = upload(s, items);
+            PlaneWalk walk = plane_walk_of(s); const WalkShare* dw = nullptr;
+            const int wgs = plan_pair(items.data(), (int)items.size(), walk);
+            const PairItem* d = upload_walk(s, items, walk, &dw);
             ProfScope ps(s, cls_pair, bytes, flops);
-            launch_mfma_pair(s->stream, d, (int)items.size(), wgs);
+            launch_mfma_pair(s->stream, d, (int)items.size(), wgs, dw);
         }
         for (;;) {
             std::vector<Pair16Item> it16; std::vector<std::pair<size_t, std::pair<int, int>>> sel16; double by16 = 0, fl16 = 0;
diff --git a/tensornetworkquantumsimulator.jl_amd/csrc/engine_bp.cpp b/tensornetworkquantumsimulator.jl_amd/csrc/engine_bp.cpp
--- a/tensornetworkquantumsimulator.jl_amd/csrc/engine_bp.cpp
+++ b/tensornetworkquantumsimulator.jl_amd/csrc/engine_bp.cpp
@@ -440,10 +440,11 @@
 
     void launch_products() {
         if (!sh_pair.empty()) {
-            const int wgs = plan_pair(sh_pair.data(), (int)sh_pair.size());
-            const PairItem* d = upload(s, sh_pair);
+            PlaneWalk walk = plane_walk_of(s); const WalkShare* dw = nullptr;
+            const int wgs = plan_pair(sh_pair.data(), (int)sh_pair.size(), walk);
+            const PairItem* d = upload_walk(s, sh_pair, walk, &dw);
             ProfScope ps(s, TNQS_PROF_BP_PAIR, 2.0 * sh_pair_slices * 16384.0 * esz, 2 * 8.0 * sh_pair_slices * 16384.0 * 32);
-            launch_mfma_pair(s->stream, d, (int)sh_pair.size(), wgs);
+            launch_mfma_pair(s->stream, d, (int)sh_pair.size(), wgs, dw);
         }
         on_side(true);
         run_chains<T>(s, chains, TNQS_PROF_BP_MODEPROD, TNQS_PROF_BP_PAIR);
diff --git a/tensornetworkquantumsimulator.jl_amd/csrc/engine_core.cpp b/tensornetworkquantumsimulator.jl_amd/csrc/engine_core.cpp
--- a/tensornetworkquantumsimulator.jl_amd/csrc/engine_core.cpp
+++ b/tensornetworkquantumsimulator.jl_amd/csrc/engine_core.cpp
@@ -199,6 +199,7 @@
     auto s = std::make_unique<State>();
     s->g = make_graph(nv, ne, es, ed);
     s->dtype = dtype; s->real_io = real_io; s->device = device;
+    if (hipDeviceGetAttribute(&s->cus, hipDeviceAttributeMultiprocessorCount, device) != hipSuccess || s->cus <= 0) s->cus = 256;
     s->d.assign(nv, 2);
     if (sd) for (int v = 0; v < nv; ++v) { if (sd[v] < 1 || sd[v] > 16) throw Err(TNQS_ERR_INVALID, "tnqs_create: site dimension out of range"); s->d[v] = sd[v]; }
     s->chi.assign(ne, 1);
@@ -213,7 +214,7 @@
 
 State* state_copy(const State* o) {
     auto s = std::make_unique<State>();
-    s->g = o->g; s->dtype = o->dtype; s->real_io = o->real_io; s->device = o->device; s->d = o->d; s->chi = o->chi;
+    s->g = o->g; s->dtype = o->dtype; s->real_io = o->real_io; s->device = o->device; s->cus = o->cus; s->d = o->d; s->chi = o->chi;
     s->site = o->site; s->sscale = o->sscale; s->msg = o->msg; s->pool = o->pool; s->prof = o->prof;
     s->pend1 = o->pend1; s->unit_norm = o->unit_norm; s->projected = o->projected;
     s->rank = o->rank; s->nranks = o->nranks; s->owner = o->owner; s->ag_fn = o->ag_fn; s->ag_ctx = o->ag_ctx;
diff --git a/tensornetworkquantumsimulator.jl_amd/csrc/engine_internal.hpp b/tensornetworkquantumsimulator.jl_amd/csrc/engine_internal.hpp
--- a/tensornetworkquantumsimulator.jl_amd/csrc/engine_internal.hpp
+++ b/tensornetworkquantumsimulator.jl_amd/csrc/engine_internal.hpp
@@ -108,6 +108,26 @@
     return reinterpret_cast<const Item*>(b->p);
 }
 
+template <class Item> const Item* upload_walk(State* s, const std::vector<Item>& v, const PlaneWalk& w, const WalkShare** d_shares) {
+    static_assert(sizeof(Item) % alignof(WalkShare) == 0, "the shares follow the items");
+    *d_shares = nullptr;
+    if (w.shares.empty() || v.empty()) return upload(s, v);
+    const size_t ib = v.size() * sizeof(Item), bytes = ib + w.shares.size() * sizeof(WalkShare);
+    HostArena& ar = s->arena;
+    if (!ar.base) ar = acquire_arena();
+    const size_t aligned = (bytes + 255) & ~size_t(255);
+    if (aligned > ar.cap) throw Err(TNQS_ERR_UNSUPPORTED, "descriptor batch too large");
+    if (ar.off + aligned > ar.cap) { drain_for_arena_reuse(s); ar.off = 0; s->prof->chain = false; }
+    char* h = ar.base + ar.off; ar.off += aligned;
+    std::memcpy(h, v.data(), ib); std::memcpy(h + ib, w.shares.data(), bytes - ib);
+    Buf b = dalloc(s, bytes);
+    HIPCHK(hipMemcpyAsync(b->p, h, bytes, hipMemcpyHostToDevice, s->stream));
+    s->keepalive.push_back(b);
+    *d_shares = reinterpret_cast<const WalkShare*>(static_cast<const char*>(b->p) + ib);
+    return reinterpret_cast<const Item*>(b->p);
+}
+inline PlaneWalk plane_walk_of(const State* s) { PlaneWalk w; w.cus = s->cus; return w; }
+
 template <class Item> const Item* upload_small(State* s, const std::vector<Item>& v) {
     if (v.empty()) return nullptr;
     const size_t bytes = v.size() * sizeof(Item);
diff --git a/tensornetworkquantumsimulator.jl_amd/csrc/kernels.hpp b/tensornetworkquantumsimulator.jl_amd/csrc/kernels.hpp
--- a/tensornetworkquantumsimulator.jl_amd/csrc/kernels.hpp
+++ b/tensornetworkquantumsimulator.jl_amd/csrc/kernels.hpp
@@ -314,9 +314,15 @@
 void launch_mfma_gauge_gram32(hipStream_t s, const GramItem* d_items, int nitems, int total_chunks);
 void launch_mfma_gauge_gram64(hipStream_t s, const GramItem* d_items, int nitems, int total_chunks);
 bool launch_mfma_gram128_f64(hipStream_t s, const GramItem* d_items, int nitems, int total_chunks, int KKmax, bool all_kk128 = false);
-int plan_pair(PairItem* it, int n, int spw = 0);
-void launch_mfma_pair(hipStream_t s, const PairItem* d_items, int nitems, int total_wgs);
-void launch_x3_pair(hipStream_t s, const PairItem* d_items, int nitems, int total_wgs);
+struct WalkShare { int item, s_begin, count; };
+__host__ __device__ inline int walk_pair_of(int gw) { return ((gw >> 4) << 3) | (gw & 7); }
+__host__ __device__ inline int walk_half_of(int gw) { return (gw >> 3) & 1; }
+struct PlaneWalk { int cus = 0, k = 0, grid = 0; std::vector<WalkShare> shares; };
+int plane_walk_grid(int cus, int k, long long total_slices);
+void plan_plane_walk(const int* slices, int n, int grid, std::vector<WalkShare>& shares);
+int plan_pair(PairItem* it, int n, PlaneWalk& w, int spw = 0);
+void launch_mfma_pair(hipStream_t s, const PairItem* d_items, int nitems, int total_wgs, const WalkShare* d_shares);
+void launch_x3_pair(hipStream_t s, const PairItem* d_items, int nitems, int total_wgs, const WalkShare* d_shares);
 struct PairGram2Item { const void* X; const void* Y; const void* Mx; const void* My; void* partial_y; void* partial_x; PairGeom g; int wg_begin; int spw; };
 int plan_pair_gram2(PairGram2Item* it, int n, int* nwg = nullptr, int spw = 0);
 void launch_mfma_pair_gram2(hipStream_t s, const PairGram2Item* d_items, int nitems, int total_wgs);
diff --git a/tensornetworkquantumsimulator.jl_amd/csrc/kernels_mfma.hip b/tensornetworkquantumsimulator.jl_amd/csrc/kernels_mfma.hip
--- a/tensornetworkquantumsimulator.jl_amd/csrc/kernels_mfma.hip
+++ b/tensornetworkquantumsimulator.jl_amd/csrc/kernels_mfma.hip
@@ -509,15 +509,23 @@
     #undef TNQS_PIN
 }
 static int pair_slices(const PairGeom& g) { return g.n0 * g.n1 * g.n2; }
-int plan_pair(PairItem* it, int n, int spw) {
+int plan_pair(PairItem* it, int n, PlaneWalk& w, int spw) {
+    w.shares.clear();
+    if (mfma_use_x3()) {
+        std::vector<int> sl((size_t)n); long long tot = 0;
+        for (int i = 0; i < n; ++i) { it[i].slice_begin = 0; it[i].spw = 0; sl[(size_t)i] = pair_slices(it[i].g); tot += sl[(size_t)i]; }
+        const int grid = w.grid > 0 ? w.grid : plane_walk_grid(w.cus, w.k > 0 ? w.k : plane_walk_k(), tot);
+        plan_plane_walk(sl.data(), n, grid, w.shares);
+        return grid;
+    }
     if (spw <= 0) {
         double tot = 0; for (int i = 0; i < n; ++i) tot += pair_slices(it[i].g); spw = 16; while (spw > 1 && 2.0 * tot / spw < 1024.0) spw >>= 1;
     }
     return lay_out(it, n, &PairItem::slice_begin, nullptr, [&](PairItem& p) { p.spw = spw; const int np = (pair_slices(p.g) + spw - 1) / spw; return 16 * ((np + 7) / 8); });
 }
-void launch_mfma_pair(hipStream_t s, const PairItem* d_items, int nitems, int total_wgs) {
+void launch_mfma_pair(hipStream_t s, const PairItem* d_items, int nitems, int total_wgs, const WalkShare* d_shares) {
     if (total_wgs <= 0) return;
-    if (mfma_use_x3()) { launch_x3_pair(s, d_items, nitems, total_wgs); return; }
+    if (mfma_use_x3()) { launch_x3_pair(s, d_items, nitems, total_wgs, d_shares); return; }
     const size_t lds = (size_t)16 * (32 * 33 + 4) * 2 * sizeof(float);
     set_max_dynamic_lds((const void*)mfma_pair_kernel, lds); hipLaunchKernelGGL(mfma_pair_kernel, dim3(total_wgs), dim3(512), lds, s, d_items, nitems);
     TNQS_CHECK_LAUNCH();
diff --git a/tensornetworkquantumsimulator.jl_amd/csrc/kernels_x3.hip b/tensornetworkquantumsimulator.jl_amd/csrc/kernels_x3.hip
--- a/tensornetworkquantumsimulator.jl_amd/csrc/kernels_x3.hip
+++ b/tensornetworkquantumsimulator.jl_amd/csrc/kernels_x3.hip
@@ -196,21 +196,22 @@
     TNQS_CHECK_LAUNCH();
 }
 
-__global__ __launch_bounds__(512) __attribute__((amdgpu_waves_per_eu(2, 2))) void x3_pair_kernel(const PairItem* __restrict__ items, int nitems) {
+__global__ __launch_bounds__(512) __attribute__((amdgpu_waves_per_eu(2, 2))) void x3_pair_kernel(const PairItem* __restrict__ items, const WalkShare* __restrict__ shares) {
     constexpr int P = 34;
     constexpr int PS = 32 * P + 2;
     constexpr int BUF = 8 * PS;
     extern __shared__ __attribute__((aligned(16))) char smem[];
     v2f* L = reinterpret_cast<v2f*>(smem);
     const int tid = threadIdx.x, lane = tid & 63, w = tid >> 6, ln = lane & 31, h = lane >> 5;
-    const int gw = blockIdx.x;
-    const int lo = find_item(items, nitems, &PairItem::slice_begin, gw);
-    const PairItem it = items[lo];
+    const int gw = blockIdx.x, half = walk_half_of(gw);
+    const WalkShare sh = shares[walk_pair_of(gw)];
+    #define TNQS_PIN() __builtin_amdgcn_sched_barrier(0x2 | 0x4)
+    int left = sh.count, s_first = sh.s_begin;
+    for (int item = sh.item; left > 0; ++item, s_first = 0) {
+    const PairItem it = items[item];
     const PairGeom g = it.g;
-    const int nslices = g.n0 * g.n1 * g.n2;
-    const int lw = gw - it.slice_begin;
-    const int half = (lw >> 3) & 1, pw = ((lw >> 4) << 3) | (lw & 7);
-    const int s_begin = pw * it.spw, s_end = min(nslices, s_begin + it.spw);
+    const int s_begin = s_first, s_end = min(g.n0 * g.n1 * g.n2, s_begin + left);
+    left -= s_end - s_begin;
     const cf* __restrict__ in = reinterpret_cast<const cf*>(it.in);
     cf* __restrict__ out = reinterpret_cast<cf*>(it.out);
     P3 Mxr[2], Mxi[2];
@@ -234,7 +235,6 @@
     const long long toff = (long long)(4 * half + f4) * g.cstr + g.sx * ix0 + g.sy * iy0, tstr = 4 * g.sy;
     v2f* const lbase = L + (2 * f4) * PS + iy0 * P + ix0;
     v4f preA[8], preB[8];
-    #define TNQS_PIN() __builtin_amdgcn_sched_barrier(0x2 | 0x4)
     auto commit = [&](int buf, const v4f (&pre)[8]) {
 #pragma unroll
         for (int j = 0; j < 8; ++j) {
@@ -249,7 +249,7 @@
         v4f v; v[0] = a[0]; v[1] = a[1]; v[2] = c[0]; v[3] = c[1];
         stg4(out + ob + tstr * j, v);
     };
-    if (s_begin < s_end) {
+    {
         const long long b = x3_slice_base(g, s_begin) + toff;
 #pragma unroll
         for (int j = 0; j < 8; ++j) preB[j] = ldg4(in + b + tstr * j);
@@ -305,19 +305,22 @@
         phase(sl, 0, preA, preB);
         if (sl + 1 < s_end) phase(sl + 1, 1, preB, preA);
     }
-    if (s_begin < s_end) {
+    {
         const int buf = (s_end - 1 - s_begin) & 1;
         const long long ob = x3_slice_base(g, s_end - 1) + toff;
 #pragma unroll
         for (int j = 0; j < 8; ++j) store1(buf, ob, j);
     }
+    lds_barrier();
+    }
     #undef TNQS_PIN
 }
-void launch_x3_pair(hipStream_t s, const PairItem* d_items, int nitems, int total_wgs) {
+void launch_x3_pair(hipStream_t s, const PairItem* d_items, int nitems, int total_wgs, const WalkShare* d_shares) {
     if (total_wgs <= 0) return;
+    if (!d_shares || total_wgs % 16) throw_unsupported("x3 pair: a launch needs the shares of its walk and whole groups of 16 workgroups");
     const size_t lds = (size_t)16 * (32 * 34 + 2) * 2 * sizeof(float) + 12 * 64 * 16;
     set_max_dynamic_lds((const void*)x3_pair_kernel, lds);
-    hipLaunchKernelGGL(x3_pair_kernel, dim3(total_wgs), dim3(512), lds, s, d_items, nitems);
+    hipLaunchKernelGGL(x3_pair_kernel, dim3(total_wgs), dim3(512), lds, s, d_items, d_shares);
     TNQS_CHECK_LAUNCH();
 }
 
diff --git a/tensornetworkquantumsimulator.jl_amd/csrc/launch_util.hpp b/tensornetworkquantumsimulator.jl_amd/csrc/launch_util.hpp
--- a/tensornetworkquantumsimulator.jl_amd/csrc/launch_util.hpp
+++ b/tensornetworkquantumsimulator.jl_amd/csrc/launch_util.hpp
@@ -22,4 +22,7 @@
 
 inline bool mfma_use_x3() { static const bool v = [] { const char* e = std::getenv("TNQS_NO_BF16X3"); return !(e && e[0] == '1'); }(); return v; }
 
+
+inline int plane_walk_k() { static const int v = [] { const char* e = std::getenv("TNQS_WALK_K"); const int k = e ? std::atoi(e) : 0; return (k == 1 || k == 2 || k == 4) ? k : 1; }(); return v; }
+
 }
diff --git a/tensornetworkquantumsimulator.jl_amd/csrc/plane_walk.cpp b/tensornetworkquantumsimulator.jl_amd/csrc/plane_walk.cpp
--- /dev/null
+++ b/tensornetworkquantumsimulator.jl_amd/csrc/plane_walk.cpp
@@ -0,0 +1,33 @@
+#include <algorithm>
+#include "kernels.hpp"
+
+namespace tnqs {
+
+int plane_walk_grid(int cus, int k, long long total_slices) {
+    if (cus <= 0) cus = 256;
+    cus = std::max(16, cus / 16 * 16);
+    if (k <= 0) k = 1;
+    const long long need = 16 * ((total_slices + 7) / 8);
+    return (int)std::max<long long>(16, std::min<long long>((long long)k * cus, need));
+}
+
+void plan_plane_walk(const int* slices, int n, int grid, std::vector<WalkShare>& shares) {
+    if (grid <= 0 || grid % 16) throw_unsupported("plane walk: the workgroups of a launch come in groups of 16");
+    const int pairs = grid / 2;
+    long long T = 0; for (int i = 0; i < n; ++i) T += slices[i];
+    shares.assign((size_t)pairs, WalkShare{0, 0, 0});
+    int item = 0, off = 0;
+    for (int p = 0; p < pairs; ++p) {
+        int rem = (int)(T * (p + 1) / pairs - T * p / pairs);
+        if (rem == 0) continue;
+        while (off == slices[item]) { ++item; off = 0; }
+        shares[(size_t)p] = WalkShare{item, off, rem};
+        while (rem > 0) {
+            if (off == slices[item]) { ++item; off = 0; }
+            const int seg = std::min(rem, slices[item] - off);
+            off += seg; rem -= seg;
+        }
+    }
+}
+
+}
```

Result: faster. 6892 (median of 5 runs) (+1.8%).
